# klauspost/compress

Measured on AMD Instinct MI355X. Metric: encode MB/s (input) + ratio, zstd SpeedFastest 128KiB blocks, 1/2/4/8 GPU, higher is better.
Workload: dtype u8

## Files before the change

compress_amd/csrc/kc_batch.cpp:

```cpp
#include "kc_host.h"

namespace kci {


void build_better_dict_tables(const uint8_t* dict, size_t len, int pos_bits, uint8_t* out, int reserved_bits = 0) {
    const int TB = (32 - pos_bits - reserved_bits) > 16 ? 16 : (32 - pos_bits - reserved_bits);
    auto tagOf = [&](uint32_t v) -> uint32_t { return TB > 0 ? ((v * 2654435761u) >> (32 - TB)) : 0u; };
    auto mk = [&](uint64_t pos, uint32_t val) -> uint32_t { return ((uint32_t)pos + 1u) | (tagOf(val) << pos_bits); };
    auto ld64h = [&](size_t i) -> uint64_t { uint64_t v; memcpy(&v, dict + i, 8); return v; };
    uint32_t* ltab = (uint32_t*)out;
    uint32_t* stab = (uint32_t*)(out + ((size_t)8 << 19));
    if (len < 8) return;
    for (size_t i = 0; i + 8 < len; i += 4) {
        const uint64_t cv = ld64h(i);
        for (int k = 0; k < 4; k++) {
            const uint64_t v = cv >> (8 * k);
            const uint32_t h = (uint32_t)(((v << 24) * 889523592379ULL) >> (64 - 13));
            stab[h] = mk(i + k, (uint32_t)v);
        }
    }
    for (size_t i = 0; i + 8 < len || i == 0; i++) {
        const uint64_t cv = ld64h(i);
        const uint32_t h = (uint32_t)((cv * 0xcf1bbcdcb7a56463ULL) >> (64 - 19));
        const uint32_t old = ltab[2 * h];
        ltab[2 * h] = mk(i, (uint32_t)cv);
        ltab[2 * h + 1] = old;
        if (i + 8 >= len) break;
    }
}

void build_fast_dict_table(const uint8_t* dict, size_t len, int pos_bits, uint32_t* tab) {
    const int TB = (32 - pos_bits) > 16 ? 16 : (32 - pos_bits);
    auto tagOf = [&](uint32_t v) -> uint32_t { return TB > 0 ? ((v * 2654435761u) >> (32 - TB)) : 0u; };
    auto mk = [&](uint64_t pos, uint32_t val) -> uint32_t { return ((uint32_t)pos + 1u) | (tagOf(val) << pos_bits); };
    if (len < 8) return;
    for (size_t i = 0; i + 8 < len; i += 2) {
        uint64_t cv;
        memcpy(&cv, dict + i, 8);
        const uint32_t h0 = (uint32_t)(((cv << 16) * 227718039650203ULL) >> (64 - 15));
        const uint32_t h1 = (uint32_t)((((cv >> 8) << 16) * 227718039650203ULL) >> (64 - 15));
        tab[h0] = mk(i, (uint32_t)cv);
        tab[h1] = mk(i + 1, (uint32_t)(cv >> 8));
    }
}
void build_dfast_dict_long(const uint8_t* dict, size_t len, int pos_bits, uint32_t* ltab) {
    const int TB = (32 - pos_bits) > 16 ? 16 : (32 - pos_bits);
    auto tagOf = [&](uint32_t v) -> uint32_t { return TB > 0 ? ((v * 2654435761u) >> (32 - TB)) : 0u; };
    if (len < 8) return;
    for (size_t i = 0; i == 0 || i + 8 < len; i++) {
        uint64_t cv;
        memcpy(&cv, dict + i, 8);
        const uint32_t h = (uint32_t)((cv * 0xcf1bbcdcb7a56463ULL) >> (64 - 17));
        ltab[h] = ((uint32_t)i + 1u) | (tagOf((uint32_t)cv) << pos_bits);
        if (i + 8 >= len) break;
    }
}

kc_status check_supported(kc_ctx* c, const kc_zstd_opts* o) {
    if (o->level < KC_SPEED_FASTEST || o->level > KC_SPEED_BEST) { c->err = "unknown encoder level"; return KC_ERR_UNSUPPORTED; }
    if (o->dict_len > ((uint64_t)64 << 20)) { c->err = "dictionary larger than 64 MiB not served by the device path"; return KC_ERR_UNSUPPORTED; }
    if (o->block_size < 1024 || o->block_size > kMaxCompressedBlockSize || o->window_size < kMinWindowSize) { c->err = "bad block/window size"; return KC_ERR_BAD_ARG; }
    return KC_OK;
}


size_t match_table_bytes(int level) {
    if (level == KC_SPEED_BEST) return 0;
    return level == KC_SPEED_BETTER ? kc_zbetter_table_bytes() : (level == KC_SPEED_DEFAULT ? kc_zdfast_table_bytes() : kc_zfast_table_bytes());
}

bool zfast_use_lds(const kc_ctx* c, const KcMatchParams& mp, uint32_t n_launch, int level) {
    (void)mp;
    if (level != KC_SPEED_FASTEST) return false;
    if (c->cfg.match_path == KC_PATH_HBM) return false;
    if (c->cfg.match_path == KC_PATH_LDS) return true;
    return (int64_t)n_launch <= c->cfg.zfast_lds_max_units;
}
bool zfast_lds_needs_hbm(const kc_ctx* c, const KcMatchParams& mp) {
    return (uint64_t)mp.hist0 + c->plan.max_unit_bytes > KC_ZFAST_LDS_MAX_UNIT;
}

kc_status ensure_best_slots(kc_ctx* c, uint32_t n_launch, hipStream_t st) {
    uint32_t want = (uint32_t)std::min<int64_t>((int64_t)n_launch, c->cfg.best_slots);
    if (want < 1) want = 1;
    if (!c->best_cost.p) {
        kc_status s = ensure(c, c->predef, kc_fse_predef_bytes());
        if (s != KC_OK) return s;
        if (!c->predef_ready) {
            kc_launch_fse_predef_init(c->predef.p, st);
            c->predef_ready = true;
        }
        if ((s = ensure(c, c->best_cost, 96 * 4)) != KC_OK) return s;
        kc_launch_zbest_cost(c->predef.p, (int32_t*)c->best_cost.p, st);
    }
    if (want <= c->best_n) return KC_OK;
    uint32_t n = 1;
    while (n < want) n <<= 1;
    if ((int64_t)n > c->cfg.best_slots) n = (uint32_t)c->cfg.best_slots;
    size_t fr = 0, tot = 0;
    if (hipMemGetInfo(&fr, &tot) == hipSuccess) {
        const uint64_t room = (uint64_t)((double)(fr + c->best_tables.cap) * 0.8) / kc_zbest_table_bytes();
        if (room < 1) { c->err = "device memory exhausted: no room for one SpeedBestCompression table slot (34 MiB)"; c->oom = true; return KC_ERR_UNSUPPORTED; }
        if ((uint64_t)n > room) n = (uint32_t)room;
    } else (void)hipGetLastError();
    if (n <= c->best_n) return KC_OK;
    HIPCHK(c, hipStreamSynchronize(st));
    if (c->best_tables.p) HIPCHK(c, hipFree(c->best_tables.p));
    c->best_tables.p = nullptr;
    c->best_tables.cap = 0;
    c->best_n = 0;
    {
        const hipError_t e = hipMalloc(&c->best_tables.p, (size_t)n * kc_zbest_table_bytes());
        if (e != hipSuccess) {
            (void)hipGetLastError();
            c->best_tables.p = nullptr;
            c->err = "device memory exhausted (" + std::to_string(((size_t)n * kc_zbest_table_bytes()) >> 20) + " MiB of SpeedBestCompression tables wanted)";
            c->oom = true;
            return KC_ERR_UNSUPPORTED;
        }
        c->best_tables.cap = (size_t)n * kc_zbest_table_bytes();
    }
    kc_status s;
    if ((s = ensure(c, c->best_cur, (size_t)8192 * 4)) != KC_OK) return s;
    HIPCHK(c, hipMemsetAsync(c->best_tables.p, 0, (size_t)n * kc_zbest_table_bytes(), st));
    HIPCHK(c, hipMemsetAsync(c->best_cur.p, 0, (size_t)8192 * 4, st));
    c->best_n = n;
    return KC_OK;
}

bool better_epoch_mode(const kc_ctx* c, int level, int pos_bits, int hist0) {
    return level == KC_SPEED_BETTER && !c->job_primed && c->job_hist == nullptr && pos_bits <= 22 && (hist0 == 0 || c->cfg.better_dict_epoch != 0);
}

kc_status prepare_tables(kc_ctx* c, const KcMatchParams& mp, uint32_t n_launch, hipStream_t st, int level) {
    if (level == KC_SPEED_BEST) return ensure_best_slots(c, n_launch, st);
    { const kc_status sc = tables_claim(c, st); if (sc != KC_OK) return sc; }
    c->better_epoch_now = 0;
    if (better_epoch_mode(c, level, mp.pos_bits, mp.hist0)) {
        const size_t tbb = match_table_bytes(level);
        kc_status se = ensure(c, c->tables, (size_t)n_launch * tbb);
        if (se != KC_OK) return se;
        const bool fresh = c->tab_owner != 1 || c->tab_pb != mp.pos_bits || n_launch > c->tab_units || c->tab_ep >= 15u || c->tab_ptr != c->tables.p;
        if (fresh) {
            HIPCHK(c, hipMemsetAsync(c->tables.p, 0, (size_t)n_launch * tbb, st));
            c->tab_owner = 1;
            c->tab_pb = mp.pos_bits;
            c->tab_units = n_launch;
            c->tab_ep = 1;
            c->tab_ptr = c->tables.p;
        } else {
            c->tab_ep++;
        }
        c->better_epoch_now = c->tab_ep;
        return KC_OK;
    }
    if (zfast_use_lds(c, mp, n_launch, level) && !zfast_lds_needs_hbm(c, mp) && !c->job_primed) return KC_OK;
    const bool fastEpoch = level == KC_SPEED_FASTEST && c->cfg.zfast_epoch != 0 && mp.hist0 == 0 && !c->job_primed && mp.pos_bits + KC_ZF_EPOCH_BITS + 4 <= 32;
    if (!fastEpoch) c->tab_owner = 0;
    c->fast_epoch_now = 0;
    const size_t tb = match_table_bytes(level);
    if (c->job_primed) {
        kc_status sj = ensure(c, c->tables, (size_t)n_launch * tb);
        if (sj != KC_OK) return sj;
        if (c->job_tables == nullptr) {
            HIPCHK(c, hipMemsetAsync(c->tables.p, 0, (size_t)n_launch * tb, st));
            KcPrimeParams pp;
            pp.src = mp.src;
            pp.unit_off = mp.unit_off;
            pp.unit_hist = mp.unit_hist;
            pp.unit_list = mp.unit_list;
            pp.unit_base = mp.unit_base;
            pp.n_launch = n_launch;
            pp.level = level;
            pp.pos_bits = mp.pos_bits;
            pp.tables = (uint8_t*)c->tables.p;
            pp.table_bytes = tb;
            kc_launch_zstd_prime(pp, st);
            return KC_OK;
        }
        if (mp.unit_list == nullptr) {
            HIPCHK(c, hipMemcpyAsync(c->tables.p, c->job_tables, (size_t)n_launch * tb, hipMemcpyHostToDevice, st));
            return KC_OK;
        }
        if (c->job_redo_list.size() < n_launch) { c->err = "job re-run without its unit list"; return KC_ERR_INTERNAL; }
        for (uint32_t i = 0; i < n_launch; i++)
            HIPCHK(c, hipMemcpyAsync((uint8_t*)c->tables.p + (size_t)i * tb, c->job_tables + (size_t)c->job_redo_list[i] * tb, tb, hipMemcpyHostToDevice, st));
        return KC_OK;
    }
    kc_status s = ensure(c, c->tables, (size_t)n_launch * tb);
    if (s != KC_OK) return s;
    if (mp.hist0 > 0) kc_launch_bcast((const uint8_t*)c->proto.p, (uint8_t*)c->tables.p, tb, n_launch, st);
    else if (fastEpoch) {
        const bool fresh = c->tab_owner != 2 || c->tab_pb != mp.pos_bits || n_launch > c->tab_units || c->tab_ep >= (1u << KC_ZF_EPOCH_BITS) - 1u || c->tab_ptr != c->tables.p;
        if (fresh) {
            HIPCHK(c, hipMemsetAsync(c->tables.p, 0, (size_t)n_launch * tb, st));
            c->tab_owner = 2;
            c->tab_pb = mp.pos_bits;
            c->tab_units = n_launch;
            c->tab_ep = 1;
            c->tab_ptr = c->tables.p;
        } else {
            c->tab_ep++;
        }
        c->fast_epoch_now = c->tab_ep;
    }
    else HIPCHK(c, hipMemsetAsync(c->tables.p, 0, (size_t)n_launch * tb, st));
    return KC_OK;
}

void launch_match_kernel(kc_ctx* c, const KcMatchParams& mp, uint32_t slot0, uint32_t n_launch, hipStream_t st, int level, bool lds = false) {
    if (lds) {
        KcMatchParams ml = mp;
        ml.spec_w0 = (int32_t)c->cfg.lds_spec_w0;
        ml.lds_any_big = c->plan.max_unit_bytes > (uint64_t)131072 ? 1 : 0;
        if (c->job_primed)
            kc_launch_zfast_match_lds(ml, (const uint32_t*)((uint8_t*)c->tables.p + (size_t)slot0 * match_table_bytes(level)), 1u << 15, n_launch, st);
        else
            kc_launch_zfast_match_lds(ml, mp.hist0 > 0 ? (const uint32_t*)c->proto.p : nullptr, 0u, n_launch, st);
        c->last_path = KC_PATH_LDS;
        if (zfast_lds_needs_hbm(c, mp)) {
            ml = mp;
            ml.lds_split = 1;
            ml.epoch = c->fast_epoch_now;
            ml.xseg_k = (int32_t)c->cfg.zfast_xseg_k;
            ml.empty_filter = c->cfg.zfast_filter != 0;
            ml.tuned = c->cfg.zfast_variant < 0 ? (c->last_incompressible ? 1 : 0) : (int32_t)c->cfg.zfast_variant;
            kc_launch_zfast_match_grp(ml, (uint32_t*)((uint8_t*)c->tables.p + (size_t)slot0 * match_table_bytes(level)), n_launch, st);
        }
        return;
    }
    c->last_path = KC_PATH_HBM;
    if (level == KC_SPEED_BEST) {
        kc_launch_zbest_match(mp, (uint64_t*)c->best_tables.p, (uint32_t*)c->best_cur.p, (const int32_t*)c->best_cost.p, n_launch, c->best_n, st);
        return;
    }
    uint8_t* tab = (uint8_t*)c->tables.p + (size_t)slot0 * match_table_bytes(level);
    if (level == KC_SPEED_BETTER) {
        KcMatchParams mb = mp;
        mb.epoch = c->better_epoch_now;
        mb.proto = (mb.epoch != 0u && mp.hist0 > 0) ? (const uint8_t*)c->proto.p : nullptr;
        kc_launch_zbetter_match_grp(mb, tab, n_launch, mp.hist0 > 0, st);
    }
    else if (level == KC_SPEED_DEFAULT) kc_launch_zdfast_match_grp(mp, (uint32_t*)tab, n_launch, st);
    else {
        KcMatchParams mf = mp;
        mf.epoch = c->fast_epoch_now;
        mf.xseg_k = (int32_t)c->cfg.zfast_xseg_k;
        mf.empty_filter = c->cfg.zfast_filter != 0;
        mf.tuned = c->cfg.zfast_variant < 0 ? (c->last_incompressible ? 1 : 0) : (int32_t)c->cfg.zfast_variant;
        kc_launch_zfast_match_grp(mf, (uint32_t*)tab, n_launch, st);
    }
}

kc_status launch_match(kc_ctx* c, const KcMatchParams& mp, const uint64_t* unit_off, uint32_t n_units, uint32_t n_launch, int bs, hipStream_t st, int level) {
    (void)unit_off; (void)n_units; (void)bs;
    kc_status s = prepare_tables(c, mp, n_launch, st, level);
    if (s != KC_OK) return s;
    HIPCHK(c, hipEventRecord(c->ev[7], st));
    c->ev7_valid = true;
    launch_match_kernel(c, mp, 0, n_launch, st, level, zfast_use_lds(c, mp, n_launch, level));
    return KC_OK;
}

uint32_t plan_stream_blocks(uint64_t bs, uint64_t len, const uint64_t* cuts, uint64_t n_cuts, std::vector<uint32_t>* starts, uint32_t* flags) {
    uint64_t pos = 0, ci = 0, lastStart = 0;
    uint32_t ub = 0;
    while (pos < len) {
        uint64_t e = pos + bs;
        while (ci < n_cuts && cuts[ci] <= pos) ci++;
        if (ci < n_cuts && cuts[ci] < e) e = cuts[ci];
        if (e > len) e = len;
        if (starts) starts->push_back((uint32_t)pos);
        lastStart = pos;
        pos = e;
        ub++;
    }
    const bool flushedAtEnd = n_cuts > 0 && cuts[n_cuts - 1] >= len;
    const bool tailBuffered = ub > 0 && !flushedAtEnd && (len - lastStart) < bs;
    const bool streamU = len > 0 && !(ub == 1 && tailBuffered);
    *flags = (streamU ? 1u : 0u) | ((streamU && !tailBuffered) ? 2u : 0u);
    return ub;
}

kc_status batch_begin(kc_ctx* c, const kc_zstd_opts* o, const uint8_t* d_src_base, const uint64_t* unit_off, uint32_t n_units,
                      uint8_t* d_dst, uint64_t dst_cap, ChunkFeed* feed) {
    hipStream_t st = c->stream;
    if (c->pend) { c->err = "a batch is already in flight on this context"; return KC_ERR_BAD_ARG; }
    const int bs = o->block_size;
    Plan& pl = c->plan;
    pl.n_units = n_units;
    pl.blk0.resize(n_units + 1);
    pl.stage_off.resize(n_units + 1);
    pl.rel_off.resize(n_units + 1);
    uint64_t so = 0;
    uint32_t nb = 0;
    const bool irregular = c->cuts != nullptr;
    pl.blk_start.clear();
    pl.unit_flags.clear();
    for (uint32_t i = 0; i < n_units; i++) {
        const uint64_t len = unit_off[i + 1] - unit_off[i];
        pl.blk0[i] = nb;
        pl.stage_off[i] = so;
        pl.rel_off[i] = unit_off[i] - unit_off[0];
        uint32_t ub = (uint32_t)((len - (c->job_hist ? c->job_hist[i] : 0) + bs - 1) / bs);
        if (irregular) {
            const uint64_t* cp = c->cuts + c->cut_off[c->cut_unit0 + i];
            const uint64_t nc = c->cut_off[c->cut_unit0 + i + 1] - c->cut_off[c->cut_unit0 + i];
            uint32_t fl = 0;
            ub = plan_stream_blocks((uint64_t)bs, len, cp, nc, &pl.blk_start, &fl);
            pl.unit_flags.push_back(fl);
        }
        nb += ub;
        so += ((uint64_t)kc_zstd_max_encoded_size(o, (int64_t)len) + (irregular ? 3ull * (c->cut_off[c->cut_unit0 + i + 1] - c->cut_off[c->cut_unit0 + i]) + 3ull : 0ull) + 15) & ~(uint64_t)15;
    }
    pl.blk0[n_units] = nb;
    pl.stage_off[n_units] = so;
    pl.rel_off[n_units] = unit_off[n_units] - unit_off[0];
    pl.n_blocks = nb;
    pl.seq_stride = (uint32_t)(bs / 4 + 8);
    pl.lit_stride = (uint32_t)(bs + 64);
    if (so > dst_cap) { c->err = "dst_cap smaller than the sum of MaxEncodedSize(unit)"; return KC_ERR_DST_TOO_SMALL; }

    kc_status s;
    if ((s = ensure(c, c->unit_off, (n_units + 1) * 8)) || (s = ensure(c, c->unit_blk0, (n_units + 1) * 4)) ||
        (s = ensure(c, c->stage_off, (n_units + 1) * 8)) || (s = ensure(c, c->out_off, (n_units + 1 + (feed ? feed->cut.size() : 0)) * 8)) ||
        (s = ensure(c, c->seqs, (size_t)nb * pl.seq_stride * 8)) || (s = ensure(c, c->aux, (size_t)nb * pl.seq_stride * 8)) ||
        (s = ensure(c, c->lits, (size_t)nb * pl.lit_stride)) || (s = ensure(c, c->meta, (size_t)nb * sizeof(KcBlkMeta))) ||
        (s = ensure(c, c->stage, so + 64)) || (s = ensure(c, c->out_size, (size_t)n_units * 4)) ||
        (s = ensure(c, c->xxh, (size_t)n_units * 8)) || (s = ensure(c, c->redo, (size_t)n_units * 4)) ||
        (s = ensure(c, c->redo_blk, (size_t)nb + 1)) || (s = ensure(c, c->pop_blk, (size_t)nb + 1)) || (s = ensure(c, c->unit_list, (size_t)n_units * 4)) ||
        (s = ensure(c, c->predef, kc_fse_predef_bytes())) || (s = ensure(c, c->errflag, 64)))
        return s;
    if (!c->predef_ready) {
        kc_launch_fse_predef_init(c->predef.p, st);
        c->predef_ready = true;
    }
    if (irregular) {
        if ((s = ensure(c, c->blk_start, ((size_t)nb + 1) * 4)) || (s = ensure(c, c->unit_flags, (size_t)n_units * 4))) return s;
        if (nb) HIPCHK(c, hipMemcpyAsync(c->blk_start.p, pl.blk_start.data(), (size_t)nb * 4, hipMemcpyHostToDevice, st));
        HIPCHK(c, hipMemcpyAsync(c->unit_flags.p, pl.unit_flags.data(), (size_t)n_units * 4, hipMemcpyHostToDevice, st));
    }
    {
        auto same = [](const std::vector<uint8_t>& held, const void* p, size_t n, const void* dev, const void* held_dev) {
            return dev == held_dev && held.size() == n && memcmp(held.data(), p, n) == 0;
        };
        auto keep = [](std::vector<uint8_t>& held, const void* p, size_t n) { held.assign((const uint8_t*)p, (const uint8_t*)p + n); };
        const size_t n8 = (size_t)(n_units + 1) * 8, n4 = (size_t)(n_units + 1) * 4;
        if (!same(c->up_unit_off, pl.rel_off.data(), n8, c->unit_off.p, c->up_ptr[0])) {
            HIPCHK(c, hipMemcpyAsync(c->unit_off.p, pl.rel_off.data(), n8, hipMemcpyHostToDevice, st));
            keep(c->up_unit_off, pl.rel_off.data(), n8);
            c->up_ptr[0] = c->unit_off.p;
        }
        if (!same(c->up_blk0, pl.blk0.data(), n4, c->unit_blk0.p, c->up_ptr[1])) {
            HIPCHK(c, hipMemcpyAsync(c->unit_blk0.p, pl.blk0.data(), n4, hipMemcpyHostToDevice, st));
            keep(c->up_blk0, pl.blk0.data(), n4);
            c->up_ptr[1] = c->unit_blk0.p;
        }
        if (!same(c->up_stage_off, pl.stage_off.data(), n8, c->stage_off.p, c->up_ptr[2])) {
            HIPCHK(c, hipMemcpyAsync(c->stage_off.p, pl.stage_off.data(), n8, hipMemcpyHostToDevice, st));
            keep(c->up_stage_off, pl.stage_off.data(), n8);
            c->up_ptr[2] = c->stage_off.p;
        }
    }

    const uint8_t* d_src = d_src_base + unit_off[0];
    const bool useDict = o->dict != nullptr && o->dict_len > 0;
    const int hist0 = useDict ? (int)o->dict_len : 0;
    uint64_t maxLen = 16;
    for (uint32_t i = 0; i < n_units; i++) maxLen = std::max<uint64_t>(maxLen, unit_off[i + 1] - unit_off[i]);
    pl.max_unit_bytes = maxLen;
    int pos_bits = 1;
    while (((uint64_t)1 << pos_bits) <= (uint64_t)hist0 + maxLen + 2) pos_bits++;
    if (std::min<uint64_t>((uint64_t)o->window_size, (uint64_t)hist0 + maxLen) + 3 > 0xFFFFFFull) {
        c->err = "window above 8 MiB with units above 16 MiB: offsets beyond the device path's 24-bit sequence field";
        return KC_ERR_UNSUPPORTED;
    }
    const uint8_t* k_src = d_src;
    const uint64_t* k_off = (const uint64_t*)c->unit_off.p;
    if (useDict) {
        std::vector<uint64_t> woff(n_units + 1);
        for (uint32_t i = 0; i <= n_units; i++) woff[i] = pl.rel_off[i] + (uint64_t)i * (uint64_t)hist0;
        if ((s = ensure(c, c->work, woff[n_units] + 64)) || (s = ensure(c, c->work_off, (n_units + 1) * 8)) ||
            (s = ensure(c, c->dictbuf, (size_t)hist0 + 64)) || (s = ensure(c, c->proto, kc_zbetter_table_bytes())))
            return s;
        HIPCHK(c, hipMemcpyAsync(c->work_off.p, woff.data(), (n_units + 1) * 8, hipMemcpyHostToDevice, st));
        const bool epochMode = better_epoch_mode(c, o->level, pos_bits, hist0);
        uint64_t key = 0xcbf29ce484222325ULL;
        for (int i = 0; i < hist0; i++) key = (key ^ o->dict[i]) * 0x100000001b3ULL;
        key ^= ((uint64_t)(uint32_t)hist0 << 32) ^ ((uint64_t)o->level << 8) ^ ((uint64_t)pos_bits << 16) ^ (epochMode ? (uint64_t)1 << 24 : 0);
        if (key == 0) key = 1;
        const size_t tbz = kc_zbetter_table_bytes();
        if (c->proto_key != key || c->proto_ptr != c->proto.p || c->dictbuf_ptr != c->dictbuf.p) {
            c->proto_key = 0;
            HIPCHK(c, hipMemcpyAsync(c->dictbuf.p, o->dict, (size_t)hist0, hipMemcpyHostToDevice, st));
            std::vector<uint8_t> proto(tbz, 0);
            if (o->level == KC_SPEED_BEST) {  }
            else if (o->level == KC_SPEED_BETTER) {
                build_better_dict_tables(o->dict, (size_t)hist0, pos_bits, proto.data(), epochMode ? 4 : 0);
            } else if (o->level == KC_SPEED_DEFAULT) {
                build_dfast_dict_long(o->dict, (size_t)hist0, pos_bits, (uint32_t*)proto.data());
                build_fast_dict_table(o->dict, (size_t)hist0, pos_bits, (uint32_t*)(proto.data() + ((size_t)4 << 17)));
            } else build_fast_dict_table(o->dict, (size_t)hist0, pos_bits, (uint32_t*)proto.data());
            HIPCHK(c, hipMemcpyAsync(c->proto.p, proto.data(), proto.size(), hipMemcpyHostToDevice, st));
            HIPCHK(c, hipStreamSynchronize(st));
            c->proto_key = key;
            c->proto_ptr = c->proto.p;
            c->dictbuf_ptr = c->dictbuf.p;
        } else {
            HIPCHK(c, hipStreamSynchronize(st));
        }
        kc_launch_prefix_units(d_src, (const uint64_t*)c->unit_off.p, (const uint64_t*)c->work_off.p, (const uint8_t*)c->dictbuf.p,
                               (uint32_t)hist0, (uint8_t*)c->work.p, n_units, st);
        k_src = (const uint8_t*)c->work.p;
        k_off = (const uint64_t*)c->work_off.p;
    }
    if (c->job_hist) {
        if (useDict) { c->err = "jobs of a WithConcurrentBlocks stream take no dictionary"; return KC_ERR_INTERNAL; }
        if ((s = ensure(c, c->d_job_hist, (size_t)n_units * 4)) || (s = ensure(c, c->d_job_flags, (size_t)n_units * 4))) return s;
        HIPCHK(c, hipMemcpyAsync(c->d_job_hist.p, c->job_hist, (size_t)n_units * 4, hipMemcpyHostToDevice, st));
        HIPCHK(c, hipMemcpyAsync(c->d_job_flags.p, c->job_flags, (size_t)n_units * 4, hipMemcpyHostToDevice, st));
    }
    KcMatchParams mp;
    memset(&mp, 0, sizeof(mp));
    mp.unit_hist = c->job_hist ? (const uint32_t*)c->d_job_hist.p : nullptr;
    mp.job_flags = c->job_hist ? (const uint32_t*)c->d_job_flags.p : nullptr;
    mp.src = k_src;
    mp.src_end = k_src + (useDict ? pl.rel_off[n_units] + (uint64_t)n_units * (uint64_t)hist0 : pl.rel_off[n_units]);
    mp.unit_off = k_off;
    mp.hist0 = hist0;
    mp.pos_bits = pos_bits;
    mp.stream_mode = c->stream_mode;
    mp.rep1 = (int32_t)o->dict_offsets[0];
    mp.rep2 = (int32_t)o->dict_offsets[1];
    mp.rep3 = (int32_t)o->dict_offsets[2];
    if (mp.rep1 <= 0 || mp.rep2 <= 0 || mp.rep3 <= 0) { mp.rep1 = 1; mp.rep2 = 4; mp.rep3 = 8; }
    mp.unit_blk0 = (const uint32_t*)c->unit_blk0.p;
    mp.seqs = (uint64_t*)c->seqs.p;
    mp.meta = (KcBlkMeta*)c->meta.p;
    mp.pop_blk = nullptr;
    mp.unit_list = nullptr;
    mp.blk_start = irregular ? (const uint32_t*)c->blk_start.p : nullptr;
    mp.unit_flags = irregular ? (const uint32_t*)c->unit_flags.p : nullptr;
    mp.seq_stride = pl.seq_stride;
    mp.block_size = bs;
    mp.max_match_off = o->window_size;
    mp.spec_w0 = c->cfg.spec_w0 >= 0 ? (int)c->cfg.spec_w0 : (o->level == KC_SPEED_DEFAULT ? 2 : (o->level == KC_SPEED_BETTER ? 16 : 1));
    mp.spec_grow = c->cfg.spec_grow >= 0 ? (int)c->cfg.spec_grow : (o->level == KC_SPEED_FASTEST ? 1 : (o->level == KC_SPEED_BETTER ? 0 : 2));
    if (mp.spec_w0 < 1) mp.spec_w0 = 1;
    if (mp.spec_w0 > 64) mp.spec_w0 = 64;

    KcEntropyParams ep;
    memset(&ep, 0, sizeof(ep));
    ep.unit_hist = mp.unit_hist;
    ep.job_flags = mp.job_flags;
    ep.src = k_src;
    ep.unit_off = k_off;
    ep.hist0 = hist0;
    ep.stream_mode = c->stream_mode;
    ep.stream_sync = o->concurrent == 1;
    ep.dict_huf = nullptr;
    ep.dict_huf_len = 0;
    ep.dict_huf_log = 0;
    if (o->dict_huf_len > 0) {
        uint8_t blobh[768];
        memcpy(blobh, o->dict_huf_val, 512);
        memcpy(blobh + 512, o->dict_huf_nbits, 256);
        if ((s = ensure(c, c->dicthuf, 768))) return s;
        HIPCHK(c, hipMemcpyAsync(c->dicthuf.p, blobh, 768, hipMemcpyHostToDevice, st));
        HIPCHK(c, hipStreamSynchronize(st));
        ep.dict_huf = (const uint8_t*)c->dicthuf.p;
        ep.dict_huf_len = o->dict_huf_len;
        ep.dict_huf_log = o->dict_huf_log;
    }
    ep.unit_blk0 = mp.unit_blk0;
    ep.seqs = mp.seqs;
    ep.meta = mp.meta;
    ep.lits = (uint8_t*)c->lits.p;
    ep.aux = (uint64_t*)c->aux.p;
    ep.stage = (uint8_t*)c->stage.p;
    ep.stage_off = (const uint64_t*)c->stage_off.p;
    ep.out_size = (uint32_t*)c->out_size.p;
    ep.xxh = (const uint64_t*)c->xxh.p;
    ep.redo_mask = (uint32_t*)c->redo.p;
    ep.redo_blk = (uint8_t*)c->redo_blk.p;
    ep.blk_start = mp.blk_start;
    ep.unit_flags = mp.unit_flags;
    ep.unit_list = nullptr;
    ep.predef = c->predef.p;
    ep.seq_stride = pl.seq_stride;
    ep.lit_stride = pl.lit_stride;
    ep.block_size = bs;
    ep.window_size = o->window_size;
    ep.crc = o->crc;
    ep.single = o->single;
    ep.no_entropy = o->no_entropy;
    ep.all_lit_entropy = o->all_lit_entropy;
    ep.full_zero = o->full_zero;
    ep.dict_id = o->dict_id;
    ep.err_flag = (uint32_t*)c->errflag.p;
    if ((s = ensure(c, c->rawdef, ((size_t)nb + 1) * sizeof(KcRawDef))) != KC_OK) return s;
    ep.rawdef = (KcRawDef*)c->rawdef.p;
    const bool fuse_xxh = c->cfg.fuse_raw_xxh != 0 && o->crc && !c->job_hist && !useDict && hist0 == 0 && !irregular && (bs % 256) == 0 && feed == nullptr;
    ep.unit_raw = nullptr;
    if (fuse_xxh) {
        if ((s = ensure(c, c->unit_raw, (size_t)n_units * 4 + 4)) != KC_OK) return s;
        ep.unit_raw = (uint32_t*)c->unit_raw.p;
        ep.xxh = nullptr;
    }
    {
        KcClearList cl;
        memset(&cl, 0, sizeof(cl));
        auto add = [&](void* q, size_t bytes) { cl.p[cl.count] = q; cl.n16[cl.count] = (bytes + 15) / 16; cl.count++; };
        add(c->redo.p, (size_t)n_units * 4);
        add(c->redo_blk.p, (size_t)nb + 1);
        add(c->errflag.p, 64);
        add(c->rawdef.p, ((size_t)nb + 1) * sizeof(KcRawDef));
        if (fuse_xxh) add(c->unit_raw.p, (size_t)n_units * 4);
        kc_launch_clear(cl, st);
    }
    ep.prof = nullptr;
    const bool k2prof = c->cfg.k2_prof != 0;
    if (k2prof) {
        if ((s = ensure(c, c->prof, 48 * 8)) != KC_OK) return s;
        HIPCHK(c, hipMemsetAsync(c->prof.p, 0, 48 * 8, st));
        ep.prof = (unsigned long long*)c->prof.p;
        mp.prof = (unsigned long long*)c->prof.p + 32;
    }

    if (c->chain_after) HIPCHK(c, hipStreamWaitEvent(st, c->chain_after->ev[2], 0));
    HIPCHK(c, hipEventRecord(c->ev[0], st));
    c->prescan_ran = false;
    {
        const bool tuned_now = c->cfg.zfast_variant < 0 ? c->last_incompressible : c->cfg.zfast_variant == 1;
        const bool want = c->cfg.zfast_prescan > 0 || (c->cfg.zfast_prescan < 0 && tuned_now);
        if (want && o->level == KC_SPEED_FASTEST && fuse_xxh && !c->stream_mode && !o->all_lit_entropy && bs >= 16 && n_units > 0) {
            if (c->probe_bs != bs || c->probe_rel.p == nullptr) {
                std::vector<uint32_t> rel(4096);
                uint32_t n = kc_zfast_probe_positions(bs, rel.data(), (uint32_t)rel.size());
                if (n > rel.size()) { rel.resize(n); n = kc_zfast_probe_positions(bs, rel.data(), (uint32_t)rel.size()); }
                if ((s = ensure(c, c->probe_rel, (size_t)n * 4 + 16)) != KC_OK) return s;
                HIPCHK(c, hipMemcpyAsync(c->probe_rel.p, rel.data(), (size_t)n * 4, hipMemcpyHostToDevice, st));
                HIPCHK(c, hipStreamSynchronize(st));
                c->probe_bs = bs;
                c->probe_n = n;
            }
            if ((s = ensure(c, c->unit_done, (size_t)n_units * 4 + 16)) != KC_OK) return s;
            KcPrescanParams pp;
            memset(&pp, 0, sizeof(pp));
            pp.src = k_src;
            pp.unit_off = k_off;
            pp.unit_blk0 = mp.unit_blk0;
            pp.n_units = n_units;
            pp.block_size = bs;
            pp.probe_rel = (const uint32_t*)c->probe_rel.p;
            pp.n_probe = c->probe_n;
            pp.rep1 = mp.rep1;
            pp.rep2 = mp.rep2;
            pp.meta = mp.meta;
            pp.unit_done = (uint32_t*)c->unit_done.p;
            pp.stage = ep.stage;
            pp.stage_off = ep.stage_off;
            pp.out_size = ep.out_size;
            pp.rawdef = ep.rawdef;
            pp.unit_raw = ep.unit_raw;
            pp.window_size = o->window_size;
            pp.crc = o->crc;
            pp.single = o->single;
            pp.dict_id = o->dict_id;
            kc_launch_zfast_prescan(pp, st);
            mp.unit_done = pp.unit_done;
            ep.unit_done = pp.unit_done;
            c->prescan_ran = true;
        }
    }
    mp.unit_base = 0;
    ep.unit_base = 0;
    if (feed == nullptr) {
        if (o->crc && !c->job_hist && !fuse_xxh) kc_launch_xxh64(d_src, (const uint64_t*)c->unit_off.p, n_units, (uint64_t*)c->xxh.p, st);
        HIPCHK(c, hipEventRecord(c->ev[1], st));
        if ((s = launch_match(c, mp, unit_off, n_units, n_units, bs, st, o->level)) != KC_OK) return s;
    } else {
        if (useDict) { c->err = "chunk feed does not take dictionaries"; return KC_ERR_INTERNAL; }
        HIPCHK(c, hipEventRecord(c->ev[1], st));
        if ((s = prepare_tables(c, mp, n_units, st, o->level)) != KC_OK) return s;
        const bool feed_lds = zfast_use_lds(c, mp, n_units, o->level);
        HIPCHK(c, hipEventRecord(c->ev[6], st));
        const size_t nchunk = feed->cut.size() - 1;
        for (size_t k = 0; k < nchunk; k++) {
            if (!feed->wait_recorded(k)) { c->err = "host pipeline: staging failed"; return KC_ERR_HIP; }
            hipStream_t sk = feed->streams[k % feed->streams.size()];
            const uint32_t u0 = feed->cut[k], nk = feed->cut[k + 1] - feed->cut[k];
            HIPCHK(c, hipStreamWaitEvent(sk, c->ev[6], 0));
            HIPCHK(c, hipStreamWaitEvent(sk, feed->landed[k], 0));
            if (o->crc) kc_launch_xxh64(d_src, (const uint64_t*)c->unit_off.p + u0, nk, (uint64_t*)c->xxh.p + u0, sk);
            KcMatchParams mk = mp;
            mk.unit_base = u0;
            launch_match_kernel(c, mk, u0, nk, sk, o->level, feed_lds);
            KcEntropyParams ek = ep;
            ek.unit_base = u0;
            kc_launch_zstd_entropy(ek, nk, sk);
            feed->loc_off = (uint64_t*)c->out_off.p;
            kc_launch_scan_sizes((const uint32_t*)c->out_size.p + u0, nk, feed->loc_off + u0 + k, sk);
            kc_launch_compact((const uint8_t*)c->stage.p, (const uint64_t*)c->stage_off.p + u0, (const uint32_t*)c->out_size.p + u0,
                              feed->loc_off + u0 + k, d_dst + pl.stage_off[u0], nk, sk, ep.src, ep.unit_off + u0, ep.unit_blk0 + u0, ep.rawdef);
            HIPCHK(c, hipEventRecord(feed->done[k], sk));
        }
        for (size_t k = 0; k < nchunk; k++) HIPCHK(c, hipStreamWaitEvent(st, feed->done[k], 0));
    }
    HIPCHK(c, hipEventRecord(c->ev[2], st));
    HIPCHK(c, hipGetLastError());
    Pending* P = new Pending();
    P->o = *o;
    P->mp = mp;
    P->ep = ep;
    P->unit_off.assign(unit_off, unit_off + n_units + 1);
    P->n_units = n_units;
    P->d_dst = d_dst;
    P->need = pl.stage_off[n_units];
    P->fed = feed != nullptr;
    P->bs = bs;
    P->k2prof = k2prof;
    c->pend = P;
    return KC_OK;
}

kc_status batch_end(kc_ctx* c, uint64_t* out_off_host, uint64_t* produced) {
    if (!c->pend) { c->err = "no batch in flight on this context"; return KC_ERR_BAD_ARG; }
    std::unique_ptr<Pending> P((Pending*)c->pend);
    c->pend = nullptr;
    hipStream_t st = c->stream;
    if (c->stream2 != nullptr) {
        st = c->stream2;
        HIPCHK(c, hipStreamWaitEvent(st, c->ev[2], 0));
    }
    const kc_zstd_opts* o = &P->o;
    KcMatchParams& mp = P->mp;
    KcEntropyParams& ep = P->ep;
    const uint64_t* unit_off = P->unit_off.data();
    const uint32_t n_units = P->n_units;
    uint8_t* d_dst = P->d_dst;
    const int bs = P->bs;
    const bool k2prof = P->k2prof;
    kc_status s;
    kc_launch_zstd_entropy(ep, n_units, st);
    HIPCHK(c, hipEventRecord(c->ev[3], st));
    HIPCHK(c, hipGetLastError());

    auto finish_pass = [&]() -> kc_status {
        kc_launch_scan_sizes((const uint32_t*)c->out_size.p, n_units, (uint64_t*)c->out_off.p, st);
        if (ep.unit_raw != nullptr) {
            KcXxhFinParams xf;
            xf.src = ep.src;
            xf.unit_off = ep.unit_off;
            xf.n_units = n_units;
            xf.stage = (uint8_t*)c->stage.p;
            xf.stage_off = (const uint64_t*)c->stage_off.p;
            xf.out_size = (const uint32_t*)c->out_size.p;
            xf.out_off = (const uint64_t*)c->out_off.p;
            xf.dst = d_dst;
            xf.unit_raw = ep.unit_raw;
            xf.rawdef = ep.rawdef;
            xf.unit_blk0 = ep.unit_blk0;
            xf.xxh_out = (uint64_t*)c->xxh.p;
            xf.mode = (int32_t)c->cfg.xxh_fin_mode;
            kc_launch_xxh64_fin(xf, st);
        }
        kc_launch_compact((const uint8_t*)c->stage.p, (const uint64_t*)c->stage_off.p, (const uint32_t*)c->out_size.p,
                          (const uint64_t*)c->out_off.p, d_dst, n_units, st, ep.src, ep.unit_off, ep.unit_blk0, ep.rawdef, ep.unit_raw);
        HIPCHK(c, hipGetLastError());
        return KC_OK;
    };
    HIPCHK(c, hipEventRecord(c->ev[4], st));
    if ((s = finish_pass()) != KC_OK) return s;
    HIPCHK(c, hipEventRecord(c->ev[5], st));
    uint32_t redo_units = 0;
    {
        const Plan& pl = c->plan;
        const uint32_t nb = pl.n_blocks;
        uint32_t maxBlocks = 1;
        for (uint32_t i = 0; i < n_units; i++) maxBlocks = std::max(maxBlocks, pl.blk0[i + 1] - pl.blk0[i]);
        std::vector<uint32_t> redo(n_units), list;
        std::vector<uint8_t> redo_blk, pop_blk;
        uint32_t errv[16];
        for (uint32_t iter = 0;; iter++) {
            HIPCHK(c, hipMemcpyAsync(redo.data(), c->redo.p, (size_t)n_units * 4, hipMemcpyDeviceToHost, st));
            HIPCHK(c, hipMemcpyAsync(errv, c->errflag.p, 64, hipMemcpyDeviceToHost, st));
            std::vector<uint32_t> doneh;
            if (iter == 0 && c->prescan_ran) {
                doneh.resize(n_units);
                HIPCHK(c, hipMemcpyAsync(doneh.data(), c->unit_done.p, (size_t)n_units * 4, hipMemcpyDeviceToHost, st));
            }
            HIPCHK(c, hipStreamSynchronize(st));
            if (iter == 0) {
                c->last_prescan_units = 0;
                for (uint32_t v : doneh) c->last_prescan_units += v != 0u;
            }
            if (errv[0] != 0) {
                char b[96];
                snprintf(b, sizeof(b), "device invariant violated (code %u)", errv[0]);
                c->err = b;
                return errv[0] == 100u ? KC_ERR_UNSUPPORTED : KC_ERR_INTERNAL;
            }
            list.clear();
            for (uint32_t i = 0; i < n_units; i++)
                if (redo[i]) list.push_back(i);
            if (list.empty()) break;
            if (iter > maxBlocks + 1) { c->err = "speculation re-run did not converge"; return KC_ERR_INTERNAL; }
            redo_blk.resize(nb);
            if (pop_blk.empty()) pop_blk.assign(nb, 0);
            HIPCHK(c, hipMemcpyAsync(redo_blk.data(), c->redo_blk.p, nb, hipMemcpyDeviceToHost, st));
            HIPCHK(c, hipStreamSynchronize(st));
            for (uint32_t i : list)
                for (uint32_t b = pl.blk0[i]; b < pl.blk0[i + 1]; b++)
                    if (redo_blk[b]) { pop_blk[b] = 1; break; }
            redo_units += (uint32_t)list.size();
            HIPCHK(c, hipMemcpyAsync(c->pop_blk.p, pop_blk.data(), nb, hipMemcpyHostToDevice, st));
            HIPCHK(c, hipMemcpyAsync(c->unit_list.p, list.data(), list.size() * 4, hipMemcpyHostToDevice, st));
            HIPCHK(c, hipMemsetAsync(c->redo.p, 0, (size_t)n_units * 4, st));
            HIPCHK(c, hipMemsetAsync(c->redo_blk.p, 0, (size_t)nb + 1, st));
            c->job_redo_list = list;
            mp.pop_blk = (const uint8_t*)c->pop_blk.p;
            mp.unit_list = (const uint32_t*)c->unit_list.p;
            ep.unit_list = mp.unit_list;
            if ((s = launch_match(c, mp, unit_off, n_units, (uint32_t)list.size(), bs, st, o->level)) != KC_OK) return s;
            kc_launch_zstd_entropy(ep, (uint32_t)list.size(), st);
            HIPCHK(c, hipGetLastError());
            HIPCHK(c, hipStreamSynchronize(st));
        }
    }
    if (redo_units != 0) {
        HIPCHK(c, hipEventRecord(c->ev[4], st));
        if ((s = finish_pass()) != KC_OK) return s;
        HIPCHK(c, hipEventRecord(c->ev[5], st));
    }
    HIPCHK(c, hipMemcpyAsync(out_off_host, c->out_off.p, (n_units + 1) * 8, hipMemcpyDeviceToHost, st));
    HIPCHK(c, hipStreamSynchronize(st));
    HIPCHK(c, hipGetLastError());
    float t01 = 0, t12 = 0, t23 = 0, t34 = 0, t45 = 0, t05 = 0, tk2 = 0;
    (void)hipEventElapsedTime(&t01, c->ev[0], c->ev[1]);
    (void)hipEventElapsedTime(&t12, c->ev[1], c->ev[2]);
    (void)hipEventElapsedTime(&t23, c->ev[2], c->ev[3]);
    (void)hipEventElapsedTime(&t34, c->ev[3], c->ev[4]);
    (void)hipEventElapsedTime(&t45, c->ev[4], c->ev[5]);
    (void)hipEventElapsedTime(&t05, c->ev[0], c->ev[5]);
    if (c->ev7_valid) {
        float t17 = 0;
        if (hipEventElapsedTime(&t17, c->ev[1], c->ev[7]) == hipSuccess && t17 >= 0 && t17 <= t12) c->last.prep_ms += t17;
        c->ev7_valid = false;
    }
    tk2 = t23;
    c->last.match_ms += t12;
    c->last.entropy_ms += tk2;
    c->last.other_ms += t01 + t34 + t45;
    c->last.total_ms += t05;
    c->last.redo_units += redo_units;
    if (k2prof) {
        unsigned long long pv[48];
        HIPCHK(c, hipMemcpy(pv, c->prof.p, sizeof(pv), hipMemcpyDeviceToHost));
        {
            unsigned long long lt = 0;
            for (int i = 32; i < 40; i++) lt += pv[i];
            if (lt && o->level == KC_SPEED_DEFAULT) {
                fprintf(stderr, "[dfast stats] per unit: probes looked up %.0f, committed %.0f, candidate / repeat 16-byte loads %.0f, long lookups at s+1 %.0f, matches %.0f, offset-2 matches %.0f, ring refills (128 B) %.0f\n",
                        (double)pv[32] / n_units, (double)pv[33] / n_units, (double)pv[34] / n_units, (double)pv[35] / n_units, (double)pv[36] / n_units, (double)pv[37] / n_units, (double)pv[38] / n_units);
            } else if (lt) {
                fprintf(stderr, "[LDS match prof] shader clocks per phase (window, probe bytes, table, candidates issued, verdicts, commit, -, round tail):");
                for (int i = 32; i < 40; i++) fprintf(stderr, " %.1f%%", 100.0 * (double)pv[i] / (double)lt);
                fprintf(stderr, "  (total %.4g cycles over %u units)\n", (double)lt, n_units);
            }
        }
        {
            unsigned long long ft = 0;
            for (int i = 40; i < 48; i++) ft += pv[i];
            if (ft) {
                fprintf(stderr, "[K2 fine] wave 0, shader clocks per unit; -DKC_K2_FINE=1: gather (pass A, barrier, step: sequences + scan, step: literal loads + ORs, step: flush + histogram, step: carry + zero, tail, closing barrier); =2: (Huffman size pass, payload zero fill + barrier, stream emit, barrier, payload copy + headers, code staging, chains, pack):");
                for (int i = 40; i < 48; i++) fprintf(stderr, " %.0f", (double)pv[i] / (double)(n_units ? n_units : 1));
                fprintf(stderr, "\n");
            }
        }
        unsigned long long tot = 0;
        for (int i = 0; i < 16; i++) tot += pv[i];
        fprintf(stderr, "[K2 prof] shader-clock share per phase:");
        for (int i = 0; i < 14; i++) fprintf(stderr, " p%d=%.1f%%", i, tot ? 100.0 * (double)pv[i] / (double)tot : 0.0);
        fprintf(stderr, "  (total %.3g cycles over %u units)\n", (double)tot, n_units);
        fprintf(stderr, "[K2 prof] tANS chains (counted with -DKC_CHAIN_STATS): %llu chunk-streams (%llu RLE, %llu predefined), %llu repair passes (LL %llu, OF %llu, ML %llu; %llu on RLE tables), %llu segments re-encoded\n",
                pv[16], pv[26], pv[27], pv[17], pv[18], pv[19], pv[20], pv[25], pv[24]);
    }
    *produced = out_off_host[n_units];
    {
        const uint64_t in_total = unit_off[n_units] - unit_off[0];
        c->last_incompressible = in_total >= (1u << 20) && (double)*produced >= 0.98 * (double)in_total;
    }
    return KC_OK;
}

uint64_t zstd_unit_scratch(const kc_zstd_opts* o, uint64_t len, uint64_t n_cuts) {
    const uint64_t bsz = (uint64_t)o->block_size;
    const uint64_t table_b = o->level == KC_SPEED_BEST ? 0 : o->level == KC_SPEED_BETTER ? kc_zbetter_table_bytes() : (o->level == KC_SPEED_DEFAULT ? kc_zdfast_table_bytes() : kc_zfast_table_bytes());
    const uint64_t per_block = 2 * (bsz / 4 + 8) * 8 + (bsz + 64) + sizeof(KcBlkMeta);
    const uint64_t hist0 = (o->dict != nullptr) ? o->dict_len : 0;
    const uint64_t blocks = (len + bsz - 1) / bsz + n_cuts;
    const uint64_t enc = ((uint64_t)kc_zstd_max_encoded_size(o, (int64_t)len) + 3 * n_cuts + 3 + 15) & ~(uint64_t)15;
    return table_b + blocks * per_block + enc + (hist0 ? hist0 + len : 0) + 64;
}

uint64_t scratch_budget(kc_ctx* c) {
    uint64_t budget = c->max_scratch_bytes;
    size_t fr = 0, tot = 0;
    if (hipMemGetInfo(&fr, &tot) == hipSuccess) {
        uint64_t held = 0;
        const DevBuf* bufs[] = {&c->seqs, &c->aux, &c->lits, &c->meta, &c->stage, &c->tables, &c->work};
        for (const DevBuf* b : bufs) held += b->cap;
        const uint64_t avail = (uint64_t)((double)(fr + held) * 0.85);
        if (avail < budget) budget = avail;
    } else {
        (void)hipGetLastError();
    }
    return budget;
}

kc_status feed_finish(kc_ctx* c, bool* redo_needed) {
    if (!c->pend) { c->err = "no batch in flight on this context"; return KC_ERR_BAD_ARG; }
    std::unique_ptr<Pending> P((Pending*)c->pend);
    c->pend = nullptr;
    hipStream_t st = c->stream;
    const uint32_t n_units = P->n_units;
    std::vector<uint32_t> redo(n_units);
    uint32_t errv[16];
    HIPCHK(c, hipMemcpyAsync(redo.data(), c->redo.p, (size_t)n_units * 4, hipMemcpyDeviceToHost, st));
    HIPCHK(c, hipMemcpyAsync(errv, c->errflag.p, 64, hipMemcpyDeviceToHost, st));
    HIPCHK(c, hipStreamSynchronize(st));
    HIPCHK(c, hipGetLastError());
    if (errv[0] != 0) {
        char b[96];
        snprintf(b, sizeof(b), "device invariant violated (code %u)", errv[0]);
        c->err = b;
        return errv[0] == 100u ? KC_ERR_UNSUPPORTED : KC_ERR_INTERNAL;
    }
    *redo_needed = false;
    for (uint32_t i = 0; i < n_units; i++) if (redo[i]) *redo_needed = true;
    return KC_OK;
}

kc_status run_batch(kc_ctx* c, const kc_zstd_opts* o, const uint8_t* d_src_base, const uint64_t* unit_off, uint32_t n_units,
                    uint8_t* d_dst, uint64_t dst_cap, uint64_t* out_off_host, uint64_t* produced) {
    kc_status s = batch_begin(c, o, d_src_base, unit_off, n_units, d_dst, dst_cap);
    if (s != KC_OK) return s;
    return batch_end(c, out_off_host, produced);
}

}

extern "C" {

kc_status kc_zstd_encode_units_dev(kc_ctx* c, const kc_zstd_opts* o, const uint8_t* d_src, const uint64_t* unit_off, uint32_t n_units,
                                   uint8_t* d_dst, uint64_t dst_cap, uint64_t* out_off) {
    if (!c || !o || !unit_off || !out_off || (n_units && (!d_src || !d_dst))) return KC_ERR_BAD_ARG;
    c->err.clear();
    c->last = kc_timings{0, 0, 0, 0, 0, 0};
    kc_status s = check_supported(c, o);
    if (s != KC_OK) return s;
    HIPCHK(c, hipSetDevice(c->device));
    for (uint32_t i = 0; i < n_units; i++) {
        if (unit_off[i + 1] < unit_off[i]) { c->err = "unit_off not ascending"; return KC_ERR_BAD_ARG; }
        if (unit_off[i + 1] - unit_off[i] > KC_MAX_UNIT_BYTES) {
            c->err = "unit larger than 1 GiB: not served by the device path";
            return KC_ERR_UNSUPPORTED;
        }
    }
    out_off[0] = 0;
    c->last_batches = 0;
    uint64_t pos = 0;
    uint32_t i0 = 0;
    std::vector<uint64_t> tmp;
    auto unit_scratch = [&](uint32_t i) {
        const uint64_t nc = c->cuts ? c->cut_off[i + 1] - c->cut_off[i] : 0;
        return zstd_unit_scratch(o, unit_off[i + 1] - unit_off[i], nc);
    };
    uint64_t budget = scratch_budget(c);
    for (int attempt = 0;; attempt++) {
        bool oom = false;
        while (i0 < n_units) {
            uint32_t i1 = i0;
            const uint64_t cap_bytes = o->level == KC_SPEED_BETTER ? ((uint64_t)1 << 30) : c->max_batch_bytes;
            const uint32_t cap_units = o->level == KC_SPEED_BETTER ? 16384u : 0xFFFFFFFFu;
            uint64_t scratch = 0;
            while (i1 < n_units) {
                const uint64_t us = unit_scratch(i1);
                if (i1 > i0 && (unit_off[i1 + 1] - unit_off[i0] > cap_bytes || i1 - i0 >= cap_units || (scratch + us) + ((scratch + us) >> 3) > budget)) break;
                scratch += us;
                i1++;
            }
            const uint32_t nb = i1 - i0;
            tmp.resize(nb + 1);
            uint64_t produced = 0;
            c->cut_unit0 = i0;
            c->oom = false;
            s = run_batch(c, o, d_src, unit_off + i0, nb, d_dst + pos, dst_cap - pos, tmp.data(), &produced);
            if (s == KC_ERR_UNSUPPORTED && c->oom && nb > 1 && attempt < 6) { oom = true; break; }
            if (s != KC_OK) return s;
            c->last_batches++;
            for (uint32_t k = 0; k <= nb; k++) out_off[i0 + k] = pos + tmp[k];
            pos += produced;
            i0 = i1;
        }
        if (!oom) break;
        budget /= 2;
        c->err.clear();
    }
    if (n_units == 0) out_off[0] = 0;
    return KC_OK;
}

}
namespace kci {
kc_status validate_units(kc_ctx* c, const kc_zstd_opts* o, const uint64_t* unit_off, uint32_t n_units) {
    for (uint32_t i = 0; i < n_units; i++) {
        if (unit_off[i + 1] < unit_off[i]) { c->err = "unit_off not ascending"; return KC_ERR_BAD_ARG; }
        if (unit_off[i + 1] - unit_off[i] > KC_MAX_UNIT_BYTES) {
            c->err = "unit larger than 1 GiB: not served by the device path";
            return KC_ERR_UNSUPPORTED;
        }
    }
    return KC_OK;
}
}
extern "C" {

kc_status kc_zstd_encode_units_dev_begin(kc_ctx* c, const kc_zstd_opts* o, const uint8_t* d_src, const uint64_t* unit_off, uint32_t n_units,
                                         uint8_t* d_dst, uint64_t dst_cap) {
    if (!c || !o || !unit_off || n_units == 0 || !d_src || !d_dst) return KC_ERR_BAD_ARG;
    c->err.clear();
    c->last = kc_timings{0, 0, 0, 0, 0, 0};
    kc_status s = check_supported(c, o);
    if (s != KC_OK) return s;
    HIPCHK(c, hipSetDevice(c->device));
    if ((s = validate_units(c, o, unit_off, n_units)) != KC_OK) return s;
    const uint64_t cap_bytes = o->level == KC_SPEED_BETTER ? ((uint64_t)1 << 30) : c->max_batch_bytes;
    if (unit_off[n_units] - unit_off[0] > cap_bytes || (o->level == KC_SPEED_BETTER && n_units > 16384u)) {
        c->err = "begin/end serves one device batch; use kc_zstd_encode_units_dev for larger inputs";
        return KC_ERR_UNSUPPORTED;
    }
    return batch_begin(c, o, d_src, unit_off, n_units, d_dst, dst_cap);
}

kc_status kc_zstd_encode_units_dev_end(kc_ctx* c, uint64_t* out_off) {
    if (!c || !out_off) return KC_ERR_BAD_ARG;
    HIPCHK(c, hipSetDevice(c->device));
    uint64_t produced = 0;
    return batch_end(c, out_off, &produced);
}

kc_status kc_zstd_encode_units_dev_end_at(kc_ctx* c, uint8_t* d_dst, uint64_t dst_cap, uint64_t* out_off) {
    if (!c || !out_off || !d_dst) return KC_ERR_BAD_ARG;
    if (!c->pend) { c->err = "no batch in flight on this context"; return KC_ERR_BAD_ARG; }
    Pending* P = (Pending*)c->pend;
    if (P->fed) { c->err = "a chunk-fed batch has written its frames already"; return KC_ERR_UNSUPPORTED; }
    if (P->need > dst_cap) { c->err = "dst_cap smaller than the sum of MaxEncodedSize(unit)"; return KC_ERR_DST_TOO_SMALL; }
    P->d_dst = d_dst;
    return kc_zstd_encode_units_dev_end(c, out_off);
}

void kc_ctx_chain_after(kc_ctx* c, kc_ctx* prev) {
    if (c) c->chain_after = prev;
}

kc_status kc_zstd_encode_streams_dev(kc_ctx* c, const kc_zstd_opts* o, const uint8_t* d_src, const uint64_t* unit_off, uint32_t n_units,
                                     uint8_t* d_dst, uint64_t dst_cap, uint64_t* out_off) {
    if (!c || !o) return KC_ERR_BAD_ARG;
    c->stream_mode = 1;
    const kc_status s = kc_zstd_encode_units_dev(c, o, d_src, unit_off, n_units, d_dst, dst_cap, out_off);
    c->stream_mode = 0;
    return s;
}

}
```

compress_amd/csrc/kc_ctx.cpp:

```cpp
#include "kc_host.h"

extern "C" {

void kc_zstd_opts_default(kc_zstd_opts* o) {
    memset(o, 0, sizeof(*o));
    o->level = KC_SPEED_DEFAULT;
    o->window_size = 8 << 20;
    o->block_size = kMaxCompressedBlockSize;
    o->crc = 1;
    o->single = -1;
    o->full_zero = 1;
    o->no_entropy = 0;
    o->all_lit_entropy = 0;
    o->low_mem = 0;
    o->dict_offsets[0] = 1; o->dict_offsets[1] = 4; o->dict_offsets[2] = 8;
    o->concurrent = 0;
}

int kc_zstd_opts_concurrency(kc_zstd_opts* o, int n) {
    if (n < 1) return KC_ERR_BAD_ARG;
    o->concurrent = n;
    return KC_OK;
}

int kc_zstd_opts_level(kc_zstd_opts* o, int l) {
    if (l < KC_SPEED_FASTEST || l > 4) return KC_ERR_BAD_ARG;
    o->level = l;
    if (!o->custom_window) {
        switch (l) {
        case KC_SPEED_FASTEST:
            o->window_size = 4 << 20;
            if (!o->custom_block) o->block_size = 1 << 16;
            break;
        default:
            o->window_size = 8 << 20;
            break;
        }
    }
    if (!o->custom_alent) o->all_lit_entropy = l > KC_SPEED_DEFAULT;
    return KC_OK;
}

int kc_zstd_opts_window(kc_zstd_opts* o, int n) {
    if (n < kMinWindowSize || n > kMaxWindowSize || (n & (n - 1)) != 0) return KC_ERR_BAD_ARG;
    o->window_size = n;
    o->custom_window = 1;
    if (o->block_size > o->window_size) {
        o->block_size = o->window_size;
        o->custom_block = 1;
    }
    return KC_OK;
}
int kc_zstd_opts_crc(kc_zstd_opts* o, int b) { o->crc = b != 0; return KC_OK; }
int kc_zstd_opts_zero_frames(kc_zstd_opts* o, int b) { o->full_zero = b != 0; return KC_OK; }
int kc_zstd_opts_no_entropy(kc_zstd_opts* o, int b) { o->no_entropy = b != 0; return KC_OK; }
int kc_zstd_opts_all_lit_entropy(kc_zstd_opts* o, int b) { o->custom_alent = 1; o->all_lit_entropy = b != 0; return KC_OK; }
int kc_zstd_opts_single_segment(kc_zstd_opts* o, int b) { o->single = b != 0; return KC_OK; }
int kc_zstd_opts_dict_raw(kc_zstd_opts* o, uint32_t id, const uint8_t* content, uint64_t len) {
    if (len > ((uint64_t)1 << 31)) return KC_ERR_BAD_ARG;
    o->dict_id = id;
    o->dict = content;
    o->dict_len = len;
    o->dict_offsets[0] = 1; o->dict_offsets[1] = 4; o->dict_offsets[2] = 8;
    o->dict_huf_len = 0;
    o->dict_huf_log = 0;
    return KC_OK;
}

int64_t kc_zstd_max_encoded_size(const kc_zstd_opts* o, int64_t size) {
    int64_t frameHeader = 4 + 2;
    if (o->dict != nullptr || o->dict_id != 0) frameHeader += 4;
    if (size < 256) frameHeader++;
    else if (size < 65536 + 256) frameHeader += 2;
    else if (size < 0x7fffffff) frameHeader += 4;
    else frameHeader += 8;
    if (o->crc) frameHeader += 4;
    const int64_t blocks = (size + o->block_size) / o->block_size;
    return frameHeader + 3 * blocks + size;
}

namespace {
struct SelfCheck {
    std::mutex m;
    std::condition_variable cv;
    bool done = false;
    kc_status st = KC_OK;
    std::string text;
};
std::mutex g_sc_m;
int g_sc_state[64] = {0};
kc_status g_sc_status[64];
std::string g_sc_text[64];
thread_local std::string t_create_err;

void selfcheck_body(int device, const std::shared_ptr<SelfCheck>& sc) {
    kc_status st = KC_OK;
    std::string text;
    uint8_t h_in[256];
    for (int i = 0; i < 256; i++) h_in[i] = (uint8_t)i;
    const uint64_t h_off[2] = {0, 256};
    uint64_t h_out = 0;
    uint8_t* d_in = nullptr;
    uint64_t *d_off = nullptr, *d_out = nullptr;
    hipStream_t s = nullptr;
    auto fail = [&](const char* what, hipError_t e) { st = KC_ERR_HIP; text = std::string("device self-check: ") + what + ": " + hipGetErrorString(e); };
    hipError_t e = hipSetDevice(device);
    if (e != hipSuccess) fail("hipSetDevice", e);
    if (st == KC_OK && (e = hipStreamCreateWithFlags(&s, hipStreamNonBlocking)) != hipSuccess) fail("hipStreamCreate", e);
    if (st == KC_OK && (e = hipMalloc((void**)&d_in, 256 + 64)) != hipSuccess) fail("hipMalloc", e);
    if (st == KC_OK && (e = hipMalloc((void**)&d_off, 16)) != hipSuccess) fail("hipMalloc", e);
    if (st == KC_OK && (e = hipMalloc((void**)&d_out, 8)) != hipSuccess) fail("hipMalloc", e);
    if (st == KC_OK && (e = hipMemcpyAsync(d_in, h_in, 256, hipMemcpyHostToDevice, s)) != hipSuccess) fail("hipMemcpyAsync (H2D)", e);
    if (st == KC_OK && (e = hipMemcpyAsync(d_off, h_off, 16, hipMemcpyHostToDevice, s)) != hipSuccess) fail("hipMemcpyAsync (H2D)", e);
    if (st == KC_OK) {
        kc_launch_xxh64(d_in, d_off, 1, d_out, s);
        if ((e = hipGetLastError()) != hipSuccess) fail("kernel launch", e);
    }
    if (st == KC_OK && (e = hipMemcpyAsync(&h_out, d_out, 8, hipMemcpyDeviceToHost, s)) != hipSuccess) fail("hipMemcpyAsync (D2H)", e);
    if (st == KC_OK && (e = hipStreamSynchronize(s)) != hipSuccess) fail("hipStreamSynchronize", e);
    if (st == KC_OK && h_out != 0x1FACBE8406CD904BULL) {
        char b[160];
        snprintf(b, sizeof(b), "device self-check: XXH64 known answer differs (got %016llx, want 1facbe8406cd904b): the device computes wrong results", (unsigned long long)h_out);
        st = KC_ERR_INTERNAL;
        text = b;
    }
    if (d_in) (void)hipFree(d_in);
    if (d_off) (void)hipFree(d_off);
    if (d_out) (void)hipFree(d_out);
    if (s) (void)hipStreamDestroy(s);
    std::lock_guard<std::mutex> lk(sc->m);
    sc->st = st;
    sc->text = text;
    sc->done = true;
    sc->cv.notify_all();
}

kc_status device_selfcheck(int device, std::string* text) {
    if (device < 0 || device >= 64) return KC_OK;
    std::lock_guard<std::mutex> g(g_sc_m);
    if (g_sc_state[device] == 0) {
        auto sc = std::make_shared<SelfCheck>();
        std::thread([device, sc] { selfcheck_body(device, sc); }).detach();
        std::unique_lock<std::mutex> lk(sc->m);
        const int deadline_s = 90;
        if (!sc->cv.wait_for(lk, std::chrono::seconds(deadline_s), [&] { return sc->done; })) {
            g_sc_state[device] = -1;
            g_sc_status[device] = KC_ERR_HIP;
            g_sc_text[device] = "device self-check: the device did not answer a 256-byte known-answer launch within " + std::to_string(deadline_s) + " s (hung queue or faulted context): no kc_* call was attempted";
        } else {
            g_sc_state[device] = sc->st == KC_OK ? 1 : -1;
            g_sc_status[device] = sc->st;
            g_sc_text[device] = sc->text;
        }
    }
    if (g_sc_state[device] < 0) { *text = g_sc_text[device]; return g_sc_status[device]; }
    return KC_OK;
}
}

const char* kc_create_error(void) { return t_create_err.c_str(); }

kc_status kc_ctx_create(kc_ctx** out, int device, void* stream) {
    if (!out) return KC_ERR_BAD_ARG;
    *out = nullptr;
    t_create_err.clear();
    int n = 0;
    if (hipGetDeviceCount(&n) != hipSuccess || n <= 0 || device < 0 || device >= n) { t_create_err = "no such HIP device"; return KC_ERR_NO_DEVICE; }
    {
        const kc_status sc = device_selfcheck(device, &t_create_err);
        if (sc != KC_OK) return sc;
    }
    kc_ctx* c = new kc_ctx();
    c->device = device;
    if (hipSetDevice(device) != hipSuccess || hipGetDeviceProperties(&c->prop, device) != hipSuccess) {
        delete c;
        return KC_ERR_NO_DEVICE;
    }
    if (stream) {
        c->stream = (hipStream_t)stream;
    } else {
        if (hipStreamCreate(&c->stream) != hipSuccess) { delete c; return KC_ERR_HIP; }
        c->own_stream = true;
    }
    for (auto& e : c->ev)
        if (hipEventCreate(&e) != hipSuccess) { delete c; return KC_ERR_HIP; }
    *out = c;
    return KC_OK;
}

kc_status kc_ctx_set_option(kc_ctx* c, int key, int64_t v) {
    if (!c) return KC_ERR_BAD_ARG;
    KcCfg& g = c->cfg;
    switch (key) {
        case KC_OPT_MATCH_PATH: if (v < KC_PATH_AUTO || v > KC_PATH_LDS) return KC_ERR_BAD_ARG; g.match_path = v; break;
        case KC_OPT_ZFAST_LDS_MAX_UNITS: g.zfast_lds_max_units = v; break;
        case KC_OPT_S2_LDS_MAX_BLOCKS: g.s2_lds_max_blocks = v; break;
        case KC_OPT_SPEC_W0: g.spec_w0 = v; break;
        case KC_OPT_SPEC_GROW: g.spec_grow = v; break;
        case KC_OPT_LDS_SPEC_W0: g.lds_spec_w0 = v; break;
        case KC_OPT_S2_LDS_SPEC_W0: g.s2_lds_spec_w0 = v; break;
        case KC_OPT_HOST_SERIAL: g.host_serial = v; break;
        case KC_OPT_HOST_PIPE_MIB: g.host_pipe_mib = v; break;
        case KC_OPT_HOST_OVERLAP_MIN_MIB: g.host_overlap_min_mib = v; break;
        case KC_OPT_HOST_COPY_THREADS: g.host_copy_threads = v; break;
        case KC_OPT_HOST_TRACE: g.host_trace = v; break;
        case KC_OPT_HOST_ROLL: g.host_roll = v != 0; break;
        case KC_OPT_HOST_ROLL_MIB: if (v < 0) return KC_ERR_BAD_ARG; g.host_roll_mib = v; break;
        case KC_OPT_HOST_CHUNK_MIB: g.host_chunks.clear(); if (v > 0) g.host_chunks.push_back((uint64_t)v << 20); break;
        case KC_OPT_HOST_CHUNK_MIB_APPEND: if (v < 1) return KC_ERR_BAD_ARG; g.host_chunks.push_back((uint64_t)v << 20); break;
        case KC_OPT_K2_PROF: g.k2_prof = v; break;
        case KC_OPT_S2_HOOK_WAIT_US: g.hook_wait_us = v; break;
        case KC_OPT_S2_HOOK_BATCH: g.hook_batch = v < 1 ? 1 : v; break;
        case KC_OPT_S2_HOOK_LANES: g.hook_lanes = v < 1 ? 1 : (v > 8 ? 8 : v); break;
        case KC_OPT_S2_HOOK_HOST_FIRST: g.hook_host_first = v < -1 ? -1 : v; break;
        case KC_OPT_TEST_FEED_REDO: g.test_feed_redo = v; break;
        case KC_OPT_MAX_SCRATCH_MIB: if (v < 1) return KC_ERR_BAD_ARG; c->max_scratch_bytes = (uint64_t)v << 20; break;
        case KC_OPT_BEST_SLOTS: if (v < 1 || v > 8192) return KC_ERR_BAD_ARG; g.best_slots = v; break;
        case KC_OPT_S2_VARIANT: if (v != KC_S2_VARIANT_GO && v != KC_S2_VARIANT_AMD64) return KC_ERR_BAD_ARG; g.s2_variant = v; break;
        case KC_OPT_BETTER_DICT_EPOCH: g.better_dict_epoch = v != 0; break;
        case KC_OPT_ZFAST_EPOCH: g.zfast_epoch = v != 0; break;
        case KC_OPT_ZFAST_XSEG_K: if (v < 0) return KC_ERR_BAD_ARG; g.zfast_xseg_k = v > (1 << 30) ? (1 << 30) : v; break;
        case KC_OPT_FUSE_RAW_XXH: g.fuse_raw_xxh = v != 0; break;
        case KC_OPT_ZFAST_FILTER: g.zfast_filter = v != 0; break;
        case KC_OPT_ZFAST_VARIANT: if (v < -1 || v > 1) return KC_ERR_BAD_ARG; g.zfast_variant = v; break;
        case KC_OPT_ZFAST_PRESCAN: if (v < -1 || v > 1) return KC_ERR_BAD_ARG; g.zfast_prescan = v; break;
        case KC_OPT_XXH_FIN_MODE: if (v < 0 || v > 3) return KC_ERR_BAD_ARG; g.xxh_fin_mode = v; break;
        case KC_OPT_JOB_PRIME: g.job_prime = v != 0; break;
        case KC_OPT_DSTREAM_BLOCKS: if (v < 1 || v > 4096) return KC_ERR_BAD_ARG; g.dstream_blocks = v; break;
        case KC_OPT_STAGE2_STREAM: if (c->pend) return KC_ERR_BAD_ARG; c->stream2 = (hipStream_t)(intptr_t)v; break;
        default: return KC_ERR_BAD_ARG;
    }
    return KC_OK;
}

int64_t kc_ctx_get_option(const kc_ctx* c, int key) {
    if (!c) return -1;
    const KcCfg& g = c->cfg;
    switch (key) {
        case KC_OPT_MATCH_PATH: return g.match_path;
        case KC_OPT_ZFAST_LDS_MAX_UNITS: return g.zfast_lds_max_units;
        case KC_OPT_S2_LDS_MAX_BLOCKS: return g.s2_lds_max_blocks;
        case KC_OPT_SPEC_W0: return g.spec_w0;
        case KC_OPT_SPEC_GROW: return g.spec_grow;
        case KC_OPT_LDS_SPEC_W0: return g.lds_spec_w0;
        case KC_OPT_S2_LDS_SPEC_W0: return g.s2_lds_spec_w0;
        case KC_OPT_HOST_SERIAL: return g.host_serial;
        case KC_OPT_HOST_PIPE_MIB: return g.host_pipe_mib;
        case KC_OPT_HOST_OVERLAP_MIN_MIB: return g.host_overlap_min_mib;
        case KC_OPT_HOST_COPY_THREADS: return g.host_copy_threads;
        case KC_OPT_HOST_TRACE: return g.host_trace;
        case KC_OPT_HOST_ROLL: return g.host_roll;
        case KC_OPT_HOST_ROLL_MIB: return g.host_roll_mib;
        case KC_OPT_HOST_CHUNK_MIB: return g.host_chunks.empty() ? 0 : (int64_t)(g.host_chunks[0] >> 20);
        case KC_OPT_K2_PROF: return g.k2_prof;
        case KC_OPT_S2_HOOK_WAIT_US: return g.hook_wait_us;
        case KC_OPT_S2_HOOK_BATCH: return g.hook_batch;
        case KC_OPT_S2_HOOK_LANES: return g.hook_lanes;
        case KC_OPT_S2_HOOK_HOST_FIRST: return g.hook_host_first;
        case KC_OPT_TEST_FEED_REDO: return g.test_feed_redo;
        case KC_OPT_MAX_SCRATCH_MIB: return (int64_t)(c->max_scratch_bytes >> 20);
        case KC_OPT_BEST_SLOTS: return g.best_slots;
        case KC_OPT_S2_VARIANT: return g.s2_variant;
        case KC_OPT_BETTER_DICT_EPOCH: return g.better_dict_epoch;
        case KC_OPT_ZFAST_EPOCH: return g.zfast_epoch;
        case KC_OPT_ZFAST_XSEG_K: return g.zfast_xseg_k;
        case KC_OPT_FUSE_RAW_XXH: return g.fuse_raw_xxh;
        case KC_OPT_ZFAST_FILTER: return g.zfast_filter;
        case KC_OPT_ZFAST_VARIANT: return g.zfast_variant;
        case KC_OPT_ZFAST_PRESCAN: return g.zfast_prescan;
        case KC_OPT_XXH_FIN_MODE: return g.xxh_fin_mode;
        case KC_OPT_JOB_PRIME: return g.job_prime;
        case KC_OPT_DSTREAM_BLOCKS: return g.dstream_blocks;
        case KC_OPT_STAGE2_STREAM: return (int64_t)(intptr_t)c->stream2;
        case KC_OPT_LAST_PATH: return c->last_path;
        case KC_OPT_LAST_PRESCAN_UNITS: return c->last_prescan_units;
        case KC_OPT_LAST_BATCHES: return c->last_batches;
        default: return -1;
    }
}

static void ctx_free_scratch(kc_ctx* c) {
    DevBuf* bufs[] = {&c->unit_off, &c->unit_blk0, &c->stage_off, &c->seqs, &c->aux, &c->lits, &c->meta, &c->stage, &c->out_size, &c->xxh,
                      &c->redo, &c->popmask, &c->unit_list, &c->out_off, &c->blk_start, &c->unit_flags, &c->redo_blk, &c->pop_blk, &c->predef, &c->errflag, &c->tmp_src, &c->tmp_dst, &c->tables, &c->prof, &c->work, &c->work_off, &c->dictbuf, &c->proto, &c->dicthuf,
                      &c->d_job_hist, &c->d_job_flags, &c->rawdef, &c->unit_raw, &c->unit_done, &c->probe_rel, &c->best_tables, &c->best_cur, &c->best_cost};
    for (DevBuf* b : bufs) {
        if (b->p) (void)hipFree(b->p);
        b->p = nullptr;
        b->cap = 0;
    }
    for (DevBuf& b : c->zd) {
        if (b.p) (void)hipFree(b.p);
        b.p = nullptr;
        b.cap = 0;
    }
    for (DevBuf& b : c->s2d) {
        if (b.p) (void)hipFree(b.p);
        b.p = nullptr;
        b.cap = 0;
    }
    c->predef_ready = false;
    c->tab_owner = 0;
    c->tab_ptr = nullptr;
    c->tab_units = c->tab_ep = 0;
    c->proto_key = 0;
    c->proto_ptr = c->dictbuf_ptr = nullptr;
    c->best_n = 0;
    c->probe_bs = 0;
    c->probe_n = 0;
    c->preclear_bytes = 0;
    c->preclear_ptr = nullptr;
    c->up_ptr[0] = c->up_ptr[1] = c->up_ptr[2] = nullptr;
}

kc_status kc_ctx_trim(kc_ctx* c) {
    if (!c) return KC_ERR_BAD_ARG;
    if (c->pend || c->job_active) { c->err = "kc_ctx_trim: a batch or a submitted job is in flight on this context"; return KC_ERR_BAD_ARG; }
    HIPCHK(c, hipSetDevice(c->device));
    HIPCHK(c, hipStreamSynchronize(c->stream));
    ctx_free_scratch(c);
    if (c->hpipe) { host_pipe_free(c->hpipe); c->hpipe = nullptr; }
    return KC_OK;
}

kc_status kc_device_trim(int device) { return kci::host_roll_trim(device); }

kc_status kc_host_alloc(void** out, uint64_t bytes) {
    if (!out || bytes == 0) return KC_ERR_BAD_ARG;
    *out = nullptr;
    const hipError_t e = hipHostMalloc(out, (size_t)bytes, hipHostMallocDefault);
    if (e != hipSuccess) { (void)hipGetLastError(); *out = nullptr; return e == hipErrorOutOfMemory ? KC_ERR_UNSUPPORTED : KC_ERR_HIP; }
    return KC_OK;
}
void kc_host_free(void* p) {
    if (p) (void)hipHostFree(p);
}

void kc_ctx_destroy(kc_ctx* c) {
    if (!c) return;
    if (c->job_active && c->job.joinable()) c->job.join();
    (void)hipSetDevice(c->device);
    ctx_free_scratch(c);
    for (auto& e : c->ev)
        if (e) (void)hipEventDestroy(e);
    if (c->ev_preclear) (void)hipEventDestroy(c->ev_preclear);
    if (c->pend) { delete (Pending*)c->pend; c->pend = nullptr; }
    if (c->hook) { s2_hook_free(c->hook); c->hook = nullptr; }
    if (c->hpipe) { host_pipe_free(c->hpipe); c->hpipe = nullptr; }
    if (c->own_stream && c->stream) (void)hipStreamDestroy(c->stream);
    delete c;
}

const char* kc_last_error(const kc_ctx* c) { return c ? c->err.c_str() : "null context"; }

kc_status kc_device_info(const kc_ctx* c, int32_t* n_cu, int32_t* lds_per_cu, int32_t* clock_khz, char* name, size_t name_cap) {
    if (!c) return KC_ERR_BAD_ARG;
    if (n_cu) *n_cu = c->prop.multiProcessorCount;
    if (lds_per_cu) *lds_per_cu = (int32_t)c->prop.maxSharedMemoryPerMultiProcessor;
    if (clock_khz) *clock_khz = c->prop.clockRate;
    if (name && name_cap) { strncpy(name, c->prop.gcnArchName, name_cap - 1); name[name_cap - 1] = 0; }
    return KC_OK;
}

kc_status kc_last_timings(const kc_ctx* c, kc_timings* t) {
    if (!c || !t) return KC_ERR_BAD_ARG;
    *t = c->last;
    return KC_OK;
}

}
```

compress_amd/csrc/kc_dev.h:

```cpp
#pragma once
#include <hip/hip_runtime.h>
#include <stdint.h>

#define KC_WAVE 64

struct __attribute__((packed)) kc_u64u { uint64_t v; };
struct __attribute__((packed)) kc_u32u { uint32_t v; };
struct __attribute__((packed)) kc_u16u { uint16_t v; };
__device__ __forceinline__ uint64_t ld64(const uint8_t* p) { return ((const kc_u64u*)p)->v; }
__device__ __forceinline__ void st64(uint8_t* p, uint64_t v) { ((kc_u64u*)p)->v = v; }
__device__ __forceinline__ uint32_t ld32(const uint8_t* p) { return ((const kc_u32u*)p)->v; }
__device__ __forceinline__ void st32(uint8_t* p, uint32_t v) { ((kc_u32u*)p)->v = v; }
__device__ __forceinline__ uint16_t ld16(const uint8_t* p) { return ((const kc_u16u*)p)->v; }
struct __attribute__((packed)) kc_u128u { uint32_t x, y, z, w; };
__device__ __forceinline__ uint4 ld128u(const uint8_t* p) {
    const kc_u128u v = *(const kc_u128u*)p;
    return make_uint4(v.x, v.y, v.z, v.w);
}

#ifdef KC_HIPEMU
#define KC_WAVE_SYNC() hipemu::wave_sync()
#else
#define KC_WAVE_SYNC() do { __builtin_amdgcn_fence(__ATOMIC_SEQ_CST, "wavefront"); __builtin_amdgcn_wave_barrier(); } while (0)
#endif

__device__ __forceinline__ int lane_id() { return (int)(threadIdx.x & 63); }
__device__ __forceinline__ uint64_t ballot64(bool p) { return __ballot(p); }
__device__ __forceinline__ int ctz64(uint64_t v) { return __builtin_ctzll(v); }
struct KcUnitBlocks { int nblk; bool streamU; bool emptyLast; };
__device__ __forceinline__ KcUnitBlocks kc_unit_blocks(const uint32_t* blk_start, const uint32_t* unit_flags, const uint32_t* unit_blk0,
                                                       uint32_t u, int ulen, int bs, int stream_mode) {
    KcUnitBlocks r;
    if (blk_start != nullptr) {
        const uint32_t f = unit_flags[u];
        r.nblk = (int)(unit_blk0[u + 1] - unit_blk0[u]);
        r.streamU = (f & 1u) != 0u;
        r.emptyLast = (f & 2u) != 0u;
    } else {
        r.nblk = (ulen + bs - 1) / bs;
        r.streamU = stream_mode != 0 && ulen >= bs;
        r.emptyLast = r.streamU && (ulen % bs) == 0;
    }
    return r;
}
__device__ __forceinline__ int kc_blk_begin(const uint32_t* blk_start, uint32_t blk0, int b, int bs) {
    return blk_start != nullptr ? (int)blk_start[blk0 + (uint32_t)b] : b * bs;
}
__device__ __forceinline__ int kc_blk_end(const uint32_t* blk_start, uint32_t blk0, int b, int nblk, int bs, int ulen) {
    if (blk_start != nullptr) return b + 1 < nblk ? (int)blk_start[blk0 + (uint32_t)b + 1u] : ulen;
    const int e = (b + 1) * bs;
    return e < ulen ? e : ulen;
}

__device__ __forceinline__ uint32_t bcast32(uint32_t v, int srcLane) { return (uint32_t)__shfl((int)v, srcLane, 64); }
__device__ __forceinline__ uint64_t bcast64(uint64_t v, int srcLane) {
    uint32_t lo = bcast32((uint32_t)v, srcLane), hi = bcast32((uint32_t)(v >> 32), srcLane);
    return ((uint64_t)hi << 32) | lo;
}
__device__ __forceinline__ uint32_t rdlane32(uint32_t v, int srcLane) { return (uint32_t)__builtin_amdgcn_readlane((int)v, srcLane); }
__device__ __forceinline__ uint64_t rdlane64(uint64_t v, int srcLane) {
    return (uint64_t)rdlane32((uint32_t)v, srcLane) | ((uint64_t)rdlane32((uint32_t)(v >> 32), srcLane) << 32);
}
__device__ __forceinline__ int uni(int v) { return __builtin_amdgcn_readfirstlane(v); }
__device__ __forceinline__ uint32_t uniu(uint32_t v) { return (uint32_t)__builtin_amdgcn_readfirstlane((int)v); }

__device__ __forceinline__ int bits_len32(uint32_t v) { return v == 0 ? 0 : 32 - __builtin_clz(v); }
__device__ __forceinline__ uint32_t high_bit(uint32_t v) { return (uint32_t)(bits_len32(v) - 1); }

#define KC_PRIME4 2654435761u
#define KC_PRIME5 889523592379ULL
#define KC_PRIME6 227718039650203ULL
#define KC_PRIME8 0xcf1bbcdcb7a56463ULL
__device__ __forceinline__ uint32_t hash4(uint32_t u, int bits) { return (u * KC_PRIME4) >> (32 - bits); }
__device__ __forceinline__ uint32_t hash5(uint64_t u, int bits) { return (uint32_t)(((u << 24) * KC_PRIME5) >> (64 - bits)); }
__device__ __forceinline__ uint32_t hash6(uint64_t u, int bits) { return (uint32_t)(((u << 16) * KC_PRIME6) >> (64 - bits)); }
__device__ __forceinline__ uint32_t hash8(uint64_t u, int bits) { return (uint32_t)((u * KC_PRIME8) >> (64 - bits)); }

__device__ __forceinline__ uint64_t seq_pack(uint32_t ll, uint32_t ml, uint32_t of) {
    return (uint64_t)of | ((uint64_t)ml << 24) | ((uint64_t)ll << 44);
}
__device__ __forceinline__ uint32_t seq_of(uint64_t s) { return (uint32_t)(s & 0xFFFFFF); }
__device__ __forceinline__ uint32_t seq_ml(uint64_t s) { return (uint32_t)((s >> 24) & 0xFFFFF); }
__device__ __forceinline__ uint32_t seq_ll(uint64_t s) { return (uint32_t)(s >> 44); }

__device__ __forceinline__ int wave_matchlen(const uint8_t* a, const uint8_t* b, int left, int lane) {
    int n = 0;
    int width = 8;
    for (;;) {
        int words = (left - n) >> 3;
        int active = words < width ? words : width;
        uint64_t diff = 0;
        if (lane < active) diff = ld64(a + n + 8 * lane) ^ ld64(b + n + 8 * lane);
        uint64_t m = ballot64(diff != 0);
        if (m) {
            int fl = ctz64(m);
            uint64_t d = rdlane64(diff, fl);
            return n + 8 * fl + (ctz64(d) >> 3);
        }
        n += 8 * active;
        if (active < width) break;
        width = 64;
    }
    int tail = left - n;
    bool ne = lane < tail && a[n + lane] != b[n + lane];
    uint64_t m = ballot64(ne);
    return n + (m ? ctz64(m) : tail);
}

__device__ __forceinline__ int wave_backlen(const uint8_t* base, int s, int t, int kmax, int lane) {
    int cnt = 0;
    while (cnt < kmax) {
        int k = cnt + lane + 1;
        bool ne = true;
        if (k <= kmax) ne = base[t - k] != base[s - k];
        uint64_t m = ballot64(ne);
        int c = m ? ctz64(m) : 64;
        cnt += c;
        if (c < 64) break;
    }
    return cnt < kmax ? cnt : kmax;
}

template <int G>
__device__ __forceinline__ uint32_t gballot(bool p, int grp) {
    return (uint32_t)((ballot64(p) >> (grp * G)) & ((1ull << G) - 1ull));
}
template <int G>
__device__ __forceinline__ uint64_t gbcast64(uint64_t v, int grp, int srcLig) {
    const int src = grp * G + srcLig;
    const uint32_t lo = (uint32_t)__shfl((int)(uint32_t)v, src, 64), hi = (uint32_t)__shfl((int)(uint32_t)(v >> 32), src, 64);
    return ((uint64_t)hi << 32) | lo;
}
template <int G>
__device__ __forceinline__ uint32_t gbcast32(uint32_t v, int grp, int srcLig) {
    return (uint32_t)__shfl((int)v, grp * G + srcLig, 64);
}
template <int G>
__device__ __forceinline__ int grp_matchlen(const uint8_t* __restrict__ base, int a, int b, int left, int lig, int grp) {
    int n = 0;
    for (;;) {
        const int words = (left - n) >> 3;
        const int active = words < G ? words : G;
        uint64_t diff = 0;
        if (lig < active) diff = ld64(base + a + n + 8 * lig) ^ ld64(base + b + n + 8 * lig);
        const uint32_t m = gballot<G>(diff != 0, grp);
        if (m) {
            const int fl = __builtin_ctz(m);
            const uint64_t d = gbcast64<G>(diff, grp, fl);
            return n + 8 * fl + (ctz64(d) >> 3);
        }
        n += 8 * active;
        if (active < G) break;
    }
    const int tail = left - n;
    for (int k0 = 0; k0 < tail; k0 += G) {
        const int k = k0 + lig;
        const bool ne = k < tail && base[a + n + k] != base[b + n + k];
        const uint32_t m = gballot<G>(ne, grp);
        if (m) return n + k0 + __builtin_ctz(m);
    }
    return n + tail;
}
template <int G>
__device__ __forceinline__ int grp_backlen(const uint8_t* __restrict__ base, int s, int t, int kmax, int lig, int grp) {
    int cnt = 0;
    while (cnt < kmax) {
        const int k = cnt + lig + 1;
        bool ne = true;
        if (k <= kmax) ne = base[t - k] != base[s - k];
        const uint32_t m = gballot<G>(ne, grp);
        const int c = m ? __builtin_ctz(m) : G;
        cnt += c;
        if (c < G) break;
    }
    return cnt < kmax ? cnt : kmax;
}


struct KcBlkMeta {
    uint32_t nseq;
    uint32_t nlit;
    uint32_t extra_lits;
    uint32_t flags;
    uint32_t o1_in, o2_in;
    uint32_t o1_out, o2_out;
};
#define KC_BF_POP_A 1u
#define KC_BF_FORCED 2u
```

compress_amd/csrc/kc_host.h:

```cpp
#pragma once
#include <hip/hip_runtime.h>
#include <stdint.h>
#include <stdio.h>
#include <stdlib.h>
#include <string.h>
#include <atomic>
#include <chrono>
#include <condition_variable>
#include <functional>
#include <memory>
#include <mutex>
#include <string>
#include <thread>
#include <vector>
#include <algorithm>

#include "../../include/kcgpu.h"
#include "kc_kernels.h"


namespace kci {

const int kMinWindowSize = 1 << 10;
const int kMaxWindowSize = 1 << 29;
const int kMaxCompressedBlockSize = 128 << 10;

struct DevBuf {
    void* p = nullptr;
    size_t cap = 0;
};

struct Pending {
    kc_zstd_opts o;
    KcMatchParams mp;
    KcEntropyParams ep;
    std::vector<uint64_t> unit_off;
    uint32_t n_units = 0;
    uint8_t* d_dst = nullptr;
    uint64_t need = 0;
    bool fed = false;
    int bs = 0;
    bool k2prof = false;
};


static const uint64_t KC_MAX_UNIT_BYTES = (uint64_t)1 << 30;

struct ChunkFeed {
    std::vector<uint32_t> cut;
    std::vector<hipEvent_t> landed;
    std::vector<hipEvent_t> done;
    std::vector<hipStream_t> streams;
    std::function<bool(size_t)> wait_recorded;
    uint64_t* loc_off = nullptr;
};

struct Plan {
    uint32_t n_units = 0, n_blocks = 0;
    std::vector<uint32_t> blk0;
    std::vector<uint64_t> stage_off;
    std::vector<uint32_t> blk_start, unit_flags;
    std::vector<uint64_t> stage64;
    std::vector<uint64_t> rel_off;
    uint32_t seq_stride = 0, lit_stride = 0;
    uint64_t max_unit_bytes = 0;
};

}
using namespace kci;

struct KcCfg {
    int64_t match_path = KC_PATH_AUTO;
    int64_t zfast_lds_max_units = 768;
    int64_t s2_lds_max_blocks = 1280;
    int64_t spec_w0 = -1, spec_grow = -1;
    int64_t lds_spec_w0 = 16;
    int64_t s2_lds_spec_w0 = 0;
    int64_t host_serial = 0, host_pipe_mib = 0, host_overlap_min_mib = -1, host_copy_threads = 0, host_trace = 0;
    int64_t host_roll = 1;
    int64_t host_roll_mib = 0;
    std::vector<uint64_t> host_chunks;
    int64_t k2_prof = 0;
    int64_t hook_wait_us = 0, hook_batch = 256, hook_lanes = 4;
    int64_t hook_host_first = -1;
    int64_t test_feed_redo = 0;
    int64_t better_dict_epoch = 0;
    int64_t s2_variant = 0;
    int64_t best_slots = 6144;
    int64_t zfast_epoch = 1;
    int64_t zfast_xseg_k = 0;
    int64_t zfast_variant = -1;
    int64_t zfast_filter = 1;
    int64_t xxh_fin_mode = 1;
    int64_t zfast_prescan = -1;
    int64_t job_prime = 1;
    int64_t dstream_blocks = 512;
    int64_t fuse_raw_xxh = 1;
};

struct kc_ctx {
    KcCfg cfg;
    int device = 0;
    hipStream_t stream = nullptr;
    uint32_t s2_pend_n = 0;
    bool lane_preclear = false;
    hipEvent_t ev_preclear = nullptr;
    void* preclear_ptr = nullptr;
    size_t preclear_bytes = 0;
    hipStream_t stream2 = nullptr;
    bool own_stream = false;
    std::string err;
    bool oom = false;
    hipDeviceProp_t prop;
    DevBuf blk_start, unit_flags, redo_blk, pop_blk;
    DevBuf unit_off, unit_blk0, stage_off, seqs, aux, lits, meta, stage, out_size, xxh, redo, popmask, unit_list, out_off,
        predef, errflag, tmp_src, tmp_dst, tables, prof, work, work_off, dictbuf, proto, dicthuf;
    bool predef_ready = false;
    int tab_owner = 0;
    int tab_pb = 0;
    uint32_t tab_units = 0, tab_ep = 0, better_epoch_now = 0, fast_epoch_now = 0;
    void* tab_ptr = nullptr;
    uint64_t proto_key = 0;
    void* proto_ptr = nullptr;
    void* dictbuf_ptr = nullptr;
    DevBuf best_tables, best_cur, best_cost;
    uint32_t best_n = 0;
    hipEvent_t ev[8] = {nullptr, nullptr, nullptr, nullptr, nullptr, nullptr, nullptr, nullptr};
    kc_timings last = {0, 0, 0, 0, 0, 0};
    size_t max_batch_bytes = (size_t)8 << 30;
    uint64_t max_scratch_bytes = (uint64_t)160 << 30;
    int stream_mode = 0;
    std::thread job;
    bool job_active = false;
    kc_status job_status = KC_OK;
    const uint64_t* cut_off = nullptr;
    const uint64_t* cuts = nullptr;
    uint32_t cut_unit0 = 0;
    const uint32_t* job_hist = nullptr;
    const uint32_t* job_flags = nullptr;
    const uint8_t* job_tables = nullptr;
    bool job_primed = false;
    DevBuf d_job_hist, d_job_flags, rawdef, unit_raw;
    DevBuf zd[20];
    DevBuf s2d[13];
    DevBuf unit_done, probe_rel;
    int probe_bs = 0;
    uint32_t probe_n = 0;
    bool prescan_ran = false;
    int64_t last_prescan_units = 0;
    std::vector<uint32_t> job_redo_list;
    void* pend = nullptr;
    kc_ctx* chain_after = nullptr;
    void* hpipe = nullptr;
    Plan plan;
    std::once_flag hook_once;
    void* hook = nullptr;
    bool ev7_valid = false;
    int last_batches = 0;
    int last_path = 0;
    bool last_incompressible = false;
    std::vector<uint8_t> up_unit_off, up_blk0, up_stage_off;
    const void* up_ptr[3] = {nullptr, nullptr, nullptr};
};

#define KC_S2_MAX_BLOCK ((uint64_t)1 << 30)
#define KC_S2_MAX_FRAMED_BLOCK ((uint64_t)4 << 20)

struct kc_s2_ropts {
    uint32_t max_block = (uint32_t)KC_S2_MAX_FRAMED_BLOCK;
    int ignore_crc = 0;
    int ignore_id = 0;
};

struct kc_zstd_dopts {
    uint64_t max_memory = (uint64_t)64 << 30;
    uint64_t max_window = (uint64_t)1 << 29;
    int ignore_checksum = 0;
    std::vector<KcZdDict> dicts;
    std::vector<uint8_t> arena;
};

namespace kci {

#define HIPCHK(ctx, call)                                                                              \
    do {                                                                                               \
        hipError_t e__ = (call);                                                                       \
        if (e__ != hipSuccess) {                                                                       \
            (ctx)->err = std::string(#call) + ": " + hipGetErrorString(e__);                            \
            return KC_ERR_HIP;                                                                         \
        }                                                                                              \
    } while (0)

inline kc_status ensure(kc_ctx* c, DevBuf& b, size_t bytes) {
    if (b.cap >= bytes) return KC_OK;
    if (b.p) HIPCHK(c, hipFree(b.p));
    b.p = nullptr;
    b.cap = 0;
    size_t want = bytes + (bytes >> 3) + 256;
    hipError_t e = hipMalloc(&b.p, want);
    if (e == hipErrorOutOfMemory) {
        (void)hipGetLastError();
        want = bytes + 256;
        e = hipMalloc(&b.p, want);
    }
    if (e != hipSuccess) {
        (void)hipGetLastError();
        b.p = nullptr;
        if (e == hipErrorOutOfMemory) {
            c->err = "device memory exhausted (" + std::to_string(want >> 20) + " MiB of scratch wanted)";
            c->oom = true;
            return KC_ERR_UNSUPPORTED;
        }
        c->err = std::string("hipMalloc: ") + hipGetErrorString(e);
        return KC_ERR_HIP;
    }
    b.cap = want;
    return KC_OK;
}

inline kc_status tables_claim(kc_ctx* c, hipStream_t st) {
    if (c->preclear_bytes != 0) {
        c->preclear_bytes = 0;
        HIPCHK(c, hipStreamWaitEvent(st, c->ev_preclear, 0));
    }
    return KC_OK;
}

inline int bitsLen32(uint32_t v) { return v == 0 ? 0 : 32 - __builtin_clz(v); }

void s2_hook_free(void* h);
void host_pipe_free(void* h);

}
using namespace kci;

namespace kci {
kc_status check_supported(kc_ctx* c, const kc_zstd_opts* o);
size_t match_table_bytes(int level);
kc_status launch_match(kc_ctx* c, const KcMatchParams& mp, const uint64_t* unit_off, uint32_t n_units, uint32_t n_launch, int bs, hipStream_t st, int level);
uint32_t plan_stream_blocks(uint64_t bs, uint64_t len, const uint64_t* cuts, uint64_t n_cuts, std::vector<uint32_t>* starts, uint32_t* flags);
kc_status batch_begin(kc_ctx* c, const kc_zstd_opts* o, const uint8_t* d_src_base, const uint64_t* unit_off, uint32_t n_units,
                      uint8_t* d_dst, uint64_t dst_cap, ChunkFeed* feed = nullptr);
kc_status batch_end(kc_ctx* c, uint64_t* out_off_host, uint64_t* produced);
uint64_t zstd_unit_scratch(const kc_zstd_opts* o, uint64_t len, uint64_t n_cuts = 0);
uint64_t scratch_budget(kc_ctx* c);
kc_status feed_finish(kc_ctx* c, bool* redo_needed);
kc_status run_batch(kc_ctx* c, const kc_zstd_opts* o, const uint8_t* d_src_base, const uint64_t* unit_off, uint32_t n_units,
                    uint8_t* d_dst, uint64_t dst_cap, uint64_t* out_off_host, uint64_t* produced);
kc_status validate_units(kc_ctx* c, const kc_zstd_opts* o, const uint64_t* unit_off, uint32_t n_units);
typedef std::function<kc_status(kc_ctx* lane, const uint8_t* d_in, const uint64_t* rel_off, uint32_t n, uint8_t* d_out, uint64_t cap, uint64_t* out_off_rel)> RollEncFn;
kc_status host_rolling(kc_ctx* c, const uint8_t* src, const uint64_t* unit_off, uint32_t n_units, uint8_t* dst, uint64_t dst_cap,
                       uint64_t* out_off, const RollEncFn& enc, const std::function<uint64_t(uint64_t)>& max_out, uint64_t sub_bytes = 0);
uint64_t host_roll_sub_bytes(const kc_ctx* c, uint64_t total);
kc_status host_roll_trim(int device);
}
int kc_dict_load_decoder(const uint8_t* blob, uint64_t len, KcZdDict* D, const uint8_t** content, uint64_t* content_len);
```

compress_amd/csrc/kc_kernels.h:

```cpp
#pragma once
#include <hip/hip_runtime.h>
#include <stdint.h>
#include "kc_dev.h"

struct KcMatchParams {
    const uint8_t* src;
    const uint8_t* src_end;
    const uint64_t* unit_off;
    const uint32_t* unit_blk0;
    uint64_t* seqs;
    KcBlkMeta* meta;
    const uint32_t* blk_start;
    const uint32_t* unit_flags;
    const uint8_t* pop_blk;
    const uint32_t* unit_list;
    uint32_t unit_base;
    uint32_t seq_stride;
    int32_t block_size;
    int32_t max_match_off;
    int32_t spec_w0;
    int32_t spec_grow;
    int32_t hist0;
    int32_t pos_bits;
    int32_t rep1, rep2;
    int32_t rep3;
    int32_t stream_mode;
    const uint32_t* unit_hist;
    const uint32_t* job_flags;
    unsigned long long* prof;
    uint32_t epoch;
    const uint8_t* proto;
    int32_t lds_any_big;
    int32_t lds_split;
    int32_t empty_filter;
    int32_t tuned;
    const uint32_t* unit_done;
    int32_t xseg_k;
};
void kc_launch_zfast_match_grp(const KcMatchParams& P, uint32_t* tables, uint32_t n_launch, hipStream_t st);
static inline size_t kc_zfast_table_bytes() { return (size_t)4 << 15; }
#define KC_ZF_EPOCH_BITS 4
void kc_launch_zfast_match_lds(const KcMatchParams& P, const uint32_t* proto, uint32_t proto_stride, uint32_t n_launch, hipStream_t st);
#define KC_ZFAST_LDS_MAX_UNIT ((1u << 26) - 4u)
void kc_launch_zdfast_match_grp(const KcMatchParams& P, uint32_t* tables, uint32_t n_launch, hipStream_t st);
static inline size_t kc_zdfast_table_bytes() { return ((size_t)4 << 17) + ((size_t)4 << 15); }
void kc_launch_zbetter_match_grp(const KcMatchParams& P, uint8_t* tables, uint32_t n_launch, bool dict, hipStream_t st);
static inline size_t kc_zbetter_table_bytes() { return ((size_t)8 << 19) + ((size_t)4 << 13); }
void kc_launch_zbest_match(const KcMatchParams& P, uint64_t* tables, uint32_t* slot_cur, const int32_t* cost, uint32_t n_launch, uint32_t n_slots,
                           hipStream_t st);
void kc_launch_zbest_cost(const void* d_predef, int32_t* d_cost, hipStream_t st);
static inline size_t kc_zbest_table_bytes() { return ((size_t)8 << 22) + ((size_t)8 << 18); }

struct KcRawDef {
    uint32_t frame_pos;
    uint32_t src_pos;
    uint32_t size;
    uint32_t pad;
};

struct KcFsePredef;
struct KcEntropyParams {
    const uint8_t* src;
    const uint64_t* unit_off;
    const uint32_t* unit_blk0;
    const uint64_t* seqs;
    const KcBlkMeta* meta;
    uint8_t* lits;
    uint64_t* aux;
    uint8_t* stage;
    const uint64_t* stage_off;
    uint32_t* out_size;
    const uint64_t* xxh;
    uint32_t* redo_mask;
    uint8_t* redo_blk;
    const uint32_t* blk_start;
    const uint32_t* unit_flags;
    const uint32_t* unit_list;
    uint32_t unit_base;
    const void* predef;
    uint32_t seq_stride;
    uint32_t lit_stride;
    int32_t block_size;
    int32_t window_size;
    int32_t crc, single, no_entropy, all_lit_entropy, full_zero;
    uint32_t dict_id;
    int32_t hist0;
    const uint32_t* unit_hist;
    const uint32_t* job_flags;
    const uint8_t* dict_huf;
    int32_t dict_huf_len, dict_huf_log;
    int32_t stream_mode;
    int32_t stream_sync;
    uint32_t* unit_raw;
    KcRawDef* rawdef;
    uint32_t* err_flag;
    unsigned long long* prof;
    const uint32_t* unit_done;
};
size_t kc_fse_predef_bytes();
void kc_launch_fse_predef_init(void* d_predef, hipStream_t st);
void kc_launch_zstd_entropy(const KcEntropyParams& P, uint32_t grid, hipStream_t st);

struct KcPrescanParams {
    const uint8_t* src;
    const uint64_t* unit_off;
    const uint32_t* unit_blk0;
    uint32_t n_units;
    int32_t block_size;
    const uint32_t* probe_rel;
    uint32_t n_probe;
    int32_t rep1, rep2;
    KcBlkMeta* meta;
    uint32_t* unit_done;
    uint8_t* stage;
    const uint64_t* stage_off;
    uint32_t* out_size;
    KcRawDef* rawdef;
    uint32_t* unit_raw;
    int32_t window_size, crc, single;
    uint32_t dict_id;
};
#define KC_PRESCAN_MAX_KEYS 1024
void kc_launch_zfast_prescan(const KcPrescanParams& P, hipStream_t st);
uint32_t kc_zfast_probe_positions(int block_size, uint32_t* rel, uint32_t cap);

struct KcPrimeParams {
    const uint8_t* src;
    const uint64_t* unit_off;
    const uint32_t* unit_hist;
    const uint32_t* unit_list;
    uint32_t unit_base;
    uint32_t n_launch;
    int32_t level;
    int32_t pos_bits;
    uint8_t* tables;
    size_t table_bytes;
};
void kc_launch_zstd_prime(const KcPrimeParams& P, hipStream_t st);

struct KcS2Params {
    const uint8_t* src;
    const uint64_t* blk_off;
    const uint64_t* stage_off;
    uint8_t* stage;
    uint32_t* out_size;
    uint32_t* tables;
    uint32_t table_stride;
    uint32_t n_blocks;
    int32_t level;
    int32_t spec_w0, spec_w0b;
    int32_t spec_grow;
    int32_t framed;
    int32_t stored_only;
    int32_t variant;
};
void kc_launch_s2_encode(const KcS2Params& P, hipStream_t st);
void kc_launch_s2_best(const KcS2Params& P, hipStream_t st);
void kc_launch_s2_encode_lds(const KcS2Params& P, bool any_small, bool any_big, hipStream_t st);
struct KcS2DecParams {
    const uint8_t* enc;
    const uint64_t* enc_off;
    uint8_t* dst;
    const uint64_t* dst_off;
    uint32_t* status;
    uint32_t n_blocks;
};
void kc_launch_s2_decode(const KcS2DecParams& P, hipStream_t st);
struct KcZstdDecParams {
    const uint8_t* enc;
    const uint64_t* enc_off;
    uint8_t* dst;
    const uint64_t* dst_off;
    uint8_t* lits;
    uint32_t lit_stride;
    uint32_t* status;
    uint32_t* crc_stored;
    uint32_t* has_crc;
    uint32_t n_units;
    const uint8_t* dict;
    uint32_t dict_len;
};
void kc_launch_zstd_decode(const KcZstdDecParams& P, hipStream_t st);
enum { KCZD_OK = 0, KCZD_MAGIC = 1, KCZD_EOF = 2, KCZD_UNKNOWN_DICT = 3, KCZD_WINDOW = 4, KCZD_SIZE = 5, KCZD_CRC = 6, KCZD_CORRUPT = 7 };
#define KC_ZD_NO_SIZE 0xFFFFFFFFFFFFFFFFull
#define KC_ZD_MAX_FRAME 0xFFFFFF00ull
#define KC_ZD_LIT_STRIDE ((128u << 10) + 64u)
struct KcZdCell { uint16_t base; uint8_t sym; uint8_t nb; };
struct KcZdDict {
    uint32_t id, content_len;
    uint64_t content_off;
    uint32_t rep[3];
    uint32_t full;
    int32_t huf_log, ll_log, of_log, ml_log;
    uint16_t huf[1 << 11];
    KcZdCell ll[1 << 9], of[1 << 8], ml[1 << 9];
};
struct KcZdFrame {
    uint64_t blk_begin, blk_end;
    uint64_t window;
    uint64_t fcs;
    uint64_t slot_off;
    uint32_t slot_cap;
    uint32_t dict;
    uint32_t checksum;
    uint32_t input;
};
struct KcZdPlanParams {
    const uint8_t* src;
    const uint64_t* in_off;
    uint32_t n;
    uint64_t max_memory, max_window;
    const KcZdDict* dicts;
    uint32_t n_dicts;
    uint32_t* n_frames;
    uint64_t* bound;
    uint64_t* slot_bytes;
    uint32_t* exact;
    uint32_t* status;
    const uint32_t* frame0;
    const uint64_t* slot0;
    KcZdFrame* frames;
};
void kc_launch_zstd_plan(const KcZdPlanParams& P, hipStream_t st);
struct KcZdDecodeParams {
    const uint8_t* src;
    const KcZdFrame* frames;
    uint32_t n_frames;
    uint8_t* stage;
    uint8_t* lits;
    const KcZdDict* dicts;
    const uint8_t* dict_arena;
    uint64_t max_memory;
    uint32_t* out_size;
    uint32_t* status;
    uint32_t* crc_stored;
    uint64_t* hash_off;
};
void kc_launch_zstd_decode_all(const KcZdDecodeParams& P, hipStream_t st);
#define KC_ZS_OWN 0xFFFFFFFFu
#define KC_ZS_CARRIED 0xFFFFFFFEu
#define KC_ZS_NO_OFF 0xFFFFFFFFFFFFFFFFull
enum { KC_ZS_HUF = 0, KC_ZS_LL = 1, KC_ZS_OF = 2, KC_ZS_ML = 3 };
struct KcZsBlock {
    uint64_t pos;
    uint32_t size;
    uint32_t type;
    uint32_t parsed;
    uint32_t ltype, regen, comp, lhdr;
    uint32_t nseq, shdr, modes;
    uint32_t src[4];
    uint32_t def;
    uint32_t wt_bytes;
    uint64_t wt_off;
    uint64_t lit_off;
    uint64_t seq_off;
};
struct KcZsTables {
    uint16_t huf[1 << 11];
    KcZdCell ll[1 << 9], of[1 << 9], ml[1 << 9];
    int32_t huf_log, huf_ok;
    int32_t log[3], ok[3];
    uint32_t rep[3];
    uint32_t pad;
};
struct KcZsHash {
    uint64_t v[4];
    uint64_t total;
    uint64_t digest;
    uint32_t tail_n;
    uint8_t tail[32];
};
struct KcZsEntropyParams {
    const uint8_t* in;
    uint64_t in_len;
    const KcZsBlock* blocks;
    uint32_t n_blocks;
    uint64_t window;
    uint8_t* lits;
    uint64_t lits_len;
    uint32_t* seqs;
    uint64_t seqs_len;
    uint8_t* wts;
    const KcZsTables* cur;
    KcZsTables* next;
    uint32_t* status;
};
struct KcZsExecParams {
    const uint8_t* in;
    const KcZsBlock* blocks;
    uint32_t n_blocks;
    uint64_t window;
    const uint8_t* lits;
    const uint32_t* seqs;
    const uint32_t* estatus;
    uint8_t* hist;
    uint64_t hist_pos, hist_cap;
    const uint8_t* dict;
    uint32_t dict_len;
    uint32_t def_mask;
    const KcZsTables* cur;
    KcZsTables* next;
    uint32_t* out_size;
    uint32_t* status;
    uint64_t* result;
};
struct KcZsHashParams {
    const uint8_t* hist;
    uint64_t start;
    const uint64_t* result;
    KcZsHash* h;
    int final;
};
void kc_launch_zstd_dstream_entropy(const KcZsEntropyParams& P, hipStream_t st);
void kc_launch_zstd_dstream_execute(const KcZsExecParams& P, hipStream_t st);
void kc_launch_xxh64_stream(const KcZsHashParams& P, hipStream_t st);
enum { KCS2D_OK = 0, KCS2D_CORRUPT = 1, KCS2D_CRC = 2, KCS2D_UNSUPPORTED = 3, KCS2D_SIZE = 4, KCS2D_EOF = 5, KCS2D_UNEXPECTED_EOF = 6 };
#define KC_S2C_STORED 1u
#define KC_S2C_NOCRC 2u
struct KcS2Chunk {
    uint64_t body_off;
    uint64_t out_off;
    uint32_t body_len;
    uint32_t dlen;
    uint32_t crc;
    uint32_t kind;
    uint32_t stream, index;
};
struct KcS2PlanParams {
    const uint8_t* src;
    const uint64_t* in_off;
    uint32_t n;
    uint32_t max_block;
    uint32_t max_buf;
    int32_t ignore_id;
    int32_t blocks;
    uint32_t* n_chunks;
    uint64_t* bound;
    uint32_t* status;
    const uint32_t* chunk0;
    const uint64_t* out0;
    KcS2Chunk* chunks;
};
void kc_launch_s2_plan(const KcS2PlanParams& P, hipStream_t st);
struct KcS2DecodeAllParams {
    const uint8_t* src;
    const KcS2Chunk* chunks;
    uint32_t n_chunks;
    uint8_t* dst;
    int32_t ignore_crc;
    uint32_t* status;
};
void kc_launch_s2_decode_all(const KcS2DecodeAllParams& P, hipStream_t st);
#define KC_S2R_MID 1u
#define KC_S2R_SNAPPY 2u
#define KC_S2R_KNOWN 4u
#define KC_S2R_NO_SLOT (~0ull)
struct KcS2Req {
    uint64_t front, end;
    uint64_t pos;
    uint64_t u;
    uint64_t off, len;
    uint64_t out0;
    uint64_t slot0;
    uint32_t chunk0;
    uint32_t flags;
};
struct KcS2ReqPlan {
    uint64_t got;
    uint64_t slot_bytes;
    uint32_t n_chunks;
    uint32_t status;
};
struct KcS2RChunk {
    KcS2Chunk c;
    uint64_t slot_off;
    uint32_t clip_lo, clip_hi;
};
struct KcS2RangePlanParams {
    const uint8_t* src;
    KcS2Req* reqs;
    uint32_t m;
    uint32_t max_block, max_buf;
    int32_t ignore_id;
    KcS2ReqPlan* plan;
    KcS2RChunk* chunks;
};
void kc_launch_s2_range_plan(const KcS2RangePlanParams& P, hipStream_t st);
struct KcS2RangeDecodeParams {
    const uint8_t* src;
    const KcS2RChunk* chunks;
    uint32_t n_chunks;
    uint8_t* dst;
    uint8_t* slots;
    int32_t ignore_crc;
    uint32_t* status;
};
void kc_launch_s2_range_decode(const KcS2RangeDecodeParams& P, hipStream_t st);
static inline size_t kc_s2_table_bytes(int level, uint64_t max_block_len, int variant = 0) {
    if (variant == 1 && level == 1 && max_block_len >= ((uint64_t)16 << 10)) return ((size_t)4 << 17) + ((size_t)4 << 14);
    if (variant == 1 && level == 3) return max_block_len > ((uint64_t)64 << 10) ? (((size_t)4 << 17) + ((size_t)4 << 14)) : (((size_t)4 << 16) + ((size_t)4 << 13));
    if (level >= 4) return ((size_t)8 << 19) + ((size_t)8 << 16);
    if (level == 3) return max_block_len > ((uint64_t)64 << 10) ? (((size_t)4 << 16) + ((size_t)4 << 14)) : (((size_t)4 << 15) + ((size_t)4 << 13));
    if (level != 1) return (size_t)4 << 14;
    return max_block_len > ((uint64_t)64 << 10) ? (((size_t)4 << 17) + ((size_t)4 << 14)) : (((size_t)4 << 16) + ((size_t)4 << 13));
// ... 29 lines not shown
```

compress_amd/csrc/kc_zstd_entropy.hip:

```cpp
#include "kc_dev.h"
#include "kc_kernels.h"
#include "kc_fse_dev.h"
#include "kc_huf_dev.h"
#include "kc_frame_dev.h"

#define ET 256
#ifndef SEQ_CHUNK
#define SEQ_CHUNK 1024
#endif
#ifndef KC_PACK_REUSE
#define KC_PACK_REUSE 1
#endif
#ifndef KC_HCOPIES
#define KC_HCOPIES 2
#endif
#ifndef KC_K2_WGS
#define KC_K2_WGS 4
#endif
#ifndef KC_CHAIN_WARM
#define KC_CHAIN_WARM 48
#endif
#define CH_PAD 16
#define CH_SEG 16
#define CH_WB (KC_CHAIN_WARM / CH_SEG)
static_assert(KC_CHAIN_WARM % CH_SEG == 0 && CH_WB >= 1 && CH_WB <= 3, "warm-up is whole segments");
static_assert(SEQ_CHUNK % CH_SEG == 0 && SEQ_CHUNK / CH_SEG <= 64, "one segment per lane");
#define LONG_RUN 32

static_assert(sizeof(KcFsePredefBlob) == 3 * sizeof(KcFseT), "blob layout");
size_t kc_fse_predef_bytes() { return sizeof(KcFsePredefBlob); }

__global__ void kc_fse_predef_init_kernel(KcFsePredefBlob* B) {
    __shared__ uint8_t tsym[3][256];
    __shared__ int16_t cumul[3][66];
    const int i = threadIdx.x;
    if (i >= 3) return;
    const int16_t llNorm[36] = {4, 3, 2, 2, 2, 2, 2, 2, 2, 2, 2, 2, 2, 1, 1, 1, 2, 2, 2, 2, 2, 2, 2, 2, 2, 3, 2, 1, 1, 1, 1, 1, -1, -1, -1, -1};
    const int16_t ofNorm[29] = {1, 1, 1, 1, 1, 1, 2, 2, 2, 1, 1, 1, 1, 1, 1, 1, 1, 1, 1, 1, 1, 1, 1, 1, -1, -1, -1, -1, -1};
    const int16_t mlNorm[53] = {1, 4, 3, 2, 2, 2, 2, 2, 2, 1, 1, 1, 1, 1, 1, 1, 1, 1, 1, 1, 1, 1, 1, 1, 1, 1, 1, 1, 1, 1, 1, 1,
                                1, 1, 1, 1, 1, 1, 1, 1, 1, 1, 1, 1, 1, 1, -1, -1, -1, -1, -1, -1, -1};
    KcFseT* f = &B->t[i];
    for (int k = 0; k < 64; k++) { f->norm[k] = 0; f->dnb[k] = 0; f->dfs[k] = 0; f->outBits[k] = 0; }
    for (int k = 0; k < 256; k++) f->st[k] = 0;
    if (i == 0) { for (int k = 0; k < 36; k++) f->norm[k] = llNorm[k]; f->symbolLen = 36; f->tableLog = 6; }
    if (i == 1) { for (int k = 0; k < 29; k++) f->norm[k] = ofNorm[k]; f->symbolLen = 29; f->tableLog = 5; }
    if (i == 2) { for (int k = 0; k < 53; k++) f->norm[k] = mlNorm[k]; f->symbolLen = 53; f->tableLog = 6; }
    f->useRLE = 0; f->rleVal = 0; f->reUsed = 0; f->stLen1 = 0;
    fse_build_core<int16_t>(f->norm, f->symbolLen, f->tableLog, tsym[i], cumul[i], f->st, f->dnb, f->dfs);
    for (int k = 0; k < (int)f->symbolLen; k++)
        f->outBits[k] = (uint8_t)(i == 0 ? kc_ll_bits(k) : (i == 1 ? (uint32_t)k : kc_ml_bits(k)));
    f->preDefined = 1;
}
void kc_launch_fse_predef_init(void* d_predef, hipStream_t st) {
    hipLaunchKernelGGL(kc_fse_predef_init_kernel, dim3(1), dim3(64), 0, st, (KcFsePredefBlob*)d_predef);
}

__device__ __forceinline__ uint64_t wave_incl_scan64(uint64_t v, int lane) {
    const uint32_t lo = wave_incl_scan((uint32_t)v, lane), hi = wave_incl_scan((uint32_t)(v >> 32), lane);
    return ((uint64_t)hi << 32) | lo;
}
__device__ __forceinline__ uint64_t block_excl_scan64(uint64_t v, uint64_t* wsum, uint64_t* total, int tid) {
    const int lane = tid & 63, w = tid >> 6;
    const uint64_t inc = wave_incl_scan64(v, lane);
    __syncthreads();
    if (lane == 63) wsum[w] = inc;
    __syncthreads();
    uint64_t base = 0;
    for (int k = 0; k < w; k++) base += wsum[k];
    *total = wsum[0] + wsum[1] + wsum[2] + wsum[3];
    return base + inc - v;
}

__device__ __forceinline__ uint32_t wave_approx_size(const KcFseT* f, const uint32_t* hist, int histLen, int lane) {
    if ((int)f->symbolLen < histLen) return 0xFFFFFFFFu;
    if (f->useRLE) return 0xFFFFFFFFu;
    const uint32_t kAccuracyLog = 8;
    const uint32_t badCost = ((uint32_t)f->tableLog + 1) << kAccuracyLog;
    uint32_t term = 0;
    bool bad = false;
    if (lane < histLen) {
        const uint32_t v = hist[lane];
        if (v != 0) {
            if (f->norm[lane] == 0) bad = true;
            else {
                const uint32_t minNbBits = f->dnb[lane] >> 16;
                const uint32_t threshold = (minNbBits + 1) << 16;
                const uint32_t tableSize = 1u << f->tableLog;
                const uint32_t deltaFromThreshold = threshold - (f->dnb[lane] + tableSize);
                const uint32_t normalizedDelta = (deltaFromThreshold << kAccuracyLog) >> f->tableLog;
                const uint32_t bc = (minNbBits + 1) * (1u << kAccuracyLog) - normalizedDelta;
                if (bc > badCost) bad = true;
                term = v * bc;
            }
        }
    }
    if (__ballot(bad) != 0ull) return 0xFFFFFFFFu;
    return wave_reduce_sum(term) >> kAccuracyLog;
}

struct HufState {
    KcHufTable prev;
    int prevLen;
    uint8_t prevLog;
    int reuse;
};

struct Shared {
    uint32_t whist[4 * KC_HCOPIES][256];
    uint32_t cnt[256];
    KcHufNodes nodes;
    KcHufTable cur;
    HufState huf;
    uint8_t weights[256];
    KcWeightFse wfse;
    KcHufWaveTmp hwt;
    uint8_t tdesc[192];
    KcFseT fse[9];
    uint8_t curIdx[3], prevIdx[3];
    uint8_t useIdx[3];
    uint32_t shist[3][64];
    uint32_t smax[3];
    uint8_t tsym[3][256];
    int16_t cumul[3][66];
    int16_t posx[3][66];
    uint8_t seqhdr[224];
    uint32_t asz[3][3];
    uint8_t nc[3][72];
    int ncLen[3];
    uint8_t seqMode;
    int seqhdrLen;
    alignas(16) uint8_t codes[3][CH_PAD + SEQ_CHUNK + 16];
    alignas(16) uint16_t sbits[3][CH_PAD + SEQ_CHUNK + 16];
    uint32_t cpk[3][64];
    uint16_t state[3];
    uint64_t wsum[4];
    uint32_t wtot[4];
    int ivar[24];
    unsigned long long profAcc[24];
};

enum { IV_SYMLEN = 0, IV_MAXCNT, IV_CANREUSE, IV_LITMODE, IV_USEPREV, IV_TABLOG, IV_DESCLEN, IV_DATALEN, IV_LITSEC,
       IV_OK, IV_SEQBYTES, IV_RAW, IV_TMP0, IV_TMP1 };

__device__ __forceinline__ int lit_header_size1(int regenLen) {
    const int inBits = bits_len32((uint32_t)regenLen);
    return inBits < 5 ? 1 : (inBits < 12 ? 2 : 3);
}
__device__ __forceinline__ int put_lit_header1(uint8_t* p, uint32_t type, int regenLen) {
    const int inBits = bits_len32((uint32_t)regenLen);
    uint64_t lh = type;
    int sz;
    if (inBits < 5) { lh |= ((uint64_t)regenLen << 3); sz = 1; }
    else if (inBits < 12) { lh |= (1 << 2) | ((uint64_t)regenLen << 4); sz = 2; }
    else { lh |= (3 << 2) | ((uint64_t)regenLen << 4); sz = 3; }
    for (int i = 0; i < sz; i++) p[i] = (uint8_t)(lh >> (8 * i));
    return sz;
}
__device__ __forceinline__ int lit_header_size2(int compLen, int inLen) {
    const int compBits = bits_len32((uint32_t)compLen), inBits = bits_len32((uint32_t)inLen);
    if (compBits <= 10 && inBits <= 10) return 3;
    if (compBits <= 14 && inBits <= 14) return 4;
    return 5;
}
__device__ __forceinline__ int put_lit_header2(uint8_t* p, uint32_t type, int compLen, int inLen, bool single) {
    const int compBits = bits_len32((uint32_t)compLen), inBits = bits_len32((uint32_t)inLen);
    uint64_t lh = type;
    int sz;
    if (compBits <= 10 && inBits <= 10) {
        if (!single) lh |= 1 << 2;
        lh |= ((uint64_t)inLen << 4) | ((uint64_t)compLen << (10 + 4));
        sz = 3;
    } else if (compBits <= 14 && inBits <= 14) {
        lh |= (2 << 2) | ((uint64_t)inLen << 4) | ((uint64_t)compLen << (14 + 4));
        sz = 4;
    } else {
        lh |= (3 << 2) | ((uint64_t)inLen << 4) | ((uint64_t)compLen << (18 + 4));
        sz = 5;
    }
    for (int i = 0; i < sz; i++) p[i] = (uint8_t)(lh >> (8 * i));
    return sz;
}

__device__ __forceinline__ void wg_copy(uint8_t* __restrict__ dst, const uint8_t* __restrict__ src, int n) {
    const int tid = threadIdx.x;
    const int n4 = n >> 2;
    if ((((uintptr_t)dst) & 3) == 0) {
        for (int i = tid; i < n4; i += ET) ((uint32_t*)dst)[i] = ld32(src + 4 * i);
        for (int i = (n4 << 2) + tid; i < n; i += ET) dst[i] = src[i];
    } else {
        for (int i = tid; i < n; i += ET) dst[i] = src[i];
    }
}

__device__ __forceinline__ void or_bits(uint32_t* words, uint64_t bitpos, uint64_t value, int nbits) {
    if (nbits == 0) return;
    const uint32_t w = (uint32_t)(bitpos >> 5);
    const int sh = (int)(bitpos & 31);
    const uint64_t lo = value << sh;
    atomicOr(&words[w], (uint32_t)lo);
    if (sh + nbits > 32) atomicOr(&words[w + 1], (uint32_t)(lo >> 32));
    if (sh + nbits > 64) atomicOr(&words[w + 2], (uint32_t)(value >> (64 - sh)));
}

__device__ __forceinline__ void lds_or_bits(uint32_t* words, uint64_t bitpos, uint64_t value, int nbits) {
    if (nbits == 0) return;
    const uint32_t w = (uint32_t)(bitpos >> 5);
    const int sh = (int)(bitpos & 31);
    const uint64_t lo = value << sh;
    atomicOr(&words[w], (uint32_t)lo);
    if (sh + nbits > 32) atomicOr(&words[w + 1], (uint32_t)(lo >> 32));
    if (sh + nbits > 64) atomicOr(&words[w + 2], (uint32_t)(value >> (64 - sh)));
}

__device__ __forceinline__ uint32_t huf_lane_bits(const uint8_t* __restrict__ seg, int segLen, const KcHufTable* T, int lane, int chunk) {
    uint32_t bits = 0;
    const int r0 = lane * chunk;
    int r1 = r0 + chunk;
    if (r1 > segLen) r1 = segLen;
    int p = segLen - 1 - r0;
    const int lo = segLen - r1;
    for (; p - 15 >= lo; p -= 16) {
        const uint64_t v = ld64(seg + p - 7), v2 = ld64(seg + p - 15);
#pragma unroll
        for (int b = 7; b >= 0; b--) bits += T->nb[(uint32_t)(v >> (8 * b)) & 0xFFu];
#pragma unroll
        for (int b = 7; b >= 0; b--) bits += T->nb[(uint32_t)(v2 >> (8 * b)) & 0xFFu];
    }
    for (; p - 7 >= lo; p -= 8) {
        const uint64_t v = ld64(seg + p - 7);
#pragma unroll
        for (int b = 7; b >= 0; b--) bits += T->nb[(uint32_t)(v >> (8 * b)) & 0xFFu];
    }
    for (; p >= lo; p--) bits += T->nb[seg[p]];
    return bits;
}
__device__ __forceinline__ void huf_lane_emit(const uint8_t* __restrict__ seg, int segLen, const KcHufTable* T, int lane, int chunk,
                                              uint32_t* words, uint64_t bitpos) {
    const int r0 = lane * chunk;
    int r1 = r0 + chunk;
    if (r1 > segLen) r1 = segLen;
    uint32_t* wp = words + (bitpos >> 5);
    uint64_t acc = 0;
    int nb = (int)(bitpos & 31);
    bool firstWord = true;
    auto put = [&](uint32_t sym) {
        acc |= (uint64_t)T->val[sym] << nb;
        nb += T->nb[sym];
        if (nb >= 32) {
            if (firstWord) { atomicOr(wp, (uint32_t)acc); firstWord = false; }
            else *wp = (uint32_t)acc;
            wp++;
            acc >>= 32;
            nb -= 32;
        }
    };
    int p = segLen - 1 - r0;
    const int lo = segLen - r1;
    for (; p - 15 >= lo; p -= 16) {
        const uint64_t v = ld64(seg + p - 7), v2 = ld64(seg + p - 15);
#pragma unroll
        for (int b = 7; b >= 0; b--) put((uint32_t)(v >> (8 * b)) & 0xFFu);
#pragma unroll
        for (int b = 7; b >= 0; b--) put((uint32_t)(v2 >> (8 * b)) & 0xFFu);
    }
    for (; p - 7 >= lo; p -= 8) {
        const uint64_t v = ld64(seg + p - 7);
#pragma unroll
        for (int b = 7; b >= 0; b--) put((uint32_t)(v >> (8 * b)) & 0xFFu);
    }
    for (; p >= lo; p--) put(seg[p]);
    if (nb > 0 && (uint32_t)acc != 0u) atomicOr(wp, (uint32_t)acc);
}

template <bool EMIT>
__device__ __forceinline__ uint32_t chain_seg16(uint32_t st, const uint32_t (&pk)[CH_SEG], int cnt, const uint16_t* __restrict__ tbl, uint32_t (&sbp)[CH_SEG / 2]) {
    uint32_t out = st;
#pragma unroll
    for (int q = 0; q < CH_SEG; q++) {
        const uint32_t w = pk[q];
        const uint32_t t = (st << 12) + w;
        const uint32_t nb = t >> 28;
        const char* pb = (const char*)tbl + (((int32_t)(w << 20)) >> 19);
        if (EMIT) {
            const uint32_t v = (nb << 12) | (st & ((1u << nb) - 1u));
            if (q & 1) sbp[q >> 1] |= v << 16; else sbp[q >> 1] = v;
        }
        st = *(const uint16_t*)(pb + ((st >> nb) << 1));
        if (q + 1 == cnt) out = st;
    }
    return cnt >= CH_SEG ? st : out;
}
__device__ __forceinline__ void chain_load16(const uint8_t* __restrict__ cod, const uint32_t* __restrict__ cpk, uint32_t (&pk)[CH_SEG]) {
    const uint4 c4 = *(const uint4*)cod;
    const uint32_t cw[4] = {c4.x, c4.y, c4.z, c4.w};
#pragma unroll
    for (int q = 0; q < CH_SEG; q++) pk[q] = cpk[(cw[q >> 2] >> (8 * (q & 3))) & 0xFFu];
}

__global__ __launch_bounds__(ET, KC_K2_WGS) void kc_zstd_entropy_kernel(KcEntropyParams P) {
    __shared__ Shared S;
#ifdef KC_K2_PAD
    __shared__ uint32_t padLds[KC_K2_PAD / 4];
    if (P.block_size == -12345) padLds[threadIdx.x] = 1;
#endif
    const int tid = (int)threadIdx.x, lane = tid & 63, wv = tid >> 6;
    const uint32_t u = P.unit_list ? P.unit_list[blockIdx.x] : P.unit_base + blockIdx.x;
    if (P.unit_done != nullptr && P.unit_done[u] != 0u) return;
    const uint8_t* __restrict__ base = P.src + P.unit_off[u];
    const int hist0 = P.unit_hist != nullptr ? (int)P.unit_hist[u] : P.hist0;
    const bool JOB = P.job_flags != nullptr;
    const bool finalJob = JOB && (P.job_flags[u] & 1u) != 0;
    const int ulen = (int)(P.unit_off[u + 1] - P.unit_off[u]) - hist0;
    const uint32_t blk0 = P.unit_blk0[u];
    const int bs = P.block_size;
    const KcUnitBlocks UB = kc_unit_blocks(P.blk_start, P.unit_flags, P.unit_blk0, u, ulen, bs, P.stream_mode);
    const int nblk = UB.nblk;
    uint8_t* __restrict__ outp = P.stage + P.stage_off[u];
    const bool rawAllLits = !P.all_lit_entropy;
    const bool noEntropy = P.no_entropy != 0;

    {
        const uint32_t* pb = (const uint32_t*)P.predef;
        uint32_t* dstp = (uint32_t*)&S.fse[6];
        for (int i = tid; i < (int)(sizeof(KcFsePredefBlob) / 4); i += ET) dstp[i] = pb[i];
        if (tid < 6) {
            KcFseT* f = &S.fse[tid];
            f->symbolLen = 0; f->tableLog = 0; f->useRLE = 0; f->rleVal = 0; f->reUsed = 0; f->preDefined = 0; f->stLen1 = 0;
        }
        if (tid == 0) {
            for (int k = 0; k < 3; k++) { S.curIdx[k] = (uint8_t)(2 * k); S.prevIdx[k] = (uint8_t)(2 * k + 1); }
            S.huf.prevLen = 0;
            S.huf.prevLog = 0;
            S.huf.reuse = 2;
        }
    }
    int opos = 0;
    long long pt0 = 0;
#define PROF_MARK(i) do { if (P.prof && tid == 0) { const long long t1__ = clock64(); S.profAcc[i] += (unsigned long long)(t1__ - pt0); pt0 = t1__; } } while (0)
    if (P.prof && tid == 0) for (int i = 0; i < 24; i++) S.profAcc[i] = 0;
    if (P.prof && tid == 0) pt0 = clock64();
#ifdef KC_K2_FINE
    long long pf0 = 0;
#define PROF_FINE(i) do { if (P.prof && tid == 0) { __builtin_amdgcn_s_waitcnt(0); const long long t1__ = clock64(); S.profAcc[16 + (i)] += (unsigned long long)(t1__ - pf0); pf0 = t1__; } } while (0)
#define PROF_FINE0() do { if (P.prof && tid == 0) { __builtin_amdgcn_s_waitcnt(0); pf0 = clock64(); } } while (0)
#else
#define PROF_FINE(i) do { } while (0)
#define PROF_FINE0() do { } while (0)
#endif
#if defined(KC_K2_FINE) && KC_K2_FINE == 2
#define PROF_FINB(i) do { if (P.prof && tid == 0) { __builtin_amdgcn_s_waitcnt(0); const long long t1__ = clock64(); S.profAcc[16 + (i)] += (unsigned long long)(t1__ - pf0); pf0 = t1__; } } while (0)
#define PROF_FINB0() do { if (P.prof && tid == 0) { __builtin_amdgcn_s_waitcnt(0); pf0 = clock64(); } } while (0)
#undef PROF_FINE
#undef PROF_FINE0
#define PROF_FINE(i) do { } while (0)
#define PROF_FINE0() do { } while (0)
#else
#define PROF_FINB(i) do { } while (0)
#define PROF_FINB0() do { } while (0)
#endif
    const bool streamU = UB.streamU;
    if (ulen > 0 && !JOB) {
        uint8_t hdr[16];
        const int h = kc_frame_header(hdr, ulen, P.window_size, P.single, P.crc, P.dict_id, streamU);
        if (tid == 0) for (int i = 0; i < h; i++) outp[i] = hdr[i];
        opos = h;
    }
    __syncthreads();
    if (ulen == 0 && JOB) {
        if (tid == 0) {
            if (finalJob) { outp[0] = 0x01; outp[1] = 0x00; outp[2] = 0x00; }
            P.out_size[u] = finalJob ? 3u : 0u;
        }
        return;
    }
    if (ulen == 0) {
        if (tid == 0) {
            if (P.full_zero && P.stream_mode) {
                int h = 0;
                outp[h++] = 0x28; outp[h++] = 0xb5; outp[h++] = 0x2f; outp[h++] = 0xfd;
                uint8_t fhd = P.crc ? (1 << 2) : 0;
                const uint32_t did = P.dict_id;
                int didLen = 0;
                if (did > 0) { if (did < 256) { fhd |= 1; didLen = 1; } else if (did < (1u << 16)) { fhd |= 2; didLen = 2; } else { fhd |= 3; didLen = 4; } }
                outp[h++] = fhd;
                outp[h++] = (uint8_t)((bits_len32((uint32_t)P.window_size - 1) - 10) << 3);
                for (int i = 0; i < didLen; i++) outp[h++] = (uint8_t)(did >> (8 * i));
                outp[h++] = 0x01; outp[h++] = 0x00; outp[h++] = 0x00;
                if (P.crc) { outp[h++] = 0x99; outp[h++] = 0xe9; outp[h++] = 0xd8; outp[h++] = 0x51; }
                P.out_size[u] = (uint32_t)h;
            } else if (P.full_zero) {
                const uint8_t z[9] = {0x28, 0xb5, 0x2f, 0xfd, 0x20, 0x00, 0x01, 0x00, 0x00};
                for (int i = 0; i < 9; i++) outp[i] = z[i];
                P.out_size[u] = 9;
            } else {
                P.out_size[u] = 0;
            }
        }
        return;
    }

    int nRawDef = 0;
    for (int b = 0; b < nblk; b++) {
        const KcBlkMeta m = P.meta[blk0 + (uint32_t)b];
        const int blkStart = hist0 + kc_blk_begin(P.blk_start, blk0, b, bs);
        const int blkEnd = hist0 + kc_blk_end(P.blk_start, blk0, b, nblk, bs, ulen);
        const int size = blkEnd - blkStart;
        const bool last = JOB ? (b == nblk - 1 && finalJob) : (b == nblk - 1 && !UB.emptyLast);
        const uint8_t* __restrict__ org = base + blkStart;
        const uint64_t* __restrict__ sq = P.seqs + (size_t)(blk0 + (uint32_t)b) * P.seq_stride;
        uint8_t* __restrict__ lits = P.lits + (size_t)(blk0 + (uint32_t)b) * P.lit_stride;
        uint32_t* __restrict__ auxw = (uint32_t*)(P.aux + (size_t)(blk0 + (uint32_t)b) * P.seq_stride);
        const int nseq = (int)m.nseq;
        const int nlit = (int)m.nlit;
        uint8_t* bout = outp + opos;
        if (P.rawdef != nullptr && tid == 0) P.rawdef[blk0 + (uint32_t)b].size = 0;
        auto raw_payload = [&]() {
            if (P.rawdef != nullptr) {
                nRawDef++;
                if (tid == 0) {
                    KcRawDef r;
                    r.frame_pos = (uint32_t)(opos + 3); r.src_pos = (uint32_t)blkStart; r.size = (uint32_t)size; r.pad = 0;
                    P.rawdef[blk0 + (uint32_t)b] = r;
                }
            } else {
                wg_copy(bout + 3, org, size);
            }
        };

        bool litsOnly = false;
        if (nseq == 0) {
            litsOnly = true;
        } else {
            const uint64_t s0 = sq[0];
            if (nseq == 1 && nlit <= 1 && (int)seq_ll(s0) == nlit && seq_of(s0) - 3u == 1u) {
                if (tid == 0) {
                    put_block_header(bout, last, 1u, seq_ml(s0) + 3u + seq_ll(s0));
                    bout[3] = org[0];
                }
                opos += 4;
                __syncthreads();
                continue;
            }
            if (m.flags & KC_BF_POP_A) litsOnly = true;
        }
        const bool dictLit = b == 0 && P.dict_huf != nullptr && !(streamU && P.stream_sync);
        if (litsOnly && (rawAllLits || size < (dictLit ? 8 : 32))) {
            if (tid == 0) put_block_header(bout, last, 0u, (uint32_t)size);
            raw_payload();
            opos += 3 + size;
            __syncthreads();
            continue;
        }
        const uint8_t* __restrict__ L = litsOnly ? org : lits;
        const int nlitE = litsOnly ? size : nlit;

        PROF_MARK(0);
        for (int i = tid; i < 4 * KC_HCOPIES * 256; i += ET) ((uint32_t*)S.whist)[i] = 0;
        if (!litsOnly) for (int i = tid; i < (int)((sizeof(S.codes) + sizeof(S.sbits)) / 16); i += ET) ((uint4*)&S.codes[0][0])[i] = make_uint4(0, 0, 0, 0);
        if (!litsOnly) {
            for (int i = tid; i < 3 * 64; i += ET) ((uint32_t*)S.shist)[i] = 0;
            if (tid < 3) S.smax[tid] = 0;
        }
        __syncthreads();
        if (litsOnly) {
            for (int k = tid; k < size; k += ET) atomicAdd(&S.whist[wv * KC_HCOPIES + (lane & (KC_HCOPIES - 1))][org[k]], 1u);
        } else
        {
            uint8_t* __restrict__ tile = &S.codes[0][0];
            constexpr int TWB = 2304;
            constexpr int TWC = 2048;
            static_assert(sizeof(S.codes) + sizeof(S.sbits) >= 4 * TWB, "four gather windows");
            uint8_t* __restrict__ tw = tile + wv * TWB;
            const uint8_t* __restrict__ bsrc = base + blkStart;
            const int per = (((nseq + 3) >> 2) + 63) & ~63;
            const int q0 = wv * per < nseq ? wv * per : nseq;
            const int q1 = q0 + per < nseq ? q0 + per : nseq;
            PROF_FINE0();
            {
                uint64_t acc = 0;
                uint32_t mll = 0, mof = 0, mml = 0;
                for (int i0 = q0 + lane; i0 < q1; i0 += 8 * 64) {
                    uint64_t sv[8];
#pragma unroll
                    for (int r = 0; r < 8; r++) sv[r] = i0 + 64 * r < q1 ? sq[i0 + 64 * r] : 0ull;
#pragma unroll
                    for (int r = 0; r < 8; r++) {
                        if (i0 + 64 * r < q1) {
                            const uint32_t ll = seq_ll(sv[r]), ml = seq_ml(sv[r]), of = seq_of(sv[r]);
                            acc += (uint64_t)ll | ((uint64_t)(ll + ml + 3u) << 32);
                            const uint32_t cl = kc_ll_code(ll), co = kc_of_code(of), cm = kc_ml_code(ml);
                            atomicAdd(&S.shist[0][cl], 1u);
                            atomicAdd(&S.shist[1][co], 1u);
                            atomicAdd(&S.shist[2][cm], 1u);
                            mll = cl > mll ? cl : mll;
                            mof = co > mof ? co : mof;
                            mml = cm > mml ? cm : mml;
                        }
                    }
                }
                mll = wave_reduce_max(mll); mof = wave_reduce_max(mof); mml = wave_reduce_max(mml);
                const uint64_t tot = wave_incl_scan64(acc, lane);
                if (lane == 63) S.wsum[wv] = tot;
                if (lane == 0) { atomicMax(&S.smax[0], mll); atomicMax(&S.smax[1], mof); atomicMax(&S.smax[2], mml); }
            }
            PROF_FINE(0);
            __syncthreads();
            PROF_FINE(1);
            uint64_t run = 0;
            for (int k = 0; k < wv; k++) run += S.wsum[k];
            const uint32_t firstLo = (uint32_t)run;
            const uint32_t fw = firstLo & ~15u;
            const uint32_t hs = firstLo & 15u;
            struct GStep { uint32_t ll, lo, sp; uint64_t tot, longMask; };
            auto place = [&](uint64_t sx, bool have, uint64_t at, GStep& g) {
                uint32_t ll = 0, adv = 0;
                if (have) { ll = seq_ll(sx); adv = ll + seq_ml(sx) + 3u; }
                const uint64_t v = (uint64_t)ll | ((uint64_t)adv << 32);
                const uint64_t inc = wave_incl_scan64(v, lane);
                g.tot = bcast64(inc, 63);
                const uint64_t ex = inc - v + at;
                g.ll = ll; g.lo = (uint32_t)ex; g.sp = (uint32_t)(ex >> 32);
                g.longMask = ballot64(ll > LONG_RUN);
            };
            auto fetch = [&](const GStep& g, uint64_t (&vv)[4]) {
#pragma unroll
                for (int kk = 0; kk < 4; kk++) {
                    const uint32_t k = 8u * (uint32_t)kk;
                    vv[kk] = 0;
                    if (g.ll <= LONG_RUN && k < g.ll) {
                        const uint32_t n8 = g.ll - k < 8u ? g.ll - k : 8u;
                        if ((int)(g.sp + k) + 8 <= size) vv[kk] = ld64(bsrc + g.sp + k);
                        else { uint64_t t = 0; for (uint32_t q = 0; q < n8; q++) t |= (uint64_t)bsrc[g.sp + k + q] << (8 * q); vv[kk] = t; }
                    }
                }
            };
            GStep cur;
            uint64_t vv[4];
            uint64_t sq1 = q0 + lane < q1 ? sq[q0 + lane] : 0ull;
            for (int t0 = q0; t0 < q1; t0 += 64) {
                const int i = t0 + lane;
                place(sq1, i < q1, run, cur);
                sq1 = i + 64 < q1 ? sq[i + 64] : 0ull;
                PROF_FINE(2);
                fetch(cur, vv);
                const uint32_t ll = cur.ll, lo = cur.lo, sp = cur.sp;
                const uint64_t tot = cur.tot, longMask = cur.longMask;
                const bool mine = ll > 0 && ll <= LONG_RUN;
                const uint32_t begLo = (uint32_t)run;
                const uint32_t endLo = begLo + (uint32_t)tot;
                for (uint32_t winBase = begLo & ~15u; winBase < endLo; winBase += TWC) {
                    if (mine && lo < winBase + TWC && lo + ll > winBase) {
#pragma unroll
                        for (int kk = 0; kk < 4; kk++) {
                            const uint32_t k = 8u * (uint32_t)kk;
                            if (k < ll) {
                                const uint32_t n8 = ll - k < 8u ? ll - k : 8u;
                                const uint64_t x = n8 < 8u ? vv[kk] & ((1ull << (8u * n8)) - 1ull) : vv[kk];
                                const uint32_t o = lo + k - winBase;
                                if (lo + k >= winBase && o + n8 <= (uint32_t)TWC) {
                                    unsigned long long* pq = (unsigned long long*)(tw + (o & ~7u));
                                    const uint32_t sh = (o & 7u) * 8u;
                                    atomicOr(pq, (unsigned long long)(x << sh));
                                    if (sh != 0u && (x >> (64u - sh)) != 0ull) atomicOr(pq + 1, (unsigned long long)(x >> (64u - sh)));
                                } else {
                                    for (uint32_t q = 0; q < n8; q++) {
                                        const uint32_t oo = lo + k + q - winBase;
                                        if (oo < (uint32_t)TWC) atomicOr((uint32_t*)(tw + (oo & ~3u)), (uint32_t)((x >> (8u * q)) & 0xFFu) << (8u * (oo & 3u)));
                                    }
                                }
                            }
                        }
                    }
                    for (uint64_t lm = longMask; lm != 0ull; lm &= lm - 1ull) {
                        const int e = ctz64(lm);
                        const uint32_t lsp = bcast32(sp, e), llo = bcast32(lo, e), lln = bcast32(ll, e);
                        const uint32_t o0 = llo > winBase ? llo : winBase;
                        const uint32_t o1 = llo + lln < winBase + TWC ? llo + lln : winBase + TWC;
                        for (uint32_t o = o0 + 4u * (uint32_t)lane; o < o1; o += 4u * 64u) {
                            const uint32_t n4 = o1 - o < 4u ? o1 - o : 4u;
                            const uint32_t si = lsp + (o - llo);
                            uint32_t x;
                            if ((int)si + 4 <= size) x = ld32(bsrc + si);
                            else { x = 0; for (uint32_t q = 0; q < n4; q++) x |= (uint32_t)bsrc[si + q] << (8u * q); }
                            if (n4 < 4u) x &= (1u << (8u * n4)) - 1u;
                            const uint32_t oo = o - winBase;
                            unsigned long long* pq = (unsigned long long*)(tw + (oo & ~7u));
                            const uint32_t sh = (oo & 7u) * 8u;
                            atomicOr(pq, (unsigned long long)x << sh);
                            if (sh > 32u && (x >> (64u - sh)) != 0u) atomicOr(pq + 1, (unsigned long long)(x >> (64u - sh)));
                        }
                    }
                    KC_WAVE_SYNC();
                    PROF_FINE(3);
                    const uint32_t wEnd = endLo < winBase + TWC ? endLo : winBase + TWC;
                    const uint32_t nfull = (wEnd - winBase) >> 4;
                    const bool shared0 = hs != 0u && winBase == fw && nfull > 0u;
                    if (shared0 && (uint32_t)lane >= hs && lane < 16) { const uint8_t c = tw[lane]; lits[fw + lane] = c; atomicAdd(&S.whist[wv * KC_HCOPIES][c], 1u); }
                    for (uint32_t w = (shared0 ? 1u : 0u) + (uint32_t)lane; w < nfull; w += 64u) ((uint4*)(lits + winBase))[w] = ((const uint4*)tw)[w];
                    for (uint32_t d = (shared0 ? 4u : 0u) + (uint32_t)lane; d < 4u * nfull; d += 64u) {
                        const uint32_t x = ((const uint32_t*)tw)[d];
                        uint32_t* const hc = S.whist[wv * KC_HCOPIES + (lane & (KC_HCOPIES - 1))];
                        atomicAdd(&hc[x & 0xFFu], 1u);
                        atomicAdd(&hc[(x >> 8) & 0xFFu], 1u);
                        atomicAdd(&hc[(x >> 16) & 0xFFu], 1u);
                        atomicAdd(&hc[x >> 24], 1u);
                    }
                    const uint32_t tail = (wEnd - winBase) & 15u;
                    uint8_t carry = 0;
                    if (nfull > 0u && lane < (int)tail) carry = tw[(nfull << 4) + lane];
                    KC_WAVE_SYNC();
                    PROF_FINE(4);
                    if (nfull > 0u) {
                        for (uint32_t w = 1u + (uint32_t)lane; w <= nfull; w += 64u) ((uint4*)tw)[w] = make_uint4(0, 0, 0, 0);
                        if (lane < 16) tw[lane] = carry;
                    }
                    KC_WAVE_SYNC();
                    PROF_FINE(5);
                }
                run += tot;
            }
            {
                const uint32_t total = (uint32_t)run;
                const uint32_t rem = total & 15u;
                const uint32_t lowT = ((total & ~15u) == fw) ? hs : 0u;
                if ((uint32_t)lane >= lowT && (uint32_t)lane < rem) { const uint8_t c = tw[lane]; lits[(total & ~15u) + lane] = c; atomicAdd(&S.whist[wv * KC_HCOPIES][c], 1u); }
            }
            {
                const uint32_t len = m.extra_lits, spos = (uint32_t)size - len, lo = (uint32_t)nlit - len;
                for (uint32_t k = tid; k < len; k += ET) {
                    const uint8_t c = bsrc[spos + k];
                    lits[lo + k] = c;
                    atomicAdd(&S.whist[wv * KC_HCOPIES][c], 1u);
                }
            }
            PROF_FINE(6);
        }
        __syncthreads();
        PROF_FINE(7);
        {
            uint32_t c = 0;
#pragma unroll
            for (int k = 0; k < 4 * KC_HCOPIES; k++) c += S.whist[k][tid];
            S.cnt[tid] = c;
            const uint32_t wm = wave_reduce_max(c);
            const uint32_t wl = wave_reduce_max(c ? (uint32_t)tid + 1u : 0u);
            if (lane == 0) { S.wtot[wv] = wm; S.wsum[wv] = wl; }
        }
        __syncthreads();

        PROF_MARK(1);
        auto seq_build = [&](int k) {
            KcFseT* f = &S.fse[S.curIdx[k]];
            int doBuild = 0;
            if (lane == 0) {
                const int maxSym = (int)S.smax[k];
                uint32_t maxCount = 0;
                for (int i = 0; i <= maxSym; i++) if (S.shist[k][i] > maxCount) maxCount = S.shist[k][i];
                f->symbolLen = (uint16_t)(maxSym + 1);
                if (!f->reUsed) {
                    f->tableLog = fse_optimal_table_log(nseq, f->symbolLen);
                    f->stLen1 = 0;
                    if ((int)maxCount == nseq) {
                        f->useRLE = 1;
                    } else {
                        f->useRLE = 0;
                        if (fse_normalize_core(S.shist[k], f->norm, f->symbolLen, nseq, f->tableLog)) doBuild = 1;
                        else atomicExch(P.err_flag, 2u);
                    }
                }
            }
            doBuild = __shfl(doBuild, 0, 64);
            if (doBuild) {
                if (!fse_build_wave(f->norm, f->symbolLen, f->tableLog, S.tsym[k], S.cumul[k], S.posx[k], f->st, f->dnb, f->dfs, lane)) {
                    if (lane == 0) atomicExch(P.err_flag, 2u);
                }
            }
        };
        bool seqHistDone = !litsOnly, seqBuildDone = false;
        const bool wantHuf = litsOnly ? (nlitE > 16) : (!noEntropy && nlitE > 16);
        const bool four = nlitE >= 1024;
        if (tid == 0) {
            int litMode = 0;
            uint32_t maxCount = 0, symbolLen = 0;
            for (int k = 0; k < 4; k++) { if (S.wtot[k] > maxCount) maxCount = S.wtot[k]; if ((uint32_t)S.wsum[k] > symbolLen) symbolLen = (uint32_t)S.wsum[k]; }
            S.ivar[IV_SYMLEN] = (int)symbolLen;
            S.ivar[IV_MAXCNT] = (int)maxCount;
            S.ivar[IV_OK] = 0;
            if (dictLit) {
                const uint16_t* dv = (const uint16_t*)P.dict_huf;
                const uint8_t* dn = P.dict_huf + 512;
                for (int k = 0; k < P.dict_huf_len; k++) { S.huf.prev.val[k] = dv[k]; S.huf.prev.nb[k] = dn[k]; }
                S.huf.prevLen = P.dict_huf_len;
                S.huf.prevLog = (uint8_t)P.dict_huf_log;
                S.huf.reuse = 0;
            }
            if (wantHuf) {
                if (S.huf.reuse == 2) S.huf.prevLen = 0;
                if ((int)maxCount >= nlitE) litMode = (nlitE == 1) ? 0 : 1;
                else if (maxCount == 1 || (int)maxCount < (nlitE >> 7)) litMode = 0;
                else S.ivar[IV_OK] = 1;
            }
            S.ivar[IV_LITMODE] = litMode;
        }
        __syncthreads();
        int litSecLen = 0;
        bool single = false;
        if (S.ivar[IV_OK]) {
            const int symbolLen = S.ivar[IV_SYMLEN];
            {
                bool bad = false;
                if (S.huf.prevLen > 0) { if (S.cnt[tid] != 0 && (tid >= S.huf.prevLen || S.huf.prev.nb[tid] == 0)) bad = true; }
                else bad = true;
                const int anyBad = __syncthreads_or(bad ? 1 : 0);
                if (tid == 0) S.ivar[IV_CANREUSE] = anyBad ? 0 : 1;
            }
            PROF_MARK(2);
            if (tid < symbolLen) {
                const uint32_t c = S.cnt[tid];
                int rank = 0;
                for (int j = 0; j < symbolLen; j++) {
                    const uint32_t cj = S.cnt[j];
                    rank += (cj > c || (cj == c && j < tid)) ? 1 : 0;
                }
                S.nodes.count[rank + 1] = c;
                S.nodes.symbol[rank + 1] = (uint8_t)tid;
            }
            __syncthreads();
            if (wv == 0) {
                const uint8_t tl = huf_build_wave(&S.nodes, &S.cur, &S.hwt, symbolLen, nlitE, lane);
                if (lane == 0) {
                    if (tl == 0xFF) atomicExch(P.err_flag, 1u);
                    S.ivar[IV_TABLOG] = tl;
                }
            }
            seqHistDone = !litsOnly;
            __syncthreads();
            PROF_MARK(3);
            {
                const uint32_t c = tid < symbolLen ? S.cnt[tid] : 0u;
                const uint32_t nn = wave_reduce_sum(c * (uint32_t)(tid < symbolLen ? S.cur.nb[tid] : 0));
                const uint32_t no = wave_reduce_sum(c * (uint32_t)((tid < symbolLen && tid < S.huf.prevLen) ? S.huf.prev.nb[tid] : 0));
                if (lane == 0) { S.wtot[wv] = nn; S.wsum[wv] = no; }
            }
            __syncthreads();
            if (wv == 0) {
                const uint32_t newBits = 7 + S.wtot[0] + S.wtot[1] + S.wtot[2] + S.wtot[3];
                const uint32_t oldBits = 7 + (uint32_t)(S.wsum[0] + S.wsum[1] + S.wsum[2] + S.wsum[3]);
                const int newSize = (int)(newBits >> 3), oldSize = (int)(oldBits >> 3);
                const int wantSize = nlitE - (nlitE >> 4);
                int usePrev = 0;
                if (S.huf.reuse == 0 && S.ivar[IV_CANREUSE]) {
                    if (oldSize <= 0 + newSize || 0 + 12 >= wantSize) usePrev = 1;
                }
                int descLen = 0;
                if (!usePrev) {
                    huf_weights_wave(&S.cur, symbolLen, (uint8_t)S.ivar[IV_TABLOG], S.weights, &S.wfse, lane);
                    descLen = huf_write_table(symbolLen, S.weights, &S.wfse, S.tdesc, (int)sizeof(S.tdesc), lane);
                }
                if (lane == 0) {
                    S.ivar[IV_USEPREV] = usePrev;
                    S.ivar[IV_DESCLEN] = descLen;
                }
            }
            if (wv >= 1 && seqHistDone) seq_build(wv - 1);
            seqBuildDone = seqHistDone;
            __syncthreads();
            const bool usePrev = S.ivar[IV_USEPREV] != 0;
            const KcHufTable* T = usePrev ? &S.huf.prev : &S.cur;
            const int descLen = S.ivar[IV_DESCLEN];
            PROF_MARK(4);
            const int nstreams = four ? 4 : 1;
            const int segSize = four ? (nlitE + 3) / 4 : nlitE;
            int segStart = 0, segLen = 0, chunk = 1;
            uint32_t laneBits = 0, laneOff = 0, streamBits = 0;
            if (wv < nstreams && descLen >= 0) {
                segStart = wv * segSize;
                segLen = nlitE - segStart;
                if (segLen > segSize) segLen = segSize;
                if (segLen < 0) segLen = 0;
                chunk = (segLen + 63) / 64;
                if (chunk < 1) chunk = 1;
                PROF_FINB0();
                laneBits = huf_lane_bits(L + segStart, segLen, T, lane, chunk);
                PROF_FINB(0);
                const uint32_t inc = wave_incl_scan(laneBits, lane);
                laneOff = inc - laneBits;
                streamBits = (uint32_t)__shfl((int)inc, 63, 64);
            }
            if (lane == 0) S.wtot[wv] = (wv < nstreams) ? ((streamBits + 1 + 7) >> 3) : 0u;
            __syncthreads();
            if (tid == 0) {
                int litMode = 0;
                int wantSize = nlitE - (nlitE >> 4);
                int dataLen = (int)(S.wtot[0] + S.wtot[1] + S.wtot[2] + S.wtot[3]) + (four ? 6 : 0);
                bool ok = descLen >= 0;
                if (ok && four) for (int k = 0; k < 4; k++) if (S.wtot[k] > 65535u) ok = false;
                int outLen = dataLen + (usePrev ? 0 : descLen);
                if (ok && outLen >= wantSize) ok = false;
                if (ok && !usePrev) {
                    for (int k = 0; k < symbolLen; k++) { S.huf.prev.val[k] = S.cur.val[k]; S.huf.prev.nb[k] = S.cur.nb[k]; }
                    S.huf.prevLen = symbolLen;
                    S.huf.prevLog = (uint8_t)S.ivar[IV_TABLOG];
                }
                if (ok && outLen + 5 > nlitE) {
                    const int szRaw = litsOnly ? 0 : lit_header_size1(nlitE);
                    const int szComp = lit_header_size2(outLen, nlitE);
                    if (outLen + szComp >= nlitE + szRaw) ok = false;
                }
                if (ok) {
                    litMode = usePrev ? 3 : 2;
                    S.huf.reuse = 0;
                }
                S.ivar[IV_LITMODE] = litMode;
                S.ivar[IV_DATALEN] = outLen;
            }
            __syncthreads();
            PROF_MARK(5);
            const int litMode = S.ivar[IV_LITMODE];
            if (litMode >= 2) {
                single = !four;
                const int outLen = S.ivar[IV_DATALEN];
                const int hsz = lit_header_size2(outLen, nlitE);
                const int tabLen = usePrev ? 0 : descLen;
                const uint32_t sb0 = S.wtot[0], sb1 = S.wtot[1], sb2 = S.wtot[2];
                uint32_t myByteOff = (uint32_t)(tabLen + (four ? 6 : 0));
                if (wv >= 1) myByteOff += sb0;
                if (wv >= 2) myByteOff += sb1;
                if (wv >= 3) myByteOff += sb2;
                const int payloadWords = (outLen + 3 + 4) >> 2;
                PROF_FINB0();
                for (int i = tid; i < payloadWords; i += ET) auxw[i] = 0;
                __syncthreads();
                PROF_FINB(1);
                if (wv < nstreams) {
                    const uint64_t bitBase = (uint64_t)myByteOff * 8 + laneOff;
                    huf_lane_emit(L + segStart, segLen, T, lane, chunk, auxw, bitBase);
                    if (lane == 63) or_bits(auxw, (uint64_t)myByteOff * 8 + streamBits, 1, 1);
                }
                PROF_FINB(2);
                __syncthreads();
                PROF_FINB(3);
                uint8_t* lsec = bout + 3;
                wg_copy(lsec + hsz + tabLen + (four ? 6 : 0), (const uint8_t*)auxw + tabLen + (four ? 6 : 0), outLen - tabLen - (four ? 6 : 0));
                if (tid == 0) {
                    put_lit_header2(lsec, litMode == 3 ? 3u : 2u, outLen, nlitE, single);
                    for (int k = 0; k < tabLen; k++) lsec[hsz + k] = S.tdesc[k];
                    if (four) {
                        uint8_t* jt = lsec + hsz + tabLen;
                        jt[0] = (uint8_t)sb0; jt[1] = (uint8_t)(sb0 >> 8);
                        jt[2] = (uint8_t)sb1; jt[3] = (uint8_t)(sb1 >> 8);
                        jt[4] = (uint8_t)sb2; jt[5] = (uint8_t)(sb2 >> 8);
                    }
                }
                litSecLen = hsz + outLen;
                PROF_FINB(4);
            }
        }
        if (litsOnly) {
            const int litMode = S.ivar[IV_LITMODE];
            if (litMode == 0) {
                if (tid == 0) put_block_header(bout, last, 0u, (uint32_t)size);
                raw_payload();
                opos += 3 + size;
            } else if (litMode == 1) {
                if (tid == 0) { put_block_header(bout, last, 1u, (uint32_t)size); bout[3] = org[0]; }
                opos += 4;
            } else {
                if (tid == 0) { put_block_header(bout, last, 2u, (uint32_t)(litSecLen + 1)); bout[3 + litSecLen] = 0; }
                opos += 3 + litSecLen + 1;
            }
            __syncthreads();
            PROF_MARK(6);
            continue;
        }
        {
            const int litMode = S.ivar[IV_LITMODE];
            if (litMode == 0) {
                const int hsz = lit_header_size1(nlit);
                if (tid == 0) put_lit_header1(bout + 3, 0u, nlit);
                wg_copy(bout + 3 + hsz, lits, nlit);
                litSecLen = hsz + nlit;
            } else if (litMode == 1) {
                const int hsz = lit_header_size1(nlit);
                if (tid == 0) { put_lit_header1(bout + 3, 1u, nlit); bout[3 + hsz] = lits[0]; }
                litSecLen = hsz + 1;
            }
        }
        __syncthreads();

        PROF_MARK(6);
        PROF_MARK(7);
        if (!seqBuildDone && wv < 3) seq_build(wv);
        __syncthreads();
        PROF_MARK(8);
        if (wv < 3) {
            const int k = wv;
            const KcFseT* cur = &S.fse[S.curIdx[k]];
            if (!cur->useRLE) {
                const uint32_t* hist = S.shist[k];
                const int histLen = cur->symbolLen;
                const uint32_t v0 = wave_approx_size(cur, hist, histLen, lane);
                const uint32_t v1 = wave_approx_size(&S.fse[6 + k], hist, histLen, lane);
                const uint32_t v2 = wave_approx_size(&S.fse[S.prevIdx[k]], hist, histLen, lane);
                if (lane == 0) { S.asz[k][0] = v0; S.asz[k][1] = v1; S.asz[k][2] = v2; }
            }
        }
        __syncthreads();
        if (tid == 0) {
            uint8_t mode = 0;
            const uint32_t firstCodes[3] = {kc_ll_code(seq_ll(sq[0])), kc_of_code(seq_of(sq[0])), kc_ml_code(seq_ml(sq[0]))};
            const int shifts[3] = {6, 4, 2};
            for (int k = 0; k < 3; k++) {
                KcFseT* cur = &S.fse[S.curIdx[k]];
                int use = S.curIdx[k];
                uint32_t mk;
                if (cur->useRLE) {
                    mk = 1;
                    const uint32_t v = firstCodes[k];
                    cur->tableLog = 0;
                    cur->stLen1 = 1;
                    cur->dfs[v] = 0; cur->dnb[v] = 0; cur->outBits[v] = 0;
                    cur->st[0] = 0;
                    cur->rleVal = (uint8_t)v;
                } else {
                    uint32_t nSize = S.asz[k][0] + fse_max_header_size(cur);
                    const uint32_t predefSize = S.asz[k][1];
                    const uint32_t prevSize = S.asz[k][2];
                    nSize = nSize + ((nSize + 2 * 8 * 16) >> 4);
                    if (predefSize <= prevSize && predefSize <= nSize) { mk = 0; use = 6 + k; }
                    else if (prevSize <= nSize) { mk = 3; use = S.prevIdx[k]; }
                    else mk = 2;
                }
                S.useIdx[k] = (uint8_t)use;
                mode |= (uint8_t)(mk << shifts[k]);
            }
            S.seqMode = mode;
        }
        __syncthreads();
        if (wv < 3) {
            const int k = wv;
            KcFseT* f = &S.fse[S.useIdx[k]];
            if (lane == 0) {
                int n = 0;
                if (f->useRLE) { S.nc[k][0] = f->rleVal; n = 1; }
                else if (!(f->preDefined || f->reUsed)) {
                    n = fse_write_ncount(f->norm, f->symbolLen, f->tableLog, S.nc[k]);
                    if (n < 0) { atomicExch(P.err_flag, 3u); n = 0; }
                }
                S.ncLen[k] = n;
            }
            if (!(f->reUsed || f->preDefined)) {
                if (f->useRLE) {
                    if (lane == 0) { const uint32_t v = f->rleVal; f->outBits[v] = (uint8_t)(k == 0 ? kc_ll_bits(v) : (k == 1 ? v : kc_ml_bits(v))); }
                } else if (lane < (int)f->symbolLen) {
                    f->outBits[lane] = (uint8_t)(k == 0 ? kc_ll_bits((uint32_t)lane) : (k == 1 ? (uint32_t)lane : kc_ml_bits((uint32_t)lane)));
                }
            }
        }
        __syncthreads();
        if (tid == 0) {
            uint8_t* h = S.seqhdr;
            int hp = 0;
            if (nseq < 128) h[hp++] = (uint8_t)nseq;
            else if (nseq < 0x7f00) { h[hp++] = (uint8_t)(128 + (uint8_t)(nseq >> 8)); h[hp++] = (uint8_t)nseq; }
            else { const int n = nseq - 0x7f00; h[hp++] = 255; h[hp++] = (uint8_t)n; h[hp++] = (uint8_t)(n >> 8); }
            h[hp++] = S.seqMode;
            for (int k = 0; k < 3; k++)
                for (int i = 0; i < S.ncLen[k]; i++) h[hp++] = S.nc[k][i];
            S.seqhdrLen = hp;
        }
        __syncthreads();
        const KcFseT* E[3] = {&S.fse[S.useIdx[0]], &S.fse[S.useIdx[1]], &S.fse[S.useIdx[2]]};
        const int seqhdrLen = S.seqhdrLen;
        if (tid < 192) {
            const KcFseT* f = &S.fse[S.useIdx[tid >> 6]];
            const int c = tid & 63;
            S.cpk[tid >> 6][c] = c < (int)f->symbolLen || f->stLen1 ? ((f->dnb[c] << 12) | ((uint32_t)(int32_t)f->dfs[c] & 0xFFFu)) : 0u;
        }
        PROF_MARK(9);
        const int seqBudgetBytes = size - litSecLen - seqhdrLen;
        uint32_t* __restrict__ sw = (uint32_t*)lits;
        uint64_t bitRun = 0;
        uint32_t carry = 0;
        bool overflow = seqBudgetBytes <= 0;
        __syncthreads();
        for (int hiSeq = nseq; hiSeq > 0 && !overflow; hiSeq -= SEQ_CHUNK) {
            const int loSeq = hiSeq - SEQ_CHUNK > 0 ? hiSeq - SEQ_CHUNK : 0;
            const int cn = hiSeq - loSeq;
            const int jb = hiSeq == nseq ? 1 : 0;
            const int nrem = cn - jb;
            const int slot0 = CH_PAD - jb;
            PROF_FINB0();
            constexpr int R = SEQ_CHUNK / ET;
            uint64_t sv[R];
            {
                const int cpad = jb + ((nrem + CH_SEG - 1) & ~(CH_SEG - 1));
#pragma unroll
                for (int r = 0; r < R; r++) { const int j = tid + r * ET; sv[r] = j < cn ? sq[hiSeq - 1 - j] : 0ull; }
                const uint64_t svl = tid < cpad - cn ? sq[loSeq] : 0ull;
#pragma unroll
                for (int r = 0; r < R; r++) {
                    const int j = tid + r * ET;
                    if (j < cn) {
                        S.codes[0][slot0 + j] = (uint8_t)kc_ll_code(seq_ll(sv[r]));
                        S.codes[1][slot0 + j] = (uint8_t)kc_of_code(seq_of(sv[r]));
                        S.codes[2][slot0 + j] = (uint8_t)kc_ml_code(seq_ml(sv[r]));
                    }
                }
                if (tid < cpad - cn) {
                    S.codes[0][slot0 + cn + tid] = (uint8_t)kc_ll_code(seq_ll(svl));
                    S.codes[1][slot0 + cn + tid] = (uint8_t)kc_of_code(seq_of(svl));
                    S.codes[2][slot0 + cn + tid] = (uint8_t)kc_ml_code(seq_ml(svl));
                }
            }
            __syncthreads();
            PROF_FINB(5);
            PROF_MARK(10);
            if (wv < 3) {
                const int k = wv;
                const KcFseT* f = &S.fse[S.useIdx[k]];
                const uint16_t* __restrict__ tbl = f->st;
                const uint32_t* __restrict__ cpk = S.cpk[k];
                const uint8_t* __restrict__ cod = &S.codes[k][CH_PAD];
                const uint32_t trueIn = jb ? (uint32_t)fse_init_state(f, S.codes[k][CH_PAD - 1]) : (uint32_t)S.state[k];
                if (jb && lane == 0) S.sbits[k][CH_PAD - 1] = 0;
                const int nL = (nrem + CH_SEG - 1) / CH_SEG;
                const bool act = lane < nL;
                const int x0 = lane * CH_SEG;
                const int cnt = nrem - x0 < CH_SEG ? nrem - x0 : CH_SEG;
                uint32_t pk[CH_SEG], sbp[CH_SEG / 2];
#pragma unroll
                for (int q = 0; q < CH_SEG / 2; q++) sbp[q] = 0;
                uint32_t st = trueIn, assumed = trueIn, endSt = trueIn;
                if (act) {
                    if (lane > CH_WB) st = tbl[0];
#pragma unroll
                    for (int b = CH_WB; b >= 1; b--) {
                        if (lane >= b) {
                            chain_load16(cod + x0 - b * CH_SEG, cpk, pk);
                            st = chain_seg16<false>(st, pk, CH_SEG, tbl, sbp);
                        }
                    }
                    assumed = st;
                    chain_load16(cod + x0, cpk, pk);
                    endSt = chain_seg16<true>(st, pk, cnt, tbl, sbp);
                }
                for (;;) {
                    uint32_t prevEnd = (uint32_t)__shfl_up((int)endSt, 1, 64);
                    if (lane == 0) prevEnd = trueIn;
                    const unsigned long long bad = __ballot(act && assumed != prevEnd);
                    if (bad == 0ull) break;
#ifdef KC_CHAIN_STATS
                    if (P.prof && lane == 0) { atomicAdd(&P.prof[17], 1ull); atomicAdd(&P.prof[18 + k], 1ull); atomicAdd(&P.prof[24], (unsigned long long)__popcll(bad & ~(bad << 1))); if (f->useRLE) atomicAdd(&P.prof[25], 1ull); }
#endif
                    if ((bad & ~(bad << 1)) >> lane & 1ull) {
                        assumed = prevEnd;
                        endSt = chain_seg16<true>(prevEnd, pk, cnt, tbl, sbp);
                    }
                }
                if (act) {
                    uint4* o = (uint4*)&S.sbits[k][CH_PAD + x0];
                    o[0] = make_uint4(sbp[0], sbp[1], sbp[2], sbp[3]);
                    o[1] = make_uint4(sbp[4], sbp[5], sbp[6], sbp[7]);
                }
#ifdef KC_CHAIN_STATS
                if (P.prof && lane == 0) { atomicAdd(&P.prof[16], 1ull); if (f->useRLE) atomicAdd(&P.prof[26], 1ull); if (f->preDefined) atomicAdd(&P.prof[27], 1ull); }
#endif
                const uint32_t fin = (uint32_t)__shfl((int)endSt, nL > 0 ? nL - 1 : 0, 64);
                if (lane == 0) S.state[k] = (uint16_t)(nL > 0 ? fin : trueIn);
            }
            __syncthreads();
            PROF_FINB(6);
            PROF_MARK(11);
            for (int t0 = 0; t0 < cn; t0 += ET) {
                const int j = t0 + tid;
                uint64_t fv0 = 0, fv1 = 0;
                int fb0 = 0, fb1 = 0;
                if (j < cn) {
#if KC_PACK_REUSE
                    static_assert(R == 4, "the select below is written for four staged sequences per thread");
                    const int rr = t0 / ET;
                    const uint64_t s = rr == 0 ? sv[0] : (rr == 1 ? sv[1] : (rr == 2 ? sv[2] : sv[3]));
#else
                    const uint64_t s = sq[hiSeq - 1 - j];
#endif
                    const uint32_t cl = S.codes[0][slot0 + j], co = S.codes[1][slot0 + j], cm = S.codes[2][slot0 + j];
                    const int lb = E[0]->outBits[cl] & 31, ob = E[1]->outBits[co] & 31, mb = E[2]->outBits[cm] & 31;
                    const uint32_t ll = seq_ll(s), ml = seq_ml(s), of = seq_of(s);
                    const uint64_t lv = ll & (lb ? (0xFFFFFFFFu >> (32 - lb)) : 0u);
                    const uint64_t mv = ml & (mb ? (0xFFFFFFFFu >> (32 - mb)) : 0u);
                    const uint64_t ov = of & (ob ? (0xFFFFFFFFu >> (32 - ob)) : 0u);
                    const uint32_t so = S.sbits[1][slot0 + j], sm = S.sbits[2][slot0 + j], sl = S.sbits[0][slot0 + j];
                    fv0 = (uint64_t)(so & 0xFFF); fb0 = (int)(so >> 12);
                    fv0 |= (uint64_t)(sm & 0xFFF) << fb0; fb0 += (int)(sm >> 12);
                    fv0 |= (uint64_t)(sl & 0xFFF) << fb0; fb0 += (int)(sl >> 12);
                    fv1 = lv | (mv << lb) | (ov << (lb + mb));
                    fb1 = lb + mb + ob;
                }
                uint64_t tot;
                const uint64_t ex = block_excl_scan64((uint64_t)(fb0 + fb1), S.wsum, &tot, tid) + bitRun;
                if ((int64_t)((bitRun + tot + 7) >> 3) >= (int64_t)seqBudgetBytes) { overflow = true; break; }
                uint32_t* __restrict__ pk = (uint32_t*)S.whist;
                const uint32_t wbase = (uint32_t)(bitRun >> 5);
                const int nwords = (int)((((uint32_t)bitRun & 31u) + (uint32_t)tot + 31u) >> 5);
                for (int i = tid; i < nwords + 2; i += ET) pk[i] = i == 0 ? carry : 0u;
                __syncthreads();
                if (j < cn) {
                    const uint64_t rel = ex - ((uint64_t)wbase << 5);
                    lds_or_bits(pk, rel, fv0, fb0);
                    if (fb1 <= 32) lds_or_bits(pk, rel + fb0, fv1, fb1);
                    else { lds_or_bits(pk, rel + fb0, fv1 & 0xFFFFFFFFull, 32); lds_or_bits(pk, rel + fb0 + 32, fv1 >> 32, fb1 - 32); }
                }
                __syncthreads();
                const bool lastPartial = (((uint32_t)bitRun + (uint32_t)tot) & 31u) != 0u;
                const int nstore = lastPartial ? nwords - 1 : nwords;
                for (int i = tid; i < nstore; i += ET) sw[wbase + i] = pk[i];
                carry = lastPartial ? pk[nwords - 1] : 0u;
                bitRun += tot;
            }
            __syncthreads();
            PROF_FINB(7);
        }
        PROF_MARK(12);
        int seqStreamBytes = 0;
        if (!overflow) {
            const int tb = (int)E[2]->tableLog + (int)E[1]->tableLog + (int)E[0]->tableLog + 1;
            if ((int64_t)((bitRun + tb + 7) >> 3) >= (int64_t)seqBudgetBytes) overflow = true;
            else {
                if (tid == 0) {
                    uint64_t bp = bitRun;
                    sw[bitRun >> 5] = carry;
                    sw[(bitRun >> 5) + 1] = 0;
                    const int mlL = E[2]->tableLog, ofL = E[1]->tableLog, llL = E[0]->tableLog;
                    or_bits(sw, bp, (uint64_t)(S.state[2] & ((1u << mlL) - 1u)), mlL); bp += mlL;
                    or_bits(sw, bp, (uint64_t)(S.state[1] & ((1u << ofL) - 1u)), ofL); bp += ofL;
                    or_bits(sw, bp, (uint64_t)(S.state[0] & ((1u << llL) - 1u)), llL); bp += llL;
                    or_bits(sw, bp, 1, 1);
                }
                seqStreamBytes = (int)((bitRun + tb + 7) >> 3);
            }
        }
        __syncthreads();
        const int bodyLen = litSecLen + seqhdrLen + seqStreamBytes;
        if (overflow || bodyLen >= size) {
            __syncthreads();
            if (tid == 0) {
                put_block_header(bout, last, 0u, (uint32_t)size);
                S.huf.reuse = 2;
                if (!last) {
                    if (!(m.flags & KC_BF_FORCED) && (m.o1_out != m.o1_in || m.o2_out != m.o2_in)) { P.redo_blk[blk0 + (uint32_t)b] = 1; atomicOr(&P.redo_mask[u], 1u); }
                }
            }
            raw_payload();
            opos += 3 + size;
            __syncthreads();
            continue;
        }
        if ((m.flags & KC_BF_FORCED) && tid == 0) atomicExch(P.err_flag, 4u);
        wg_copy(bout + 3 + litSecLen + seqhdrLen, (const uint8_t*)sw, seqStreamBytes);
        if (tid == 0) {
            uint8_t* p = bout + 3 + litSecLen;
            for (int k = 0; k < seqhdrLen; k++) p[k] = S.seqhdr[k];
            put_block_header(bout, last, 2u, (uint32_t)bodyLen);
            for (int k = 0; k < 3; k++) {
                const int used = S.useIdx[k];
                if (used == S.curIdx[k]) {
                    const uint8_t t = S.prevIdx[k]; S.prevIdx[k] = S.curIdx[k]; S.curIdx[k] = t;
                    S.fse[S.curIdx[k]].reUsed = 0;
                    S.fse[S.prevIdx[k]].reUsed = 1;
                } else if (used != S.prevIdx[k]) {
                    S.fse[S.prevIdx[k]].symbolLen = 0;
                }
            }
        }
        opos += 3 + bodyLen;
        __syncthreads();
        PROF_MARK(13);
    }

    if (UB.emptyLast && !JOB) {
        if (tid == 0) { outp[opos] = 0x01; outp[opos + 1] = 0x00; outp[opos + 2] = 0x00; }
        opos += 3;
    }
    if (ulen > 0 && P.crc && !JOB) {
        if (tid == 0 && P.xxh != nullptr) {
            const uint64_t h = P.xxh[u];
            outp[opos] = (uint8_t)h; outp[opos + 1] = (uint8_t)(h >> 8); outp[opos + 2] = (uint8_t)(h >> 16); outp[opos + 3] = (uint8_t)(h >> 24);
        }
        opos += 4;
    }
    if (P.prof && tid == 0) {
        for (int i = 0; i < 16; i++) atomicAdd(&P.prof[i], S.profAcc[i]);
        for (int i = 0; i < 8; i++) atomicAdd(&P.prof[40 + i], S.profAcc[16 + i]);
    }
    if (tid == 0) {
        P.out_size[u] = (uint32_t)opos;
        if (P.unit_raw != nullptr) P.unit_raw[u] = (nblk > 0 && nRawDef == nblk && !JOB && hist0 == 0) ? 1u : 0u;
    }
}

void kc_launch_zstd_entropy(const KcEntropyParams& P, uint32_t grid, hipStream_t st) {
    hipLaunchKernelGGL(kc_zstd_entropy_kernel, dim3(grid), dim3(ET), 0, st, P);
}
```

Before: 29120.

## Split literal gather and histograms into a per-block pre-kernel before entropy

Adds a separate litgather kernel that runs one workgroup per 128KiB block (rather than per unit) to gather literals and build the literal and sequence-code histograms. It stores them in a new per-block bhist buffer that the entropy kernel then reads instead of recomputing. This moves the serial per-unit gather work out of the entropy kernel and spreads it across many more workgroups, and it frees the whist LDS space in the entropy kernel. The cost is an extra kernel launch, extra global scratch and traffic for the histograms, and a new event dependency between the two stages.

```diff
diff --git a/compress_amd/csrc/kc_batch.cpp b/compress_amd/csrc/kc_batch.cpp
--- a/compress_amd/csrc/kc_batch.cpp
+++ b/compress_amd/csrc/kc_batch.cpp
@@ -326,6 +326,7 @@
         (s = ensure(c, c->stage_off, (n_units + 1) * 8)) || (s = ensure(c, c->out_off, (n_units + 1 + (feed ? feed->cut.size() : 0)) * 8)) ||
         (s = ensure(c, c->seqs, (size_t)nb * pl.seq_stride * 8)) || (s = ensure(c, c->aux, (size_t)nb * pl.seq_stride * 8)) ||
         (s = ensure(c, c->lits, (size_t)nb * pl.lit_stride)) || (s = ensure(c, c->meta, (size_t)nb * sizeof(KcBlkMeta))) ||
+        (s = ensure(c, c->bhist, (size_t)nb * KC_BH_WORDS * 4)) ||
         (s = ensure(c, c->stage, so + 64)) || (s = ensure(c, c->out_size, (size_t)n_units * 4)) ||
         (s = ensure(c, c->xxh, (size_t)n_units * 8)) || (s = ensure(c, c->redo, (size_t)n_units * 4)) ||
         (s = ensure(c, c->redo_blk, (size_t)nb + 1)) || (s = ensure(c, c->pop_blk, (size_t)nb + 1)) || (s = ensure(c, c->unit_list, (size_t)n_units * 4)) ||
@@ -476,6 +477,10 @@
     ep.seqs = mp.seqs;
     ep.meta = mp.meta;
     ep.lits = (uint8_t*)c->lits.p;
+    ep.bhist = (uint32_t*)c->bhist.p;
+    ep.max_unit_blocks = 0;
+    for (uint32_t i = 0; i < n_units; i++) ep.max_unit_blocks = std::max(ep.max_unit_blocks, pl.blk0[i + 1] - pl.blk0[i]);
+    ep.launch_blocks = 0;
     ep.aux = (uint64_t*)c->aux.p;
     ep.stage = (uint8_t*)c->stage.p;
     ep.stage_off = (const uint64_t*)c->stage_off.p;
@@ -575,10 +580,12 @@
     }
     mp.unit_base = 0;
     ep.unit_base = 0;
+    bool gather_here = false;
     if (feed == nullptr) {
         if (o->crc && !c->job_hist && !fuse_xxh) kc_launch_xxh64(d_src, (const uint64_t*)c->unit_off.p, n_units, (uint64_t*)c->xxh.p, st);
         HIPCHK(c, hipEventRecord(c->ev[1], st));
         if ((s = launch_match(c, mp, unit_off, n_units, n_units, bs, st, o->level)) != KC_OK) return s;
+        gather_here = true;
     } else {
         if (useDict) { c->err = "chunk feed does not take dictionaries"; return KC_ERR_INTERNAL; }
         HIPCHK(c, hipEventRecord(c->ev[1], st));
@@ -608,6 +615,12 @@
         for (size_t k = 0; k < nchunk; k++) HIPCHK(c, hipStreamWaitEvent(st, feed->done[k], 0));
     }
     HIPCHK(c, hipEventRecord(c->ev[2], st));
+    if (gather_here) {
+        KcEntropyParams gp = ep;
+        if ((uint64_t)n_units * ep.max_unit_blocks > 2 * (uint64_t)nb + 64) gp.launch_blocks = nb;
+        kc_launch_zstd_litgather(gp, n_units, st);
+    }
+    HIPCHK(c, hipEventRecord(c->ev[8], st));
     HIPCHK(c, hipGetLastError());
     Pending* P = new Pending();
     P->o = *o;
@@ -631,7 +644,7 @@
     hipStream_t st = c->stream;
     if (c->stream2 != nullptr) {
         st = c->stream2;
-        HIPCHK(c, hipStreamWaitEvent(st, c->ev[2], 0));
+        HIPCHK(c, hipStreamWaitEvent(st, c->ev[8], 0));
     }
     const kc_zstd_opts* o = &P->o;
     KcMatchParams& mp = P->mp;
@@ -642,7 +655,7 @@
     const int bs = P->bs;
     const bool k2prof = P->k2prof;
     kc_status s;
-    kc_launch_zstd_entropy(ep, n_units, st);
+    kc_launch_zstd_entropy(ep, n_units, st, !P->fed);
     HIPCHK(c, hipEventRecord(c->ev[3], st));
     HIPCHK(c, hipGetLastError());
 
@@ -738,8 +751,8 @@
     HIPCHK(c, hipGetLastError());
     float t01 = 0, t12 = 0, t23 = 0, t34 = 0, t45 = 0, t05 = 0, tk2 = 0;
     (void)hipEventElapsedTime(&t01, c->ev[0], c->ev[1]);
-    (void)hipEventElapsedTime(&t12, c->ev[1], c->ev[2]);
-    (void)hipEventElapsedTime(&t23, c->ev[2], c->ev[3]);
+    (void)hipEventElapsedTime(&t12, c->ev[1], c->ev[8]);
+    (void)hipEventElapsedTime(&t23, c->ev[8], c->ev[3]);
     (void)hipEventElapsedTime(&t34, c->ev[3], c->ev[4]);
     (void)hipEventElapsedTime(&t45, c->ev[4], c->ev[5]);
     (void)hipEventElapsedTime(&t05, c->ev[0], c->ev[5]);
@@ -773,7 +786,7 @@
             unsigned long long ft = 0;
             for (int i = 40; i < 48; i++) ft += pv[i];
             if (ft) {
-                fprintf(stderr, "[K2 fine] wave 0, shader clocks per unit; -DKC_K2_FINE=1: gather (pass A, barrier, step: sequences + scan, step: literal loads + ORs, step: flush + histogram, step: carry + zero, tail, closing barrier); =2: (Huffman size pass, payload zero fill + barrier, stream emit, barrier, payload copy + headers, code staging, chains, pack):");
+                fprintf(stderr, "[K2 fine] wave 0, shader clocks per unit; -DKC_K2_FINE=2: (Huffman size pass, payload zero fill + barrier, stream emit, barrier, payload copy + headers, code staging, chains, pack):");
                 for (int i = 40; i < 48; i++) fprintf(stderr, " %.0f", (double)pv[i] / (double)(n_units ? n_units : 1));
                 fprintf(stderr, "\n");
             }
@@ -797,7 +810,7 @@
 uint64_t zstd_unit_scratch(const kc_zstd_opts* o, uint64_t len, uint64_t n_cuts) {
     const uint64_t bsz = (uint64_t)o->block_size;
     const uint64_t table_b = o->level == KC_SPEED_BEST ? 0 : o->level == KC_SPEED_BETTER ? kc_zbetter_table_bytes() : (o->level == KC_SPEED_DEFAULT ? kc_zdfast_table_bytes() : kc_zfast_table_bytes());
-    const uint64_t per_block = 2 * (bsz / 4 + 8) * 8 + (bsz + 64) + sizeof(KcBlkMeta);
+    const uint64_t per_block = 2 * (bsz / 4 + 8) * 8 + (bsz + 64) + sizeof(KcBlkMeta) + KC_BH_WORDS * 4;
     const uint64_t hist0 = (o->dict != nullptr) ? o->dict_len : 0;
     const uint64_t blocks = (len + bsz - 1) / bsz + n_cuts;
     const uint64_t enc = ((uint64_t)kc_zstd_max_encoded_size(o, (int64_t)len) + 3 * n_cuts + 3 + 15) & ~(uint64_t)15;
@@ -809,7 +822,7 @@
     size_t fr = 0, tot = 0;
     if (hipMemGetInfo(&fr, &tot) == hipSuccess) {
         uint64_t held = 0;
-        const DevBuf* bufs[] = {&c->seqs, &c->aux, &c->lits, &c->meta, &c->stage, &c->tables, &c->work};
+        const DevBuf* bufs[] = {&c->seqs, &c->aux, &c->lits, &c->meta, &c->bhist, &c->stage, &c->tables, &c->work};
         for (const DevBuf* b : bufs) held += b->cap;
         const uint64_t avail = (uint64_t)((double)(fr + held) * 0.85);
         if (avail < budget) budget = avail;
diff --git a/compress_amd/csrc/kc_ctx.cpp b/compress_amd/csrc/kc_ctx.cpp
--- a/compress_amd/csrc/kc_ctx.cpp
+++ b/compress_amd/csrc/kc_ctx.cpp
@@ -282,7 +282,7 @@
 static void ctx_free_scratch(kc_ctx* c) {
     DevBuf* bufs[] = {&c->unit_off, &c->unit_blk0, &c->stage_off, &c->seqs, &c->aux, &c->lits, &c->meta, &c->stage, &c->out_size, &c->xxh,
                       &c->redo, &c->popmask, &c->unit_list, &c->out_off, &c->blk_start, &c->unit_flags, &c->redo_blk, &c->pop_blk, &c->predef, &c->errflag, &c->tmp_src, &c->tmp_dst, &c->tables, &c->prof, &c->work, &c->work_off, &c->dictbuf, &c->proto, &c->dicthuf,
-                      &c->d_job_hist, &c->d_job_flags, &c->rawdef, &c->unit_raw, &c->unit_done, &c->probe_rel, &c->best_tables, &c->best_cur, &c->best_cost};
+                      &c->d_job_hist, &c->d_job_flags, &c->rawdef, &c->unit_raw, &c->bhist, &c->unit_done, &c->probe_rel, &c->best_tables, &c->best_cur, &c->best_cost};
     for (DevBuf* b : bufs) {
         if (b->p) (void)hipFree(b->p);
         b->p = nullptr;
diff --git a/compress_amd/csrc/kc_dev.h b/compress_amd/csrc/kc_dev.h
--- a/compress_amd/csrc/kc_dev.h
+++ b/compress_amd/csrc/kc_dev.h
@@ -187,3 +187,7 @@
 };
 #define KC_BF_POP_A 1u
 #define KC_BF_FORCED 2u
+
+#define KC_BH_LIT 256
+#define KC_BH_SEQ (3 * 64)
+#define KC_BH_WORDS (KC_BH_LIT + KC_BH_SEQ)
diff --git a/compress_amd/csrc/kc_host.h b/compress_amd/csrc/kc_host.h
--- a/compress_amd/csrc/kc_host.h
+++ b/compress_amd/csrc/kc_host.h
@@ -125,7 +125,7 @@
     void* dictbuf_ptr = nullptr;
     DevBuf best_tables, best_cur, best_cost;
     uint32_t best_n = 0;
-    hipEvent_t ev[8] = {nullptr, nullptr, nullptr, nullptr, nullptr, nullptr, nullptr, nullptr};
+    hipEvent_t ev[9] = {nullptr, nullptr, nullptr, nullptr, nullptr, nullptr, nullptr, nullptr, nullptr};
     kc_timings last = {0, 0, 0, 0, 0, 0};
     size_t max_batch_bytes = (size_t)8 << 30;
     uint64_t max_scratch_bytes = (uint64_t)160 << 30;
@@ -141,6 +141,7 @@
     const uint8_t* job_tables = nullptr;
     bool job_primed = false;
     DevBuf d_job_hist, d_job_flags, rawdef, unit_raw;
+    DevBuf bhist;
     DevBuf zd[20];
     DevBuf s2d[13];
     DevBuf unit_done, probe_rel;
diff --git a/compress_amd/csrc/kc_kernels.h b/compress_amd/csrc/kc_kernels.h
--- a/compress_amd/csrc/kc_kernels.h
+++ b/compress_amd/csrc/kc_kernels.h
@@ -96,10 +96,14 @@
     uint32_t* err_flag;
     unsigned long long* prof;
     const uint32_t* unit_done;
+    uint32_t* bhist;
+    uint32_t max_unit_blocks;
+    uint32_t launch_blocks;
 };
 size_t kc_fse_predef_bytes();
 void kc_launch_fse_predef_init(void* d_predef, hipStream_t st);
-void kc_launch_zstd_entropy(const KcEntropyParams& P, uint32_t grid, hipStream_t st);
+void kc_launch_zstd_entropy(const KcEntropyParams& P, uint32_t grid, hipStream_t st, bool gathered = false);
+void kc_launch_zstd_litgather(const KcEntropyParams& P, uint32_t n_launch, hipStream_t st);
 
 struct KcPrescanParams {
     const uint8_t* src;
diff --git a/compress_amd/csrc/kc_zgather_dev.h b/compress_amd/csrc/kc_zgather_dev.h
--- /dev/null
+++ b/compress_amd/csrc/kc_zgather_dev.h
@@ -0,0 +1,20 @@
+#pragma once
+#include "kc_dev.h"
+#include "kc_wave.h"
+
+__device__ __forceinline__ uint64_t wave_incl_scan64(uint64_t v, int lane) {
+    const uint32_t lo = wave_incl_scan((uint32_t)v, lane), hi = wave_incl_scan((uint32_t)(v >> 32), lane);
+    return ((uint64_t)hi << 32) | lo;
+}
+
+enum { KC_PRE_RLE = 0, KC_PRE_RAW = 1, KC_PRE_LITS = 2, KC_PRE_FULL = 3 };
+__device__ __forceinline__ int kc_blk_pre(const KcBlkMeta& m, const uint64_t* __restrict__ sq, int size, bool rawAllLits, bool dictLit) {
+    bool litsOnly = m.nseq == 0u;
+    if (!litsOnly) {
+        const uint64_t s0 = sq[0];
+        if (m.nseq == 1u && m.nlit <= 1u && seq_ll(s0) == m.nlit && seq_of(s0) - 3u == 1u) return KC_PRE_RLE;
+        litsOnly = (m.flags & KC_BF_POP_A) != 0u;
+    }
+    if (litsOnly) return (rawAllLits || size < (dictLit ? 8 : 32)) ? KC_PRE_RAW : KC_PRE_LITS;
+    return KC_PRE_FULL;
+}
diff --git a/compress_amd/csrc/kc_zstd_entropy.hip b/compress_amd/csrc/kc_zstd_entropy.hip
--- a/compress_amd/csrc/kc_zstd_entropy.hip
+++ b/compress_amd/csrc/kc_zstd_entropy.hip
@@ -3,6 +3,7 @@
 #include "kc_fse_dev.h"
 #include "kc_huf_dev.h"
 #include "kc_frame_dev.h"
+#include "kc_zgather_dev.h"
 
 #define ET 256
 #ifndef SEQ_CHUNK
@@ -10,9 +11,6 @@
 #endif
 #ifndef KC_PACK_REUSE
 #define KC_PACK_REUSE 1
-#endif
-#ifndef KC_HCOPIES
-#define KC_HCOPIES 2
 #endif
 #ifndef KC_K2_WGS
 #define KC_K2_WGS 4
@@ -25,7 +23,6 @@
 #define CH_WB (KC_CHAIN_WARM / CH_SEG)
 static_assert(KC_CHAIN_WARM % CH_SEG == 0 && CH_WB >= 1 && CH_WB <= 3, "warm-up is whole segments");
 static_assert(SEQ_CHUNK % CH_SEG == 0 && SEQ_CHUNK / CH_SEG <= 64, "one segment per lane");
-#define LONG_RUN 32
 
 static_assert(sizeof(KcFsePredefBlob) == 3 * sizeof(KcFseT), "blob layout");
 size_t kc_fse_predef_bytes() { return sizeof(KcFsePredefBlob); }
@@ -55,10 +52,6 @@
     hipLaunchKernelGGL(kc_fse_predef_init_kernel, dim3(1), dim3(64), 0, st, (KcFsePredefBlob*)d_predef);
 }
 
-__device__ __forceinline__ uint64_t wave_incl_scan64(uint64_t v, int lane) {
-    const uint32_t lo = wave_incl_scan((uint32_t)v, lane), hi = wave_incl_scan((uint32_t)(v >> 32), lane);
-    return ((uint64_t)hi << 32) | lo;
-}
 __device__ __forceinline__ uint64_t block_excl_scan64(uint64_t v, uint64_t* wsum, uint64_t* total, int tid) {
     const int lane = tid & 63, w = tid >> 6;
     const uint64_t inc = wave_incl_scan64(v, lane);
@@ -106,7 +99,6 @@
 };
 
 struct Shared {
-    uint32_t whist[4 * KC_HCOPIES][256];
     uint32_t cnt[256];
     KcHufNodes nodes;
     KcHufTable cur;
@@ -133,6 +125,7 @@
     alignas(16) uint16_t sbits[3][CH_PAD + SEQ_CHUNK + 16];
     uint32_t cpk[3][64];
     uint16_t state[3];
+    uint32_t pk[1024];
     uint64_t wsum[4];
     uint32_t wtot[4];
     int ivar[24];
@@ -339,21 +332,10 @@
 #define PROF_MARK(i) do { if (P.prof && tid == 0) { const long long t1__ = clock64(); S.profAcc[i] += (unsigned long long)(t1__ - pt0); pt0 = t1__; } } while (0)
     if (P.prof && tid == 0) for (int i = 0; i < 24; i++) S.profAcc[i] = 0;
     if (P.prof && tid == 0) pt0 = clock64();
-#ifdef KC_K2_FINE
+#if defined(KC_K2_FINE) && KC_K2_FINE == 2
     long long pf0 = 0;
-#define PROF_FINE(i) do { if (P.prof && tid == 0) { __builtin_amdgcn_s_waitcnt(0); const long long t1__ = clock64(); S.profAcc[16 + (i)] += (unsigned long long)(t1__ - pf0); pf0 = t1__; } } while (0)
-#define PROF_FINE0() do { if (P.prof && tid == 0) { __builtin_amdgcn_s_waitcnt(0); pf0 = clock64(); } } while (0)
-#else
-#define PROF_FINE(i) do { } while (0)
-#define PROF_FINE0() do { } while (0)
-#endif
-#if defined(KC_K2_FINE) && KC_K2_FINE == 2
 #define PROF_FINB(i) do { if (P.prof && tid == 0) { __builtin_amdgcn_s_waitcnt(0); const long long t1__ = clock64(); S.profAcc[16 + (i)] += (unsigned long long)(t1__ - pf0); pf0 = t1__; } } while (0)
 #define PROF_FINB0() do { if (P.prof && tid == 0) { __builtin_amdgcn_s_waitcnt(0); pf0 = clock64(); } } while (0)
-#undef PROF_FINE
-#undef PROF_FINE0
-#define PROF_FINE(i) do { } while (0)
-#define PROF_FINE0() do { } while (0)
 #else
 #define PROF_FINB(i) do { } while (0)
 #define PROF_FINB0() do { } while (0)
@@ -427,24 +409,20 @@
             }
         };
 
-        bool litsOnly = false;
-        if (nseq == 0) {
-            litsOnly = true;
-        } else {
+        const bool dictLit = b == 0 && P.dict_huf != nullptr && !(streamU && P.stream_sync);
+        const int pre = kc_blk_pre(m, sq, size, rawAllLits, dictLit);
+        if (pre == KC_PRE_RLE) {
             const uint64_t s0 = sq[0];
-            if (nseq == 1 && nlit <= 1 && (int)seq_ll(s0) == nlit && seq_of(s0) - 3u == 1u) {
-                if (tid == 0) {
-                    put_block_header(bout, last, 1u, seq_ml(s0) + 3u + seq_ll(s0));
-                    bout[3] = org[0];
-                }
-                opos += 4;
-                __syncthreads();
-                continue;
-            }
-            if (m.flags & KC_BF_POP_A) litsOnly = true;
-        }
-        const bool dictLit = b == 0 && P.dict_huf != nullptr && !(streamU && P.stream_sync);
-        if (litsOnly && (rawAllLits || size < (dictLit ? 8 : 32))) {
+            if (tid == 0) {
+                put_block_header(bout, last, 1u, seq_ml(s0) + 3u + seq_ll(s0));
+                bout[3] = org[0];
+            }
+            opos += 4;
+            __syncthreads();
+            continue;
+        }
+        const bool litsOnly = pre != KC_PRE_FULL;
+        if (pre == KC_PRE_RAW) {
             if (tid == 0) put_block_header(bout, last, 0u, (uint32_t)size);
             raw_payload();
             opos += 3 + size;
@@ -455,192 +433,15 @@
         const int nlitE = litsOnly ? size : nlit;
 
         PROF_MARK(0);
-        for (int i = tid; i < 4 * KC_HCOPIES * 256; i += ET) ((uint32_t*)S.whist)[i] = 0;
-        if (!litsOnly) for (int i = tid; i < (int)((sizeof(S.codes) + sizeof(S.sbits)) / 16); i += ET) ((uint4*)&S.codes[0][0])[i] = make_uint4(0, 0, 0, 0);
-        if (!litsOnly) {
-            for (int i = tid; i < 3 * 64; i += ET) ((uint32_t*)S.shist)[i] = 0;
-            if (tid < 3) S.smax[tid] = 0;
-        }
-        __syncthreads();
-        if (litsOnly) {
-            for (int k = tid; k < size; k += ET) atomicAdd(&S.whist[wv * KC_HCOPIES + (lane & (KC_HCOPIES - 1))][org[k]], 1u);
-        } else
+        const uint32_t* __restrict__ rec = P.bhist + (size_t)(blk0 + (uint32_t)b) * KC_BH_WORDS;
+        if (!litsOnly && wv < 3) {
+            const uint32_t h = rec[KC_BH_LIT + 64 * wv + lane];
+            S.shist[wv][lane] = h;
+            const uint64_t nz = ballot64(h != 0u);
+            if (lane == 0) S.smax[wv] = nz ? 63u - (uint32_t)__builtin_clzll(nz) : 0u;
+        }
         {
-            uint8_t* __restrict__ tile = &S.codes[0][0];
-            constexpr int TWB = 2304;
-            constexpr int TWC = 2048;
-            static_assert(sizeof(S.codes) + sizeof(S.sbits) >= 4 * TWB, "four gather windows");
-            uint8_t* __restrict__ tw = tile + wv * TWB;
-            const uint8_t* __restrict__ bsrc = base + blkStart;
-            const int per = (((nseq + 3) >> 2) + 63) & ~63;
-            const int q0 = wv * per < nseq ? wv * per : nseq;
-            const int q1 = q0 + per < nseq ? q0 + per : nseq;
-            PROF_FINE0();
-            {
-                uint64_t acc = 0;
-                uint32_t mll = 0, mof = 0, mml = 0;
-                for (int i0 = q0 + lane; i0 < q1; i0 += 8 * 64) {
-                    uint64_t sv[8];
-#pragma unroll
-                    for (int r = 0; r < 8; r++) sv[r] = i0 + 64 * r < q1 ? sq[i0 + 64 * r] : 0ull;
-#pragma unroll
-                    for (int r = 0; r < 8; r++) {
-                        if (i0 + 64 * r < q1) {
-                            const uint32_t ll = seq_ll(sv[r]), ml = seq_ml(sv[r]), of = seq_of(sv[r]);
-                            acc += (uint64_t)ll | ((uint64_t)(ll + ml + 3u) << 32);
-                            const uint32_t cl = kc_ll_code(ll), co = kc_of_code(of), cm = kc_ml_code(ml);
-                            atomicAdd(&S.shist[0][cl], 1u);
-                            atomicAdd(&S.shist[1][co], 1u);
-                            atomicAdd(&S.shist[2][cm], 1u);
-                            mll = cl > mll ? cl : mll;
-                            mof = co > mof ? co : mof;
-                            mml = cm > mml ? cm : mml;
-                        }
-                    }
-                }
-                mll = wave_reduce_max(mll); mof = wave_reduce_max(mof); mml = wave_reduce_max(mml);
-                const uint64_t tot = wave_incl_scan64(acc, lane);
-                if (lane == 63) S.wsum[wv] = tot;
-                if (lane == 0) { atomicMax(&S.smax[0], mll); atomicMax(&S.smax[1], mof); atomicMax(&S.smax[2], mml); }
-            }
-            PROF_FINE(0);
-            __syncthreads();
-            PROF_FINE(1);
-            uint64_t run = 0;
-            for (int k = 0; k < wv; k++) run += S.wsum[k];
-            const uint32_t firstLo = (uint32_t)run;
-            const uint32_t fw = firstLo & ~15u;
-            const uint32_t hs = firstLo & 15u;
-            struct GStep { uint32_t ll, lo, sp; uint64_t tot, longMask; };
-            auto place = [&](uint64_t sx, bool have, uint64_t at, GStep& g) {
-                uint32_t ll = 0, adv = 0;
-                if (have) { ll = seq_ll(sx); adv = ll + seq_ml(sx) + 3u; }
-                const uint64_t v = (uint64_t)ll | ((uint64_t)adv << 32);
-                const uint64_t inc = wave_incl_scan64(v, lane);
-                g.tot = bcast64(inc, 63);
-                const uint64_t ex = inc - v + at;
-                g.ll = ll; g.lo = (uint32_t)ex; g.sp = (uint32_t)(ex >> 32);
-                g.longMask = ballot64(ll > LONG_RUN);
-            };
-            auto fetch = [&](const GStep& g, uint64_t (&vv)[4]) {
-#pragma unroll
-                for (int kk = 0; kk < 4; kk++) {
-                    const uint32_t k = 8u * (uint32_t)kk;
-                    vv[kk] = 0;
-                    if (g.ll <= LONG_RUN && k < g.ll) {
-                        const uint32_t n8 = g.ll - k < 8u ? g.ll - k : 8u;
-                        if ((int)(g.sp + k) + 8 <= size) vv[kk] = ld64(bsrc + g.sp + k);
-                        else { uint64_t t = 0; for (uint32_t q = 0; q < n8; q++) t |= (uint64_t)bsrc[g.sp + k + q] << (8 * q); vv[kk] = t; }
-                    }
-                }
-            };
-            GStep cur;
-            uint64_t vv[4];
-            uint64_t sq1 = q0 + lane < q1 ? sq[q0 + lane] : 0ull;
-            for (int t0 = q0; t0 < q1; t0 += 64) {
-                const int i = t0 + lane;
-                place(sq1, i < q1, run, cur);
-                sq1 = i + 64 < q1 ? sq[i + 64] : 0ull;
-                PROF_FINE(2);
-                fetch(cur, vv);
-                const uint32_t ll = cur.ll, lo = cur.lo, sp = cur.sp;
-                const uint64_t tot = cur.tot, longMask = cur.longMask;
-                const bool mine = ll > 0 && ll <= LONG_RUN;
-                const uint32_t begLo = (uint32_t)run;
-                const uint32_t endLo = begLo + (uint32_t)tot;
-                for (uint32_t winBase = begLo & ~15u; winBase < endLo; winBase += TWC) {
-                    if (mine && lo < winBase + TWC && lo + ll > winBase) {
-#pragma unroll
-                        for (int kk = 0; kk < 4; kk++) {
-                            const uint32_t k = 8u * (uint32_t)kk;
-                            if (k < ll) {
-                                const uint32_t n8 = ll - k < 8u ? ll - k : 8u;
-                                const uint64_t x = n8 < 8u ? vv[kk] & ((1ull << (8u * n8)) - 1ull) : vv[kk];
-                                const uint32_t o = lo + k - winBase;
-                                if (lo + k >= winBase && o + n8 <= (uint32_t)TWC) {
-                                    unsigned long long* pq = (unsigned long long*)(tw + (o & ~7u));
-                                    const uint32_t sh = (o & 7u) * 8u;
-                                    atomicOr(pq, (unsigned long long)(x << sh));
-                                    if (sh != 0u && (x >> (64u - sh)) != 0ull) atomicOr(pq + 1, (unsigned long long)(x >> (64u - sh)));
-                                } else {
-                                    for (uint32_t q = 0; q < n8; q++) {
-                                        const uint32_t oo = lo + k + q - winBase;
-                                        if (oo < (uint32_t)TWC) atomicOr((uint32_t*)(tw + (oo & ~3u)), (uint32_t)((x >> (8u * q)) & 0xFFu) << (8u * (oo & 3u)));
-                                    }
-                                }
-                            }
-                        }
-                    }
-                    for (uint64_t lm = longMask; lm != 0ull; lm &= lm - 1ull) {
-                        const int e = ctz64(lm);
-                        const uint32_t lsp = bcast32(sp, e), llo = bcast32(lo, e), lln = bcast32(ll, e);
-                        const uint32_t o0 = llo > winBase ? llo : winBase;
-                        const uint32_t o1 = llo + lln < winBase + TWC ? llo + lln : winBase + TWC;
-                        for (uint32_t o = o0 + 4u * (uint32_t)lane; o < o1; o += 4u * 64u) {
-                            const uint32_t n4 = o1 - o < 4u ? o1 - o : 4u;
-                            const uint32_t si = lsp + (o - llo);
-                            uint32_t x;
-                            if ((int)si + 4 <= size) x = ld32(bsrc + si);
-                            else { x = 0; for (uint32_t q = 0; q < n4; q++) x |= (uint32_t)bsrc[si + q] << (8u * q); }
-                            if (n4 < 4u) x &= (1u << (8u * n4)) - 1u;
-                            const uint32_t oo = o - winBase;
-                            unsigned long long* pq = (unsigned long long*)(tw + (oo & ~7u));
-                            const uint32_t sh = (oo & 7u) * 8u;
-                            atomicOr(pq, (unsigned long long)x << sh);
-                            if (sh > 32u && (x >> (64u - sh)) != 0u) atomicOr(pq + 1, (unsigned long long)(x >> (64u - sh)));
-                        }
-                    }
-                    KC_WAVE_SYNC();
-                    PROF_FINE(3);
-                    const uint32_t wEnd = endLo < winBase + TWC ? endLo : winBase + TWC;
-                    const uint32_t nfull = (wEnd - winBase) >> 4;
-                    const bool shared0 = hs != 0u && winBase == fw && nfull > 0u;
-                    if (shared0 && (uint32_t)lane >= hs && lane < 16) { const uint8_t c = tw[lane]; lits[fw + lane] = c; atomicAdd(&S.whist[wv * KC_HCOPIES][c], 1u); }
-                    for (uint32_t w = (shared0 ? 1u : 0u) + (uint32_t)lane; w < nfull; w += 64u) ((uint4*)(lits + winBase))[w] = ((const uint4*)tw)[w];
-                    for (uint32_t d = (shared0 ? 4u : 0u) + (uint32_t)lane; d < 4u * nfull; d += 64u) {
-                        const uint32_t x = ((const uint32_t*)tw)[d];
-                        uint32_t* const hc = S.whist[wv * KC_HCOPIES + (lane & (KC_HCOPIES - 1))];
-                        atomicAdd(&hc[x & 0xFFu], 1u);
-                        atomicAdd(&hc[(x >> 8) & 0xFFu], 1u);
-                        atomicAdd(&hc[(x >> 16) & 0xFFu], 1u);
-                        atomicAdd(&hc[x >> 24], 1u);
-                    }
-                    const uint32_t tail = (wEnd - winBase) & 15u;
-                    uint8_t carry = 0;
-                    if (nfull > 0u && lane < (int)tail) carry = tw[(nfull << 4) + lane];
-                    KC_WAVE_SYNC();
-                    PROF_FINE(4);
-                    if (nfull > 0u) {
-                        for (uint32_t w = 1u + (uint32_t)lane; w <= nfull; w += 64u) ((uint4*)tw)[w] = make_uint4(0, 0, 0, 0);
-                        if (lane < 16) tw[lane] = carry;
-                    }
-                    KC_WAVE_SYNC();
-                    PROF_FINE(5);
-                }
-                run += tot;
-            }
-            {
-                const uint32_t total = (uint32_t)run;
-                const uint32_t rem = total & 15u;
-                const uint32_t lowT = ((total & ~15u) == fw) ? hs : 0u;
-                if ((uint32_t)lane >= lowT && (uint32_t)lane < rem) { const uint8_t c = tw[lane]; lits[(total & ~15u) + lane] = c; atomicAdd(&S.whist[wv * KC_HCOPIES][c], 1u); }
-            }
-            {
-                const uint32_t len = m.extra_lits, spos = (uint32_t)size - len, lo = (uint32_t)nlit - len;
-                for (uint32_t k = tid; k < len; k += ET) {
-                    const uint8_t c = bsrc[spos + k];
-                    lits[lo + k] = c;
-                    atomicAdd(&S.whist[wv * KC_HCOPIES][c], 1u);
-                }
-            }
-            PROF_FINE(6);
-        }
-        __syncthreads();
-        PROF_FINE(7);
-        {
-            uint32_t c = 0;
-#pragma unroll
-            for (int k = 0; k < 4 * KC_HCOPIES; k++) c += S.whist[k][tid];
+            const uint32_t c = rec[tid];
             S.cnt[tid] = c;
             const uint32_t wm = wave_reduce_max(c);
             const uint32_t wl = wave_reduce_max(c ? (uint32_t)tid + 1u : 0u);
@@ -1100,7 +901,7 @@
                 uint64_t tot;
                 const uint64_t ex = block_excl_scan64((uint64_t)(fb0 + fb1), S.wsum, &tot, tid) + bitRun;
                 if ((int64_t)((bitRun + tot + 7) >> 3) >= (int64_t)seqBudgetBytes) { overflow = true; break; }
-                uint32_t* __restrict__ pk = (uint32_t*)S.whist;
+                uint32_t* __restrict__ pk = S.pk;
                 const uint32_t wbase = (uint32_t)(bitRun >> 5);
                 const int nwords = (int)((((uint32_t)bitRun & 31u) + (uint32_t)tot + 31u) >> 5);
                 for (int i = tid; i < nwords + 2; i += ET) pk[i] = i == 0 ? carry : 0u;
@@ -1199,6 +1000,7 @@
     }
 }
 
-void kc_launch_zstd_entropy(const KcEntropyParams& P, uint32_t grid, hipStream_t st) {
+void kc_launch_zstd_entropy(const KcEntropyParams& P, uint32_t grid, hipStream_t st, bool gathered) {
+    if (!gathered) kc_launch_zstd_litgather(P, grid, st);
     hipLaunchKernelGGL(kc_zstd_entropy_kernel, dim3(grid), dim3(ET), 0, st, P);
 }
diff --git a/compress_amd/csrc/kc_zstd_litgather.hip b/compress_amd/csrc/kc_zstd_litgather.hip
--- /dev/null
+++ b/compress_amd/csrc/kc_zstd_litgather.hip
@@ -0,0 +1,244 @@
+#include "kc_dev.h"
+#include "kc_kernels.h"
+#include "kc_fse_dev.h"
+#include "kc_zgather_dev.h"
+
+#define GT 256
+#define G_LONG_RUN 32
+#define G_TWB 2304
+#define G_TWC 2048
+
+struct GatherShared {
+    alignas(16) uint8_t tile[4 * G_TWB];
+    uint32_t whist[4][256];
+    uint32_t shist[3][64];
+    uint64_t wsum[4];
+};
+static_assert(sizeof(GatherShared) <= 16 * 1024, "fits beside a full match-finder residency");
+
+__device__ __forceinline__ void gather_locate(const KcEntropyParams& P, uint32_t n_launch, uint32_t bpu, uint32_t& u, int& b) {
+    if (P.launch_blocks == 0u) {
+        const uint32_t idx = blockIdx.x / bpu;
+        b = (int)(blockIdx.x % bpu);
+        u = P.unit_list ? P.unit_list[idx] : P.unit_base + idx;
+    } else {
+        const uint32_t g = P.unit_blk0[P.unit_base] + blockIdx.x;
+        uint32_t lo = P.unit_base, hi = P.unit_base + n_launch - 1u;
+        while (lo < hi) {
+            const uint32_t mid = lo + ((hi - lo) >> 1);
+            if (P.unit_blk0[mid + 1u] > g) hi = mid; else lo = mid + 1u;
+        }
+        u = lo;
+        b = (int)(g - P.unit_blk0[lo]);
+    }
+}
+
+__global__ __launch_bounds__(GT, 5) void kc_zstd_litgather_kernel(KcEntropyParams P, uint32_t n_launch, uint32_t bpu) {
+    __shared__ GatherShared S;
+    const int tid = (int)threadIdx.x, lane = tid & 63, wv = tid >> 6;
+    uint32_t u;
+    int b;
+    gather_locate(P, n_launch, bpu, u, b);
+    if (P.unit_done != nullptr && P.unit_done[u] != 0u) return;
+    const uint8_t* __restrict__ base = P.src + P.unit_off[u];
+    const int hist0 = P.unit_hist != nullptr ? (int)P.unit_hist[u] : P.hist0;
+    const int ulen = (int)(P.unit_off[u + 1] - P.unit_off[u]) - hist0;
+    const uint32_t blk0 = P.unit_blk0[u];
+    const int bs = P.block_size;
+    const KcUnitBlocks UB = kc_unit_blocks(P.blk_start, P.unit_flags, P.unit_blk0, u, ulen, bs, P.stream_mode);
+    const int nblk = UB.nblk;
+    if (ulen <= 0 || b >= nblk) return;
+    const KcBlkMeta m = P.meta[blk0 + (uint32_t)b];
+    const int blkStart = hist0 + kc_blk_begin(P.blk_start, blk0, b, bs);
+    const int blkEnd = hist0 + kc_blk_end(P.blk_start, blk0, b, nblk, bs, ulen);
+    const int size = blkEnd - blkStart;
+    const uint8_t* __restrict__ bsrc = base + blkStart;
+    const uint64_t* __restrict__ sq = P.seqs + (size_t)(blk0 + (uint32_t)b) * P.seq_stride;
+    uint8_t* __restrict__ lits = P.lits + (size_t)(blk0 + (uint32_t)b) * P.lit_stride;
+    uint32_t* __restrict__ rec = P.bhist + (size_t)(blk0 + (uint32_t)b) * KC_BH_WORDS;
+    const int nseq = (int)m.nseq;
+    const int nlit = (int)m.nlit;
+    const bool dictLit = b == 0 && P.dict_huf != nullptr && !(UB.streamU && P.stream_sync);
+    const int pre = kc_blk_pre(m, sq, size, !P.all_lit_entropy, dictLit);
+    if (pre == KC_PRE_RLE || pre == KC_PRE_RAW) return;
+
+    for (int i = tid; i < 4 * 256; i += GT) ((uint32_t*)S.whist)[i] = 0;
+    for (int i = tid; i < (int)(sizeof(S.tile) / 16); i += GT) ((uint4*)S.tile)[i] = make_uint4(0, 0, 0, 0);
+    if (tid < 3 * 64) ((uint32_t*)S.shist)[tid] = 0;
+    __syncthreads();
+    if (pre == KC_PRE_LITS) {
+        for (int k = tid; k < size; k += GT) atomicAdd(&S.whist[wv][bsrc[k]], 1u);
+    } else {
+        constexpr int TWC = G_TWC;
+        uint8_t* __restrict__ tw = S.tile + wv * G_TWB;
+        const int per = (((nseq + 3) >> 2) + 63) & ~63;
+        const int q0 = wv * per < nseq ? wv * per : nseq;
+        const int q1 = q0 + per < nseq ? q0 + per : nseq;
+        {
+            uint64_t acc = 0;
+            for (int i0 = q0 + lane; i0 < q1; i0 += 8 * 64) {
+                uint64_t sv[8];
+#pragma unroll
+                for (int r = 0; r < 8; r++) sv[r] = i0 + 64 * r < q1 ? sq[i0 + 64 * r] : 0ull;
+#pragma unroll
+                for (int r = 0; r < 8; r++) {
+                    if (i0 + 64 * r < q1) {
+                        const uint32_t ll = seq_ll(sv[r]), ml = seq_ml(sv[r]), of = seq_of(sv[r]);
+                        acc += (uint64_t)ll | ((uint64_t)(ll + ml + 3u) << 32);
+                        atomicAdd(&S.shist[0][kc_ll_code(ll)], 1u);
+                        atomicAdd(&S.shist[1][kc_of_code(of)], 1u);
+                        atomicAdd(&S.shist[2][kc_ml_code(ml)], 1u);
+                    }
+                }
+            }
+            const uint64_t tot = wave_incl_scan64(acc, lane);
+            if (lane == 63) S.wsum[wv] = tot;
+        }
+        __syncthreads();
+        uint64_t run = 0;
+        for (int k = 0; k < wv; k++) run += S.wsum[k];
+        const uint32_t firstLo = (uint32_t)run;
+        const uint32_t fw = firstLo & ~15u;
+        const uint32_t hs = firstLo & 15u;
+        struct GStep { uint32_t ll, lo, sp; uint64_t tot, longMask; };
+        auto place = [&](uint64_t sx, bool have, uint64_t at, GStep& g) {
+            uint32_t ll = 0, adv = 0;
+            if (have) { ll = seq_ll(sx); adv = ll + seq_ml(sx) + 3u; }
+            const uint64_t v = (uint64_t)ll | ((uint64_t)adv << 32);
+            const uint64_t inc = wave_incl_scan64(v, lane);
+            g.tot = bcast64(inc, 63);
+            const uint64_t ex = inc - v + at;
+            g.ll = ll; g.lo = (uint32_t)ex; g.sp = (uint32_t)(ex >> 32);
+            g.longMask = ballot64(ll > G_LONG_RUN);
+        };
+        auto fetch = [&](const GStep& g, uint64_t (&vv)[4]) {
+#pragma unroll
+            for (int kk = 0; kk < 4; kk++) {
+                const uint32_t k = 8u * (uint32_t)kk;
+                vv[kk] = 0;
+                if (g.ll <= G_LONG_RUN && k < g.ll) {
+                    const uint32_t n8 = g.ll - k < 8u ? g.ll - k : 8u;
+                    if ((int)(g.sp + k) + 8 <= size) vv[kk] = ld64(bsrc + g.sp + k);
+                    else { uint64_t t = 0; for (uint32_t q = 0; q < n8; q++) t |= (uint64_t)bsrc[g.sp + k + q] << (8 * q); vv[kk] = t; }
+                }
+            }
+        };
+        GStep cur;
+        uint64_t vv[4];
+        uint64_t sq1 = q0 + lane < q1 ? sq[q0 + lane] : 0ull;
+        for (int t0 = q0; t0 < q1; t0 += 64) {
+            const int i = t0 + lane;
+            place(sq1, i < q1, run, cur);
+            sq1 = i + 64 < q1 ? sq[i + 64] : 0ull;
+            fetch(cur, vv);
+            const uint32_t ll = cur.ll, lo = cur.lo, sp = cur.sp;
+            const uint64_t tot = cur.tot, longMask = cur.longMask;
+            const bool mine = ll > 0 && ll <= G_LONG_RUN;
+            const uint32_t begLo = (uint32_t)run;
+            const uint32_t endLo = begLo + (uint32_t)tot;
+            for (uint32_t winBase = begLo & ~15u; winBase < endLo; winBase += TWC) {
+                if (mine && lo < winBase + TWC && lo + ll > winBase) {
+#pragma unroll
+                    for (int kk = 0; kk < 4; kk++) {
+                        const uint32_t k = 8u * (uint32_t)kk;
+                        if (k < ll) {
+                            const uint32_t n8 = ll - k < 8u ? ll - k : 8u;
+                            const uint64_t x = n8 < 8u ? vv[kk] & ((1ull << (8u * n8)) - 1ull) : vv[kk];
+                            const uint32_t o = lo + k - winBase;
+                            if (lo + k >= winBase && o + n8 <= (uint32_t)TWC) {
+                                unsigned long long* pq = (unsigned long long*)(tw + (o & ~7u));
+                                const uint32_t sh = (o & 7u) * 8u;
+                                atomicOr(pq, (unsigned long long)(x << sh));
+                                if (sh != 0u && (x >> (64u - sh)) != 0ull) atomicOr(pq + 1, (unsigned long long)(x >> (64u - sh)));
+                            } else {
+                                for (uint32_t q = 0; q < n8; q++) {
+                                    const uint32_t oo = lo + k + q - winBase;
+                                    if (oo < (uint32_t)TWC) atomicOr((uint32_t*)(tw + (oo & ~3u)), (uint32_t)((x >> (8u * q)) & 0xFFu) << (8u * (oo & 3u)));
+                                }
+                            }
+                        }
+                    }
+                }
+                for (uint64_t lm = longMask; lm != 0ull; lm &= lm - 1ull) {
+                    const int e = ctz64(lm);
+                    const uint32_t lsp = bcast32(sp, e), llo = bcast32(lo, e), lln = bcast32(ll, e);
+                    const uint32_t o0 = llo > winBase ? llo : winBase;
+                    const uint32_t o1 = llo + lln < winBase + TWC ? llo + lln : winBase + TWC;
+                    for (uint32_t o = o0 + 4u * (uint32_t)lane; o < o1; o += 4u * 64u) {
+                        const uint32_t n4 = o1 - o < 4u ? o1 - o : 4u;
+                        const uint32_t si = lsp + (o - llo);
+                        uint32_t x;
+                        if ((int)si + 4 <= size) x = ld32(bsrc + si);
+                        else { x = 0; for (uint32_t q = 0; q < n4; q++) x |= (uint32_t)bsrc[si + q] << (8u * q); }
+                        if (n4 < 4u) x &= (1u << (8u * n4)) - 1u;
+                        const uint32_t oo = o - winBase;
+                        unsigned long long* pq = (unsigned long long*)(tw + (oo & ~7u));
+                        const uint32_t sh = (oo & 7u) * 8u;
+                        atomicOr(pq, (unsigned long long)x << sh);
+                        if (sh > 32u && (x >> (64u - sh)) != 0u) atomicOr(pq + 1, (unsigned long long)(x >> (64u - sh)));
+                    }
+                }
+                KC_WAVE_SYNC();
+                const uint32_t wEnd = endLo < winBase + TWC ? endLo : winBase + TWC;
+                const uint32_t nfull = (wEnd - winBase) >> 4;
+                const bool shared0 = hs != 0u && winBase == fw && nfull > 0u;
+                if (shared0 && (uint32_t)lane >= hs && lane < 16) { const uint8_t c = tw[lane]; lits[fw + lane] = c; atomicAdd(&S.whist[wv][c], 1u); }
+                for (uint32_t w = (shared0 ? 1u : 0u) + (uint32_t)lane; w < nfull; w += 64u) ((uint4*)(lits + winBase))[w] = ((const uint4*)tw)[w];
+                for (uint32_t d = (shared0 ? 4u : 0u) + (uint32_t)lane; d < 4u * nfull; d += 64u) {
+                    const uint32_t x = ((const uint32_t*)tw)[d];
+                    uint32_t* const hc = S.whist[wv];
+                    atomicAdd(&hc[x & 0xFFu], 1u);
+                    atomicAdd(&hc[(x >> 8) & 0xFFu], 1u);
+                    atomicAdd(&hc[(x >> 16) & 0xFFu], 1u);
+                    atomicAdd(&hc[x >> 24], 1u);
+                }
+                const uint32_t tail = (wEnd - winBase) & 15u;
+                uint8_t carry = 0;
+                if (nfull > 0u && lane < (int)tail) carry = tw[(nfull << 4) + lane];
+                KC_WAVE_SYNC();
+                if (nfull > 0u) {
+                    for (uint32_t w = 1u + (uint32_t)lane; w <= nfull; w += 64u) ((uint4*)tw)[w] = make_uint4(0, 0, 0, 0);
+                    if (lane < 16) tw[lane] = carry;
+                }
+                KC_WAVE_SYNC();
+            }
+            run += tot;
+        }
+        {
+            const uint32_t total = (uint32_t)run;
+            const uint32_t rem = total & 15u;
+            const uint32_t lowT = ((total & ~15u) == fw) ? hs : 0u;
+            if ((uint32_t)lane >= lowT && (uint32_t)lane < rem) { const uint8_t c = tw[lane]; lits[(total & ~15u) + lane] = c; atomicAdd(&S.whist[wv][c], 1u); }
+        }
+        {
+            const uint32_t len = m.extra_lits, spos = (uint32_t)size - len, lo = (uint32_t)nlit - len;
+            for (uint32_t k = tid; k < len; k += GT) {
+                const uint8_t c = bsrc[spos + k];
+                lits[lo + k] = c;
+                atomicAdd(&S.whist[wv][c], 1u);
+            }
+        }
+    }
+    __syncthreads();
+    rec[tid] = S.whist[0][tid] + S.whist[1][tid] + S.whist[2][tid] + S.whist[3][tid];
+    if (pre == KC_PRE_FULL && tid < KC_BH_SEQ) rec[KC_BH_LIT + tid] = ((const uint32_t*)S.shist)[tid];
+}
+
+void kc_launch_zstd_litgather(const KcEntropyParams& P, uint32_t n_launch, hipStream_t st) {
+    if (n_launch == 0u) return;
+    if (P.launch_blocks != 0u && P.unit_list == nullptr) {
+        hipLaunchKernelGGL(kc_zstd_litgather_kernel, dim3(P.launch_blocks), dim3(GT), 0, st, P, n_launch, 1u);
+        return;
+    }
+    const uint32_t bpu = P.max_unit_blocks;
+    if (bpu == 0u) return;
+    KcEntropyParams Q = P;
+    Q.launch_blocks = 0u;
+    const uint32_t per = (0x7FFFFFFFu / bpu) ? (0x7FFFFFFFu / bpu) : 1u;
+    for (uint32_t u0 = 0; u0 < n_launch; u0 += per) {
+        const uint32_t n = n_launch - u0 < per ? n_launch - u0 : per;
+        Q.unit_base = P.unit_base + u0;
+        Q.unit_list = P.unit_list ? P.unit_list + u0 : nullptr;
+        hipLaunchKernelGGL(kc_zstd_litgather_kernel, dim3(n * bpu), dim3(GT), 0, st, Q, n, bpu);
+    }
+}
```

Result: no change. 29280 (median of 4 runs) (+0.6%).
